# ikergarcia1996/AI-Generated-GTAV

Measured on AMD Instinct MI355X. Metric: generated frames/sec (32-frame clip, 100 noise steps), higher is better.
Workload: dtype fp16 (fp32 accumulate/residual)

## Files before the change

### ai-generated-gtav_amd/csrc/api_dit.hip

```cpp
#include "api_internal.h"

#ifdef GTAV_EXPERIMENTS
static int fold_alloc(gtav_dit* h) {
    gtav_dit::Fold& f = h->fold;
    if (f.ok) return 0;
    GTAV_REQUIRE(f.geom_ok, "dit_set_fold: this geometry has no LayerNorm fold (tokens per frame %d must be a multiple of 16 and >= 64, hidden %% 256 == 0)", h->P);
    Arena& a = h->arena;
    const int D = h->D;
    const size_t Mx = round_up(h->Mmax, 128);
    int rc = 0;
#define A_(expr) do { if (!rc) rc = (expr); } while (0)
    {
        const int nhb = h->L * 2, nseam = 2 * nhb + 1;
        f.col_c.assign(nseam, 0);
        int col = 0;
        for (int hb = 0; hb < nhb; ++hb) { f.col_c[2 * hb + 1] = col; col += 2 * h->Hm; }
        for (int hb = 0; hb < nhb; ++hb) { f.col_c[2 * hb] = col; col += 2 * 3 * D; }
        f.col_c[2 * nhb] = col; col += 2 * h->Nfin;
        f.CTW = col;
        f.n_groups = 2 * nseam; f.n_groups_a = 2 * nhb;
        f.Rp = round_up(h->max_rows, 128);
        A_(a.alloc_t(&f.ctab, (size_t)h->max_rows * f.CTW));
        A_(a.alloc_t(&f.ctab_cur, (size_t)h->maxB * h->maxT * f.CTW));
        A_(a.alloc_t(&f.stats, Mx * (size_t)(D / 64) * 2));
        A_(a.alloc_t(&f.sx, (size_t)f.n_groups * f.Rp * D));
        A_(a.alloc_t(&f.groups_dev, f.n_groups)); A_(a.alloc_t(&f.gcol_dev, f.n_groups)); A_(a.alloc_t(&f.gscale_dev, f.n_groups));
        if (!rc) {
            std::vector<GemmGroup> groups(f.n_groups);
            std::vector<int> gcol(f.n_groups), gsc(f.n_groups);
            auto add = [&](int q, int seam, const f16* W, int N, const float* bias, int shift_col, int scale_col) {
                for (int kind = 0; kind < 2; ++kind) {
                    GemmGroup& g = groups[2 * q + kind];
                    g.X = f.sx + (size_t)(2 * q + kind) * f.Rp * D; g.W = W; g.N = N; g.ldo = f.CTW;
                    g.out = f.ctab + f.col_c[seam] + (kind ? N : 0); g.bias = kind ? bias : nullptr;
                    gcol[2 * q + kind] = kind ? shift_col : scale_col; gsc[2 * q + kind] = kind ? 0 : 1;
                }
            };
            for (int hb = 0; hb < nhb; ++hb) {
                add(hb, 2 * hb + 1, h->halves[hb].w_fc1, h->Hm, h->halves[hb].b_fc1, (hb * 6 + 3) * D, (hb * 6 + 4) * D);
                add(nhb + hb, 2 * hb, h->halves[hb].w_qkv, 3 * D, nullptr, (hb * 6 + 0) * D, (hb * 6 + 1) * D);
            }
            add(2 * nhb, 2 * nhb, h->w_final, h->Nfin, h->b_final, h->L * 12 * D, h->L * 12 * D + D);
            if (hipMemcpy(f.groups_dev, groups.data(), groups.size() * sizeof(GemmGroup), hipMemcpyHostToDevice) != hipSuccess ||
                hipMemcpy(f.gcol_dev, gcol.data(), gcol.size() * sizeof(int), hipMemcpyHostToDevice) != hipSuccess ||
                hipMemcpy(f.gscale_dev, gsc.data(), gsc.size() * sizeof(int), hipMemcpyHostToDevice) != hipSuccess) {
                set_error("dit_create: upload of the LayerNorm-fold group tables failed");
                rc = 1;
            }
            f.ok = !rc;
        }
    }
#undef A_
    return rc;
}
#endif

static bool fused_spatial_ok(int M, int D, int P) { return gemm_qkvs_attn_ok(M, D, P) && M / P >= 5 && (M / P) * (D / 64) >= 80; }

static void fold_policy(const gtav_dit* h, int M, bool& fa, bool& fb) {
    const gtav_dit::Fold& f = h->fold;
    fa = fb = false;
    if (!f.ok || f.mode == 0 || h->tr.on || h->fuse_tattn || h->any_bf16) return;
    fa = f.mode == 2 || M >= f.min_m_a;
    fb = f.mode == 2 || M >= f.min_m_b;
}
static int dit_fold_tables(gtav_dit* h, int rows, bool fa, bool fb, hipStream_t s) {
    if (!fa && !fb) return 0;
#ifndef GTAV_EXPERIMENTS
    (void)h; (void)rows; (void)s;
    GTAV_REQUIRE(false, "the LayerNorm fold exists only in the experiments build");
#else
    gtav_dit::Fold& f = h->fold;
    const int ng = fb ? f.n_groups : f.n_groups_a;
    RET_IF(launch_ctab_inputs(h->mod, h->MODW, rows, round_up(rows, 128), h->D, f.gcol_dev, f.gscale_dev, ng, f.sx, (size_t)f.Rp * h->D, s));
    return launch_gemm_grouped(f.groups_dev, ng, h->Hm > 3 * h->D ? h->Hm : 3 * h->D, rows, h->D, s);
#endif
}

static int dit_cond(gtav_dit* h, const int64_t* t64, int rows, int Tq, const StepParams* sp, int use_cur, const float* actions,
                    int64_t act_outer, int64_t act_inner, hipStream_t s) {
    GTAV_REQUIRE(rows <= h->max_rows, "conditioning rows %d exceed max_cond_rows %d", rows, h->max_rows);
    const int ldhc = h->D + h->Apad;
    RET_IF(launch_cond_inputs(t64, rows, Tq, sp, use_cur, h->sincos, h->E, actions, act_outer, act_inner, h->A, h->HC, ldhc,
                              h->D, h->Apad, h->err_flag, s));
    RET_IF(launch_skinny_f32(h->E, 256, h->w_t0, h->b_t0, h->HC, ldhc, rows, h->D, 256, 1, s));
    RET_IF(launch_skinny_f32(h->HC, ldhc, h->w_t2cat, actions ? h->b_t2a : h->b_t2, h->Sc, h->D, rows, h->D, ldhc, 1, s));
    RET_IF(launch_skinny_f32(h->Sc, h->D, h->w_ada, h->b_ada, h->mod, h->MODW, rows, h->MODW, h->D, 0, s));
    bool fa, fb;
    fold_policy(h, rows * h->P, fa, fb);
    return dit_fold_tables(h, rows, fa, fb, s);
}

static int dit_forward_core(gtav_dit* h, const float* x_src, const int* frame_index, int B, int Tq, int t0,
                            const float* mod, const int* mod_rows, const float* ctab, float* v_out, hipStream_t s) {
    const int D = h->D, P = h->P, NB = B * Tq, M = NB * P;
    GTAV_REQUIRE(M <= h->Mmax, "forward: %d tokens exceed workspace (%d)", M, h->Mmax);
    bool fold_a, fold_b;
    fold_policy(h, M, fold_a, fold_b);
    const gtav_dit::Fold& fo = h->fold;
    auto fold_consumer = [&](GemmParams& q, int seam, int N) {
        q.bias = nullptr;
        q.f_P = P; q.f_rows = mod_rows; q.f_stats = fo.stats; q.f_nslot = D / 64;
        q.f_c1 = ctab + fo.col_c[seam]; q.f_c2 = q.f_c1 + N; q.f_ldc = fo.CTW;
    };
    auto fold_producer = [&](int cls, const f16* X, const f16* Wt, int K, const float* bias, const float* gate, const float* next_scale) -> int {
        GemmParams q;
        memset(&q, 0, sizeof(q));
        q.X = X; q.ldx = K; q.W = Wt; q.M = M; q.N = D; q.K = K; q.out = h->resid; q.ldo = D; q.bias = bias; q.err_flag = h->err_flag;
        q.gate = gate; q.gate_stride = h->MODW; q.gate_rows = mod_rows; q.rows_per_gate = P;
        q.f_P = P; q.f_rows = mod_rows; q.f_scale = next_scale; q.f_stats_out = fo.stats; q.f_a = h->xn;
        PROF(h, cls, s, launch_gemm(q, EPI_RESID_FOLD, s));
        return 0;
    };
    const int g_embed = 2 * h->L, g_final = 2 * h->L + 1;
    PROF(h, PC_OTHER, s, h->ops(g_embed).patchify(x_src, frame_index, NB, h->C, h->H, h->W, h->p, h->xp, h->Kpe, 1.f, 0.f, h->err_of(g_embed), s));
    GemmParams g;
    memset(&g, 0, sizeof(g));
    g.X = h->xp; g.ldx = h->Kpe; g.W = h->w_pe; g.M = M; g.N = D; g.K = h->Kpe; g.bias = h->b_pe; g.out = h->resid; g.ldo = D;
    PROF(h, PC_OTHER, s, h->ops(g_embed).gemm(g, EPI_F32, s));
    LnPending pend;
    bool have_pend = false;
    const int pf_max_m = 1536;
    static const int pf_min_m = GTAV_ENV_INT("GTAV_PF_MIN_M", 256);
    const bool pf_on = h->w_prefetch && M >= pf_min_m && M <= pf_max_m;
    struct PfNext { const f16* W; int N, K, sk, consumer; };
    auto pf_target = [&](int hb, int pos) -> PfNext {
        const int q = pos + 1, hb2 = hb + q / 4, p2 = q % 4;
        if (!pf_on || hb2 >= 2 * h->L) return PfNext{nullptr, 0, 0, 1, 0};
        const gtav_dit::Half& w2 = h->halves[hb2];
        if (p2 == 0) {
            const bool fused2 = !h->tr.on && w2.w_qkv_hm && !h->ops(hb2).bf16 &&
                                ((hb2 & 1) ? h->fuse_tattn && gemm_qkvt_attn_ok(M, D, P, Tq, t0) : h->fuse_sattn && fused_spatial_ok(M, D, P));
            return PfNext{fused2 ? w2.w_qkv_hm : w2.w_qkv, 3 * D, D, 1, 3};
        }
        if (p2 == 1) return PfNext{w2.w_out, D, D, gemm_choose_splitk(M, D, D), 0};
        if (p2 == 2) return PfNext{w2.w_fc1, h->Hm, D, 1, 1};
        return PfNext{w2.w_fc2, D, h->Hm_pad, gemm_choose_splitk(M, D, h->Hm_pad), 2};
    };
    auto set_pf = [&](GemmParams& q, const PfNext& t) {
        const int v = h->w_prefetch_cls[t.consumer];
        if (!pf_on || !t.W || !v) return;
        const int nkt = t.K / 64;
        int skn = t.sk;
        if (skn < 1 || nkt % skn || (skn >= 8 ? skn % 8 : 8 % skn)) skn = 1;
        q.pf = PrefetchDesc{t.W, cdiv(t.N, 128), nkt, skn, v >= 2 ? v : 0};
    };
    auto resid_gemm = [&](const OperandOps& ops, int cls, const f16* X, int ldx, const f16* Wt, int K, const float* bias, const float* gate, const PfNext& pfn) -> int {
        GemmParams q;
        memset(&q, 0, sizeof(q));
        q.X = X; q.ldx = ldx; q.W = Wt; q.M = M; q.N = D; q.K = K; q.out = h->parts; q.ldo = D;
        set_pf(q, pfn);
        q.splitk = gemm_choose_splitk(M, D, K);
        if (gemm_pp_ok(M, D, K, EPI_RESID) || (q.splitk == 1 && M >= h->resid_inplace_min_m) || gemm_resid_inplace_ok(M, D, K, P)) {
            q.splitk = 0; q.out = h->resid; q.bias = bias; q.gate = gate; q.gate_stride = h->MODW; q.gate_rows = mod_rows;
            q.rows_per_gate = P;
            PROF(h, cls, s, ops.gemm(q, EPI_RESID, s));
            have_pend = false;
            return 0;
        }
        GTAV_REQUIRE((size_t)q.splitk * M <= h->parts_rows, "split-K slabs exceed workspace");
        PROF(h, cls, s, ops.gemm(q, EPI_PARTIAL, s));
        memset(&pend, 0, sizeof(pend));
        pend.parts = h->parts; pend.nsplit = q.splitk; pend.slab_stride = (size_t)M * D; pend.ld = D; pend.bias = bias;
        pend.gate = gate; pend.gate_stride = h->MODW; pend.gate_rows = mod_rows; pend.rows_per_gate = P;
        have_pend = true;
        return 0;
    };
    bool folded_in = false;
    for (int l = 0; l < h->L; ++l) {
        for (int hf = 0; hf < 2; ++hf) {
            const int hb = l * 2 + hf;
            const gtav_dit::Half& w = h->halves[hb];
            const OperandOps& ops = h->ops(hb);
            int* const ef = h->err_of(hb);
            const float* mb = mod + (size_t)hb * 6 * D;
            const bool fused_t = hf == 1 && h->fuse_tattn && !h->tr.on && !ops.bf16 && w.w_qkv_hm && gemm_qkvt_attn_ok(M, D, P, Tq, t0);
            if (fused_t) {
                if (!have_pend) memset(&pend, 0, sizeof(pend));
                pend.tperm_T = Tq; pend.tperm_P = P;
            }
            if (!folded_in)
                PROF(h, PC_LN, s, ops.ln_modulate(h->resid, D, h->xn, D, M, D, mb, mb + D, h->MODW, mod_rows, P, (have_pend || fused_t) ? &pend : nullptr, ef, s));
            have_pend = false;
            memset(&g, 0, sizeof(g));
            g.X = h->xn; g.ldx = D; g.W = w.w_qkv; g.M = M; g.N = 3 * D; g.K = D; g.D = D; g.S = P; g.err_flag = ef;
            if (folded_in) fold_consumer(g, 2 * hb, 3 * D);
            set_pf(g, pf_target(hb, 0));
            const bool fused_s = hf == 0 && h->fuse_sattn && !h->tr.on && !ops.bf16 && !folded_in && w.w_qkv_hm && fused_spatial_ok(M, D, P);
            if (fused_t) {
                g.W = w.w_qkv_hm; g.qkv_mode = QKV_TEMPORAL; g.k = h->kvcache[l]; g.v = h->kvcache[l]; g.out = h->ao; g.ldo = D;
                g.Tq = Tq; g.t0 = t0; g.Tmax = h->maxT; g.rope_cs = h->rope_t.cs_dev;
                PROF(h, PC_ATTN_T, s, launch_gemm_qkvt_attn(g, s));
            } else if (fused_s) {
                g.W = w.w_qkv_hm; g.qkv_mode = QKV_SPATIAL; g.out = h->ao; g.ldo = D; g.rope_cs = h->rope_s.cs_dev;
                PROF(h, PC_ATTN_S, s, launch_gemm_qkvs_attn(g, s));
            } else {
                if (hf == 0) {
                    g.qkv_mode = QKV_SPATIAL; g.q = h->qs; g.k = h->ks; g.v = h->vts;
                    g.rope_cs = h->rope_s.cs_dev;
                } else {
                    g.qkv_mode = QKV_TEMPORAL; g.q = h->qt; g.k = h->kvcache[l]; g.v = h->kvcache[l];
                    g.Tq = Tq; g.t0 = t0; g.Tmax = h->maxT;
                    g.rope_cs = h->rope_t.cs_dev;
                }
                PROF(h, PC_QKV, s, ops.gemm(g, folded_in ? EPI_QKV_FOLD : EPI_QKV, s));
                if (hf == 0) PROF(h, PC_ATTN_S, s, ops.attn_spatial(h->qs, h->ks, h->vts, h->ao, NB, h->heads, P, s, false));
                else PROF(h, PC_ATTN_T, s, ops.attn_temporal(h->qt, h->kvcache[l], h->ao, B, P, D, Tq, t0, h->maxT, s));
            }
            folded_in = false;
            memset(&g, 0, sizeof(g));
            g.X = h->xn; g.ldx = D; g.W = w.w_fc1; g.M = M; g.N = h->Hm; g.K = D; g.bias = w.b_fc1; g.out = h->hbuf; g.ldo = h->Hm_pad; g.err_flag = ef;
            set_pf(g, pf_target(hb, 2));
            if (fold_a) {
                RET_IF(fold_producer(PC_OUT, h->ao, w.w_out, D, w.b_out, mb + 2 * D, mb + 4 * D));
                fold_consumer(g, 2 * hb + 1, h->Hm);
                PROF(h, PC_FC1, s, launch_gemm(g, EPI_GELU_TANH_FOLD, s));
            } else {
                RET_IF(resid_gemm(ops, PC_OUT, h->ao, D, w.w_out, D, w.b_out, mb + 2 * D, pf_target(hb, 1)));
                PROF(h, PC_LN, s, ops.ln_modulate(h->resid, D, h->xn, D, M, D, mb + 3 * D, mb + 4 * D, h->MODW, mod_rows, P, have_pend ? &pend : nullptr, ef, s));
                have_pend = false;
                PROF(h, PC_FC1, s, ops.gemm(g, EPI_GELU_TANH, s));
            }
            if (fold_b) {
                const float* next_scale = hb + 1 < 2 * h->L ? mod + (size_t)(hb + 1) * 6 * D + D : mod + (size_t)h->L * 12 * D + D;
                RET_IF(fold_producer(PC_FC2, h->hbuf, w.w_fc2, h->Hm_pad, w.b_fc2, mb + 5 * D, next_scale));
                folded_in = true;
            } else {
                RET_IF(resid_gemm(ops, PC_FC2, h->hbuf, h->Hm_pad, w.w_fc2, h->Hm_pad, w.b_fc2, mb + 5 * D, pf_target(hb, 3)));
            }
        }
    }
    const float* mf = mod + (size_t)h->L * 12 * D;
    if (!folded_in)
        PROF(h, PC_LN, s, h->ops(g_final).ln_modulate(h->resid, D, h->xn, D, M, D, mf, mf + D, h->MODW, mod_rows, P, have_pend ? &pend : nullptr, h->err_of(g_final), s));
    memset(&g, 0, sizeof(g));
    g.X = h->xn; g.ldx = D; g.W = h->w_final; g.M = M; g.N = h->Nfin; g.K = D; g.bias = h->b_final; g.out = h->fo; g.ldo = h->Nfin;
    if (folded_in) fold_consumer(g, 4 * h->L, h->Nfin);
    PROF(h, PC_OTHER, s, h->ops(g_final).gemm(g, folded_in ? EPI_F32_FOLD : EPI_F32, s));
    PROF(h, PC_OTHER, s, launch_unpatchify(h->fo, h->Nfin, v_out, NB, h->C, h->H, h->W, h->p, 0, 1.f, 0.f, s));
    PROF(h, PC_EMPTY, s, 0);
    return h->prof.collect(s);
}

extern "C" {



int gtav_dit_create(const gtav_dit_config* c, gtav_dit** out) {
    GTAV_REQUIRE(c && out, "dit_create: null argument");
    GTAV_REQUIRE(c->hidden_size % 256 == 0 && c->hidden_size <= 2048, "hidden_size=%d must be a multiple of 256, <= 2048", c->hidden_size);
    GTAV_REQUIRE(c->num_heads > 0 && c->hidden_size / c->num_heads == 64 && c->hidden_size % c->num_heads == 0,
                 "only head_dim 64 is implemented (hidden %d, heads %d)", c->hidden_size, c->num_heads);
    GTAV_REQUIRE(c->input_h % c->patch_size == 0 && c->input_w % c->patch_size == 0, "input %dx%d not divisible by patch %d",
                 c->input_h, c->input_w, c->patch_size);
    GTAV_REQUIRE(c->max_frames >= 1 && c->max_frames <= 32, "max_frames=%d must be in [1, 32]", c->max_frames);
    GTAV_REQUIRE(c->max_batch >= 1 && c->depth >= 1, "bad max_batch/depth");
    RET_IF(skinny_init());
    gtav_dit* h = new gtav_dit();
    h->cfg = *c;
    h->D = c->hidden_size; h->L = c->depth; h->heads = c->num_heads; h->C = c->in_channels; h->p = c->patch_size;
    h->H = c->input_h; h->W = c->input_w; h->gh = h->H / h->p; h->gw = h->W / h->p; h->P = h->gh * h->gw;
    const int D = h->D;
    if ((h->P % 8) != 0) {
        set_error("tokens per frame P=%d must be a multiple of 8", h->P);
        delete h;
        return 2;
    }
    h->Hm = (int)(D * c->mlp_ratio); h->Hm_pad = round_up(h->Hm, 128);
    h->A = c->external_cond_dim > 0 ? c->external_cond_dim : 0; h->Apad = round_up(h->A > 0 ? h->A : 1, 32);
    h->MODW = h->L * 12 * D + 2 * D;
    h->Kpe = round_up(h->C * h->p * h->p, 64);
    h->Nfin = h->p * h->p * h->C;
    h->maxB = c->max_batch; h->maxT = c->max_frames; h->Mmax = h->maxB * h->maxT * h->P;
    h->max_rows = c->max_cond_rows > h->maxB * h->maxT ? c->max_cond_rows : h->maxB * h->maxT;
    Arena& a = h->arena;
    WeightTable& wt = h->wt;
    int rc = 0;
#define A_(expr) do { if (!rc) rc = (expr); } while (0)
    A_(a.alloc_t(&h->w_pe, (size_t)round_up(D, 128) * h->Kpe));
    h->n_groups = 2 * h->L + 2;
    h->grp_bf16.assign(h->n_groups, 0);
    wt.add_f16("x_embedder.proj.weight", D, h->C * h->p * h->p, h->w_pe, round_up(D, 128), h->Kpe, 2 * h->L);
    A_(a.alloc_t(&h->b_pe, D)); wt.add_f32("x_embedder.proj.bias", 1, D, h->b_pe, D);
    A_(a.alloc_t(&h->w_t0, (size_t)D * 256)); wt.add_f32("t_embedder.mlp.0.weight", D, 256, h->w_t0, 256);
    A_(a.alloc_t(&h->b_t0, D)); wt.add_f32("t_embedder.mlp.0.bias", 1, D, h->b_t0, D);
    const int ldhc = D + h->Apad;
    A_(a.alloc_t(&h->w_t2cat, (size_t)D * ldhc)); wt.add_f32("t_embedder.mlp.2.weight", D, D, h->w_t2cat, ldhc, 0);
    A_(a.alloc_t(&h->b_t2, D)); wt.add_f32("t_embedder.mlp.2.bias", 1, D, h->b_t2, D);
    A_(a.alloc_t(&h->b_ext, D)); A_(a.alloc_t(&h->b_t2a, D));
    if (h->A > 0) {
        wt.add_f32("external_cond.weight", D, h->A, h->w_t2cat, ldhc, D);
        wt.add_f32("external_cond.bias", 1, D, h->b_ext, D);
    }
    A_(a.alloc_t(&h->w_ada, (size_t)h->MODW * D)); A_(a.alloc_t(&h->b_ada, h->MODW));
    h->halves.resize(h->L * 2);
    h->fuse_sattn = h->P == 144 && D % 256 == 0;
    for (int l = 0; l < h->L && !rc; ++l)
        for (int hf = 0; hf < 2; ++hf) {
            gtav_dit::Half& w = h->halves[l * 2 + hf];
            char pre[64];
            snprintf(pre, sizeof(pre), "blocks.%d.%c_", l, hf == 0 ? 's' : 't');
            std::string P_(pre);
            const int grp = l * 2 + hf;
            A_(a.alloc_t(&w.w_qkv, (size_t)3 * D * D)); wt.add_f16(P_ + "attn.to_qkv.weight", 3 * D, D, w.w_qkv, 3 * D, D, grp);
            w.w_qkv_hm = nullptr;
            if (hf == 0 && h->P == 144 && D % 256 == 0) A_(a.alloc_t(&w.w_qkv_hm, (size_t)3 * D * D));
            A_(a.alloc_t(&w.w_out, (size_t)D * D)); wt.add_f16(P_ + "attn.to_out.weight", D, D, w.w_out, D, D, grp);
            A_(a.alloc_t(&w.b_out, D)); wt.add_f32(P_ + "attn.to_out.bias", 1, D, w.b_out, D);
            A_(a.alloc_t(&w.w_fc1, (size_t)h->Hm_pad * D)); wt.add_f16(P_ + "mlp.fc1.weight", h->Hm, D, w.w_fc1, h->Hm_pad, D, grp);
            A_(a.alloc_t(&w.b_fc1, h->Hm_pad)); wt.add_f32(P_ + "mlp.fc1.bias", 1, h->Hm, w.b_fc1, h->Hm);
            A_(a.alloc_t(&w.w_fc2, (size_t)D * h->Hm_pad)); wt.add_f16(P_ + "mlp.fc2.weight", D, h->Hm, w.w_fc2, D, h->Hm_pad, grp);
            A_(a.alloc_t(&w.b_fc2, D)); wt.add_f32(P_ + "mlp.fc2.bias", 1, D, w.b_fc2, D);
            const size_t row0 = (size_t)(l * 2 + hf) * 6 * D;
            wt.add_f32(P_ + "adaLN_modulation.1.weight", 6 * D, D, h->w_ada + row0 * D, D);
            wt.add_f32(P_ + "adaLN_modulation.1.bias", 1, 6 * D, h->b_ada + row0, 6 * D);
        }
    A_(a.alloc_t(&h->w_final, (size_t)round_up(h->Nfin, 128) * D));
    wt.add_f16("final_layer.linear.weight", h->Nfin, D, h->w_final, round_up(h->Nfin, 128), D, 2 * h->L + 1);
    A_(a.alloc_t(&h->b_final, round_up(h->Nfin, 128))); wt.add_f32("final_layer.linear.bias", 1, h->Nfin, h->b_final, h->Nfin);
    {
        const size_t row0 = (size_t)h->L * 12 * D;
        wt.add_f32("final_layer.adaLN_modulation.1.weight", 2 * D, D, h->w_ada + row0 * D, D);
        wt.add_f32("final_layer.adaLN_modulation.1.bias", 1, 2 * D, h->b_ada + row0, 2 * D);
    }
    A_(a.alloc_t(&h->sincos, (size_t)1000 * 256)); wt.add_f32("tables.timestep_sincos", 1000, 256, h->sincos, 256, 0, false);
    h->rope_s.npos = h->P; h->rope_t.npos = h->maxT;
    A_(a.alloc_t(&h->rope_s.cos_dev, (size_t)h->P * 64)); wt.add_f32("tables.rope_spatial_cos", h->P, 64, h->rope_s.cos_dev, 64, 0, false);
    A_(a.alloc_t(&h->rope_s.sin_dev, (size_t)h->P * 64)); wt.add_f32("tables.rope_spatial_sin", h->P, 64, h->rope_s.sin_dev, 64, 0, false);
    A_(a.alloc_t(&h->rope_t.cos_dev, (size_t)h->maxT * 64)); wt.add_f32("tables.rope_temporal_cos", h->maxT, 64, h->rope_t.cos_dev, 64, 0, false);
    A_(a.alloc_t(&h->rope_t.sin_dev, (size_t)h->maxT * 64)); wt.add_f32("tables.rope_temporal_sin", h->maxT, 64, h->rope_t.sin_dev, 64, 0, false);
    A_(a.alloc_t(&h->rope_s.cs_dev, (size_t)h->P * 64)); A_(a.alloc_t(&h->rope_t.cs_dev, (size_t)h->maxT * 64));
    A_(a.alloc_t(&h->freqs_s_dev, 16)); wt.add_f32("spatial_rotary_emb.freqs", 1, 16, h->freqs_s_dev, 16, 0, false);
    A_(a.alloc_t(&h->freqs_t_dev, 32)); wt.add_f32("temporal_rotary_emb.freqs", 1, 32, h->freqs_t_dev, 32, 0, false);
    const size_t Mx = round_up(h->Mmax, 128);
    A_(a.alloc_t(&h->xp, Mx * h->Kpe)); A_(a.alloc_t(&h->xn, Mx * D)); A_(a.alloc_t(&h->qs, Mx * D)); A_(a.alloc_t(&h->ks, Mx * D));
    A_(a.alloc_t(&h->vts, Mx * D)); A_(a.alloc_t(&h->qt, Mx * D)); A_(a.alloc_t(&h->ao, Mx * D)); A_(a.alloc_t(&h->hbuf, Mx * h->Hm_pad));
    h->kvcache.resize(h->L);
    for (int l = 0; l < h->L; ++l) A_(a.alloc_t(&h->kvcache[l], Mx * 2 * D));
    A_(a.alloc_t(&h->resid, Mx * D)); A_(a.alloc_t(&h->fo, Mx * h->Nfin));
    A_(a.alloc_t(&h->vout, Mx / h->P * h->C * h->H * h->W));
    h->parts_rows = (2 * Mx * D > (size_t)(8u << 20) ? 2 * Mx * D : (size_t)(8u << 20)) / D;
    A_(a.alloc_t(&h->parts, h->parts_rows * D));
    const size_t R = h->max_rows;
    A_(a.alloc_t(&h->E, R * 256)); A_(a.alloc_t(&h->HC, R * ldhc)); A_(a.alloc_t(&h->Sc, R * D)); A_(a.alloc_t(&h->mod, R * h->MODW));
    A_(a.alloc_t(&h->err_flag, 4 + h->n_groups)); A_(a.alloc_t(&h->frame_idx, (size_t)h->maxB * h->maxT)); A_(a.alloc_t(&h->ac_table, 1000));
    A_(a.alloc_t(&h->step_dev, 4)); A_(a.alloc_t(&h->mod_rows_dev, (size_t)h->maxB * h->maxT));
    A_(a.alloc_t(&h->mod_cur, (size_t)h->maxB * h->maxT * h->MODW)); A_(a.alloc_t(&h->mod_last, (size_t)h->maxB * h->maxT)); A_(a.alloc_t(&h->mod_changed, (size_t)h->maxB * h->maxT)); A_(a.alloc_t(&h->t_steps_dev, 1024));
    wt.err_words = h->err_flag; wt.err_per_group = true;
    h->use_graph = GTAV_ENV_INT("GTAV_GRAPH", 1) != 0;
    h->fold.geom_ok = h->P % 16 == 0 && h->P >= 64 && D % 256 == 0 && h->Hm % 128 == 0 && h->Nfin % 4 == 0;
#undef A_
    if (rc) {
        delete h;
        return rc;
    }
    *out = h;
    return 0;
}

void gtav_dit_destroy(gtav_dit* h) { delete h; }

int gtav_dit_set_weight(gtav_dit* h, const char* name, const float* src, int64_t numel, void* stream) {
    GTAV_REQUIRE(h && name && src, "dit_set_weight: null argument");
    std::string n(name);
    if (n.size() > 16 && n.compare(n.size() - 16, 16, "rotary_emb.freqs") == 0) {
        const bool spatial = n.rfind("spatial_", 0) == 0 || n.find(".s_attn.") != std::string::npos;
        n = spatial ? "spatial_rotary_emb.freqs" : "temporal_rotary_emb.freqs";
    }
    h->finalized = false;
    return h->wt.set(n.c_str(), src, numel, (hipStream_t)stream);
}

int gtav_dit_get_weight(gtav_dit* h, const char* name, float* dst, int64_t numel, void* stream) {
    GTAV_REQUIRE(h && name && dst, "dit_get_weight: null argument");
    return h->wt.get(name, dst, numel, (hipStream_t)stream);
}

int gtav_dit_finalize(gtav_dit* h, void* stream) {
    GTAV_REQUIRE(h, "dit_finalize: null handle");
    hipStream_t s = (hipStream_t)stream;
    RET_IF(h->wt.check_complete());
    GTAV_CHECK_HIP(hipStreamSynchronize(s));
    const int D = h->D;
    RET_IF(launch_add_f32(h->b_t2, h->b_ext, h->b_t2a, D, s));
    std::vector<float> fs(16), ft(32);
    if (h->wt.slots["spatial_rotary_emb.freqs"].set) GTAV_CHECK_HIP(hipMemcpy(fs.data(), h->freqs_s_dev, 64, hipMemcpyDeviceToHost));
    else { std::vector<float> l = linspace_f32(1.0f, 128.0f, 16); for (int i = 0; i < 16; ++i) fs[i] = l[i] * (float)M_PI; }
    if (h->wt.slots["temporal_rotary_emb.freqs"].set) GTAV_CHECK_HIP(hipMemcpy(ft.data(), h->freqs_t_dev, 128, hipMemcpyDeviceToHost));
    else for (int i = 0; i < 32; ++i) ft[i] = 1.0f / powf(10000.0f, (float)(2 * i) / 64.0f);
    if (!(h->wt.slots["tables.rope_spatial_cos"].set && h->wt.slots["tables.rope_spatial_sin"].set)) {
        std::vector<float> c, sn;
        build_axial_table(fs, h->gh, h->gw, c, sn);
        RET_IF(upload(h->rope_s.cos_dev, c)); RET_IF(upload(h->rope_s.sin_dev, sn));
    }
    if (!(h->wt.slots["tables.rope_temporal_cos"].set && h->wt.slots["tables.rope_temporal_sin"].set)) {
        std::vector<float> c((size_t)h->maxT * 64), sn((size_t)h->maxT * 64);
        for (int t = 0; t < h->maxT; ++t)
            for (int d = 0; d < 64; ++d) {
                const float ang = (float)t * ft[d / 2];
                c[t * 64 + d] = cosf(ang); sn[t * 64 + d] = sinf(ang);
            }
        RET_IF(upload(h->rope_t.cos_dev, c)); RET_IF(upload(h->rope_t.sin_dev, sn));
    }
    if (!h->wt.slots["tables.timestep_sincos"].set) {
        std::vector<float> tab((size_t)1000 * 256);
        for (int k = 0; k < 128; ++k) {
            const float f = expf(-logf(10000.0f) * (float)k / 128.0f);
            for (int t = 0; t < 1000; ++t) {
                const float arg = (float)t * f;
                tab[(size_t)t * 256 + k] = cosf(arg);
                tab[(size_t)t * 256 + 128 + k] = sinf(arg);
            }
        }
        RET_IF(upload(h->sincos, tab));
    }
    for (size_t hb = 0; hb < h->halves.size(); ++hb) {
        gtav_dit::Half& w = h->halves[hb];
        if (w.w_qkv_hm) RET_IF(launch_qkv_head_major(w.w_qkv, w.w_qkv_hm, D, s, (hb & 1) ? 0 : 1));
    }
    RET_IF(launch_rope_interleave(h->rope_s.cos_dev, h->rope_s.sin_dev, h->rope_s.cs_dev, h->P, s));
    RET_IF(launch_rope_interleave(h->rope_t.cos_dev, h->rope_t.sin_dev, h->rope_t.cs_dev, h->maxT, s));
    GTAV_CHECK_HIP(hipStreamSynchronize(s));
    h->finalized = true;
    return 0;
}

int gtav_dit_forward(gtav_dit* h, const float* x, const int64_t* t, const float* actions, float* out, int32_t B, int32_t T,
                     void* stream) {
    GTAV_REQUIRE(h && x && t && out, "dit_forward: null argument");
    GTAV_REQUIRE(h->finalized, "dit_forward: call gtav_dit_finalize first");
    GTAV_REQUIRE(B >= 1 && B <= h->maxB && T >= 1 && T <= h->maxT, "dit_forward: B=%d T=%d outside capacity (%d, %d)", B, T, h->maxB, h->maxT);
    GTAV_REQUIRE(!actions || h->A > 0, "dit_forward: model has no external_cond");
    hipStream_t s = (hipStream_t)stream;
    h->prepared.valid = false;
    h->kvrec.valid = false;
    RET_IF(dit_cond(h, t, B * T, 1, nullptr, 0, actions, h->A, 0, s));
    return dit_forward_core(h, x, nullptr, B, T, 0, h->mod, nullptr, h->fold.ctab, out, s);
}

int gtav_dit_set_schedule(gtav_dit* h, const float* ac, int32_t n) {
    GTAV_REQUIRE(h && ac && n == 1000, "dit_set_schedule: expected 1000 alphas_cumprod values");
    h->ac_host.assign(ac, ac + n);
    GTAV_CHECK_HIP(hipMemcpy(h->ac_table, ac, n * sizeof(float), hipMemcpyHostToDevice));
    return 0;
}

static int denoise_step_body(gtav_dit* h, float* x, int B, int F, int T, const float* actions, int mode, float* v_out,
                             bool prepared, hipStream_t s) {
    const size_t fsz = (size_t)h->C * h->H * h->W;
    const int Tq = mode == 1 ? 1 : T, t0 = mode == 1 ? T - 1 : 0;
    if (!prepared) RET_IF(dit_cond(h, nullptr, B * Tq, Tq, h->step_dev, mode == 1, actions, (int64_t)F * h->A, h->A, s));
    RET_IF(dit_forward_core(h, x, h->frame_idx, B, Tq, t0, prepared ? h->mod_cur : h->mod, nullptr, prepared ? h->fold.ctab_cur : h->fold.ctab, h->vout, s));
    const float* vlast = h->vout + (size_t)(Tq - 1) * fsz;
    RET_IF(launch_ddim_update_step(x, F, vlast, (size_t)Tq * fsz, B, (int)fsz, h->step_dev, s));
    if (v_out) RET_IF(launch_copy_rows_f32(vlast, (size_t)Tq * fsz, v_out, fsz, B, fsz, s));
    return 0;
}

int gtav_dit_prepare_frame(gtav_dit* h, int32_t B, int32_t F, int32_t start, int32_t cur, int32_t t_ctx,
                           const int32_t* t_steps_host, int32_t n_steps, const float* actions, void* stream) {
    GTAV_REQUIRE(h && t_steps_host, "prepare_frame: null argument");
    GTAV_REQUIRE(h->finalized, "prepare_frame: finalize the model first");
    const int T = cur - start + 1;
    GTAV_REQUIRE(start >= 0 && cur < F && T >= 1 && T <= h->maxT && B >= 1 && B <= h->maxB && n_steps >= 1 && n_steps <= 1024,
                 "prepare_frame: bad window [%d, %d] / steps %d", start, cur, n_steps);
    GTAV_REQUIRE(!actions || h->A > 0, "prepare_frame: model has no external_cond");
    const int rows = B * (T - 1) + n_steps * B;
    GTAV_REQUIRE(rows <= h->max_rows, "prepare_frame: %d conditioning rows exceed max_cond_rows %d", rows, h->max_rows);
    hipStream_t s = (hipStream_t)stream;
    GTAV_CHECK_HIP(hipStreamSynchronize(s));
    GTAV_CHECK_HIP(hipMemcpy(h->t_steps_dev, t_steps_host, n_steps * sizeof(int), hipMemcpyHostToDevice));
    const int ldhc = h->D + h->Apad;
    RET_IF(launch_cond_inputs_frame(rows, B, T, F, start, cur, t_ctx, h->t_steps_dev, h->sincos, h->E, actions, h->A, h->HC, ldhc,
                                    h->D, h->Apad, h->err_flag, s));
    RET_IF(launch_skinny_f32(h->E, 256, h->w_t0, h->b_t0, h->HC, ldhc, rows, h->D, 256, 1, s));
    RET_IF(launch_skinny_f32(h->HC, ldhc, h->w_t2cat, actions ? h->b_t2a : h->b_t2, h->Sc, h->D, rows, h->D, ldhc, 1, s));
    RET_IF(launch_skinny_f32(h->Sc, h->D, h->w_ada, h->b_ada, h->mod, h->MODW, rows, h->MODW, h->D, 0, s));
    {
        bool fa, fb, fa1, fb1;
        fold_policy(h, B * T * h->P, fa, fb);
        fold_policy(h, B * h->P, fa1, fb1);
        RET_IF(dit_fold_tables(h, rows, fa || fa1, fb || fb1, s));
        h->prepared.fold_tables = fa || fa1 || fb || fb1;
    }
    GTAV_CHECK_HIP(hipMemsetAsync(h->mod_last, 0xFF, (size_t)h->maxB * h->maxT * sizeof(int), s));
    h->prepared.valid = true; h->prepared.B = B; h->prepared.F = F; h->prepared.start = start; h->prepared.cur = cur;
    h->prepared.n_steps = n_steps; h->prepared.actions = actions;
    return 0;
}

int gtav_dit_denoise_step(gtav_dit* h, float* x, int32_t B, int32_t F, int32_t start, int32_t cur, int32_t t_ctx,
                          int32_t t_cur, int32_t t_next, int32_t is_final, const float* actions, int32_t mode,
                          int32_t cond_step, float* v_out, void* stream) {
    GTAV_REQUIRE(h && x, "denoise_step: null argument");
    GTAV_REQUIRE(h->finalized && !h->ac_host.empty(), "denoise_step: finalize the model and set the schedule first");
    const int T = cur - start + 1;
    GTAV_REQUIRE(start >= 0 && cur < F && T >= 1 && T <= h->maxT && B >= 1 && B <= h->maxB, "denoise_step: bad window [%d, %d] of %d frames", start, cur, F);
    GTAV_REQUIRE(t_cur >= 0 && t_cur < 1000 && t_next >= 0 && t_next < 1000 && t_ctx >= 0 && t_ctx < 1000, "denoise_step: timestep out of range");
    GTAV_REQUIRE(!actions || h->A > 0, "denoise_step: model has no external_cond");
    GTAV_REQUIRE(mode == 0 || mode == 1, "denoise_step: mode %d", mode);
    const bool prepared = cond_step >= 0;
    if (prepared)
        GTAV_REQUIRE(h->prepared.valid && h->prepared.B == B && h->prepared.F == F && h->prepared.start == start &&
                         h->prepared.cur == cur && cond_step < h->prepared.n_steps && h->prepared.actions == actions,
                     "denoise_step: cond_step=%d but gtav_dit_prepare_frame was not called for this window", cond_step);
    else
        h->prepared.valid = false;
    if (mode == 1) {
        GTAV_REQUIRE(h->kvrec.valid && h->kvrec.B == B && h->kvrec.F == F && h->kvrec.start == start && h->kvrec.cur == cur &&
                         h->kvrec.x == (const void*)x,
                     "denoise_step: context-cached step (mode 1) on window [%d, %d] without a preceding full-window step (mode 0) "
                     "on the same batch / window / latent buffer: the temporal K/V caches would be stale", start, cur);
    } else {
        h->kvrec.valid = true; h->kvrec.B = B; h->kvrec.F = F; h->kvrec.start = start; h->kvrec.cur = cur; h->kvrec.x = x;
    }
    hipStream_t s = (hipStream_t)stream;
    StepParams sp;
    sp.first = start; sp.cur = cur; sp.t_ctx = t_ctx; sp.t_cur = t_cur; sp.is_final = is_final != 0;
    sp.alpha_t = h->ac_host[t_cur]; sp.alpha_next = h->ac_host[t_next]; sp.cond_step = cond_step;
    RET_IF(launch_step_setup(h->step_dev, sp, h->frame_idx, h->mod_rows_dev, prepared ? h->mod_last : nullptr, h->mod_changed, B, mode == 1 ? 1 : T, T, F,
                             mode == 1, s));
    if (prepared) RET_IF(launch_gather_rows(h->mod, h->mod_rows_dev, h->mod_changed, h->mod_cur, B * (mode == 1 ? 1 : T), h->MODW,
                                            h->prepared.fold_tables ? h->fold.ctab : nullptr, h->fold.ctab_cur, h->fold.CTW, s));
    if (!h->use_graph || h->prof.on) return denoise_step_body(h, x, B, F, T, actions, mode, v_out, prepared, s);

    gtav_dit::GraphKey key{B, F, T, mode * 2 + (prepared ? 1 : 0), x, actions, v_out};
    auto it = h->graphs.find(key);
    if (it == h->graphs.end()) {
        if (h->graphs.size() > 64) {
            for (auto& kv : h->graphs)
                if (kv.second) (void)hipGraphExecDestroy(kv.second);
            h->graphs.clear();
        }
        h->graphs[key] = nullptr;
        return denoise_step_body(h, x, B, F, T, actions, mode, v_out, prepared, s);
    }
    if (!it->second) {
        if (!h->cap_stream && hipStreamCreateWithFlags(&h->cap_stream, hipStreamNonBlocking) != hipSuccess) {
            h->use_graph = false;
            return denoise_step_body(h, x, B, F, T, actions, mode, v_out, prepared, s);
        }
        hipGraph_t graph = nullptr;
        if (hipStreamBeginCapture(h->cap_stream, hipStreamCaptureModeThreadLocal) != hipSuccess) {
            (void)hipGetLastError();
            h->use_graph = false;
            return denoise_step_body(h, x, B, F, T, actions, mode, v_out, prepared, s);
        }
        const int rc = denoise_step_body(h, x, B, F, T, actions, mode, v_out, prepared, h->cap_stream);
        const hipError_t ce = hipStreamEndCapture(h->cap_stream, &graph);
        if (rc || ce != hipSuccess || !graph) {
            if (graph) (void)hipGraphDestroy(graph);
            h->use_graph = false;
            if (rc) return rc;
            return denoise_step_body(h, x, B, F, T, actions, mode, v_out, prepared, s);
        }
        hipGraphExec_t exec = nullptr;
        const hipError_t ie = hipGraphInstantiate(&exec, graph, nullptr, nullptr, 0);
        (void)hipGraphDestroy(graph);
        if (ie != hipSuccess || !exec) {
            h->use_graph = false;
            return denoise_step_body(h, x, B, F, T, actions, mode, v_out, prepared, s);
        }
        it->second = exec;
    }
    GTAV_CHECK_HIP(hipGraphLaunch(it->second, s));
    return 0;
}

int gtav_dit_set_graph(gtav_dit* h, int32_t enable) {
    GTAV_REQUIRE(h, "dit_set_graph: null handle");
    h->use_graph = enable != 0;
    return 0;
}

int gtav_dit_set_weight_prefetch(gtav_dit* h, int32_t enable) {
    GTAV_REQUIRE(h, "dit_set_weight_prefetch: null handle");
    GTAV_REQUIRE(enable == 0 || enable == 1 || (enable >> 16) == 1,
                 "dit_set_weight_prefetch: mode %d (0 off, 1 on, 0x10000 | per-class nibbles: bits 0-3 out-proj's weight, 4-7 fc1's, 8-11 fc2's, 12-15 to_qkv's; "
                 "nibble 0 = not prefetched, 1 = the whole slice, k >= 2 = the first k K tiles of every row tile)", enable);
    int cls[4];
    for (int c = 0; c < 4; ++c) cls[c] = enable == 0 ? 0 : enable == 1 ? 1 : (enable >> (4 * c)) & 15;
    const bool on = cls[0] || cls[1] || cls[2] || cls[3];
    if (h->w_prefetch != on || memcmp(cls, h->w_prefetch_cls, sizeof(cls))) {
        for (auto& kv : h->graphs)
            if (kv.second) (void)hipGraphExecDestroy(kv.second);
        h->graphs.clear();
    }
    h->w_prefetch = on;
    memcpy(h->w_prefetch_cls, cls, sizeof(cls));
    return 0;
}

#ifdef GTAV_EXPERIMENTS
int gtav_dit_set_fold(gtav_dit* h, int32_t mode, int32_t min_tokens_a, int32_t min_tokens_b) {
    GTAV_REQUIRE(h && mode >= 0 && mode <= 2, "dit_set_fold: mode %d", mode);
    if (min_tokens_a >= 0) h->fold.min_m_a = min_tokens_a;
    if (min_tokens_b >= 0) h->fold.min_m_b = min_tokens_b;
    if (mode == 2 || (mode == 1 && (h->fold.min_m_a < (1 << 30) || h->fold.min_m_b < (1 << 30)))) RET_IF(fold_alloc(h));
    for (auto& kv : h->graphs)
        if (kv.second) (void)hipGraphExecDestroy(kv.second);
    h->graphs.clear();
    h->prepared.valid = false;
    h->fold.mode = mode;
    return 0;
}
#endif

int gtav_dit_set_fused_temporal(gtav_dit* h, int32_t enable) {
    GTAV_REQUIRE(h, "dit_set_fused_temporal: null handle");
    if (h->fuse_tattn != (enable != 0)) {
        for (auto& kv : h->graphs)
            if (kv.second) (void)hipGraphExecDestroy(kv.second);
        h->graphs.clear();
    }
    if (enable && h->P % 16 == 0 && h->D % 256 == 0 && h->maxT >= 5) {
        for (int l = 0; l < h->L; ++l) {
            gtav_dit::Half& w = h->halves[l * 2 + 1];
            if (w.w_qkv_hm) continue;
            RET_IF(h->arena.alloc_t(&w.w_qkv_hm, (size_t)3 * h->D * h->D));
            if (h->finalized) RET_IF(launch_qkv_head_major(w.w_qkv, w.w_qkv_hm, h->D, nullptr));
        }
        if (h->finalized) GTAV_CHECK_HIP(hipDeviceSynchronize());
    }
    h->fuse_tattn = enable != 0;
    return 0;
}

int gtav_dit_set_fused_spatial(gtav_dit* h, int32_t enable) {
    GTAV_REQUIRE(h, "dit_set_fused_spatial: null handle");
    if (h->fuse_sattn != (enable != 0)) {
        for (auto& kv : h->graphs)
            if (kv.second) (void)hipGraphExecDestroy(kv.second);
        h->graphs.clear();
    }
    if (enable && h->P == 144 && h->D % 256 == 0) {
        for (int l = 0; l < h->L; ++l) {
            gtav_dit::Half& w = h->halves[l * 2];
            if (w.w_qkv_hm) continue;
            RET_IF(h->arena.alloc_t(&w.w_qkv_hm, (size_t)3 * h->D * h->D));
            if (h->finalized) RET_IF(launch_qkv_head_major(w.w_qkv, w.w_qkv_hm, h->D, nullptr, 1));
        }
        if (h->finalized) GTAV_CHECK_HIP(hipDeviceSynchronize());
    }
    h->fuse_sattn = enable != 0;
    return 0;
}

int gtav_dit_fused_launches(gtav_dit* h, int32_t B, int32_t T, int32_t t0) {
    if (!h || B < 1 || T < 1) return 0;
    const int M = B * T * h->P;
    int mask = 0;
    for (int hb = 0; hb < 2 * h->L; ++hb) {
        const gtav_dit::Half& w = h->halves[hb];
        if (h->tr.on || h->ops(hb).bf16 || !w.w_qkv_hm) continue;
        if (!(hb & 1) && h->fuse_sattn && fused_spatial_ok(M, h->D, h->P)) mask |= 1;
        if ((hb & 1) && h->fuse_tattn && gemm_qkvt_attn_ok(M, h->D, h->P, T, t0)) mask |= 2;
    }
    return mask;
}

int gtav_dit_profile(gtav_dit* h, int32_t enable) {
    GTAV_REQUIRE(h, "dit_profile: null handle");
    h->prof.on = enable != 0;
    h->prof.used = 0;
    for (int i = 0; i < PC_COUNT; ++i) { h->prof.ms[i] = 0; h->prof.n[i] = 0; }
    return 0;
}
int gtav_dit_profile_read(gtav_dit* h, double* ms_by_class, int64_t* launches_by_class) {
    GTAV_REQUIRE(h && ms_by_class && launches_by_class, "dit_profile_read: null argument");
    for (int i = 0; i < PC_COUNT; ++i) { ms_by_class[i] = h->prof.ms[i]; launches_by_class[i] = h->prof.n[i]; }
    return 0;
}


static int dit_read_err_words(gtav_dit* h, std::vector<int>& words, hipStream_t s) {
    words.assign(4 + h->n_groups, 0);
    GTAV_CHECK_HIP(hipMemcpyAsync(words.data(), h->err_flag, words.size() * sizeof(int), hipMemcpyDeviceToHost, s));
    GTAV_CHECK_HIP(hipStreamSynchronize(s));
    GTAV_CHECK_HIP(hipMemsetAsync(h->err_flag, 0, words.size() * sizeof(int), s));
    return 0;
}

int gtav_dit_check(gtav_dit* h, void* stream) {
    GTAV_REQUIRE(h, "dit_check: null handle");
    std::vector<int> w;
    RET_IF(dit_read_err_words(h, w, (hipStream_t)stream));
    int flag = w[0];
    for (int g = 0; g < h->n_groups; ++g) flag |= w[4 + g];
    return report_err_flag(flag, "DiT");
}

static void dit_drop_graphs(gtav_dit* h) {
    for (auto& kv : h->graphs)
        if (kv.second) (void)hipGraphExecDestroy(kv.second);
    h->graphs.clear();
}

int gtav_dit_set_operand_dtype(gtav_dit* h, int32_t group, int32_t dtype) {
    GTAV_REQUIRE(h, "dit_set_operand_dtype: null handle");
    GTAV_REQUIRE(dtype == GTAV_OPERAND_F16 || dtype == GTAV_OPERAND_BF16, "dit_set_operand_dtype: dtype %d (0 = fp16, 1 = bf16)", dtype);
    GTAV_REQUIRE(group >= -1 && group < h->n_groups, "dit_set_operand_dtype: group %d outside [-1, %d)", group, h->n_groups);
    if (h->tr.on && h->tr.bf16)
        GTAV_REQUIRE(dtype == GTAV_OPERAND_BF16, "dit_set_operand_dtype: a bf16 training handle keeps bf16 operands in every group (its masters, optimizer state and "
                     "loss scale were set up for them; create a new handle to train on fp16 operands)");
    else
        GTAV_REQUIRE(!h->tr.on || dtype == GTAV_OPERAND_F16, "dit_set_operand_dtype: a training handle keeps fp16 operands (its backward pass and loss scaling are fp16)");
    int changed = 0;
    for (int g = (group < 0 ? 0 : group); g < (group < 0 ? h->n_groups : group + 1); ++g) {
        if ((h->grp_bf16[g] != 0) == (dtype == GTAV_OPERAND_BF16)) continue;
        h->grp_bf16[g] = dtype == GTAV_OPERAND_BF16;
        changed += 1 + h->wt.set_dtype(g, dtype == GTAV_OPERAND_BF16);
    }
    if (changed) {
        h->finalized = false;
        h->kvrec.valid = false;
        dit_drop_graphs(h);
    }
    h->any_bf16 = false;
    for (unsigned char b : h->grp_bf16) h->any_bf16 |= b != 0;
    return 0;
}

int gtav_dit_get_operand_dtype(gtav_dit* h, int32_t group, int32_t* dtype) {
    GTAV_REQUIRE(h && dtype && group >= 0 && group < h->n_groups, "dit_get_operand_dtype: bad argument (group %d of %d)", group, h ? h->n_groups : 0);
    *dtype = h->grp_bf16[group] ? GTAV_OPERAND_BF16 : GTAV_OPERAND_F16;
    return 0;
}

int gtav_dit_operand_groups(gtav_dit* h, int32_t* n_groups) {
    GTAV_REQUIRE(h && n_groups, "dit_operand_groups: null argument");
    *n_groups = h->n_groups;
    return 0;
}

int gtav_dit_autorange(gtav_dit* h, int32_t* n_switched, void* stream) {
    GTAV_REQUIRE(h && n_switched, "dit_autorange: null argument");
    *n_switched = 0;
    std::vector<int> w;
    RET_IF(dit_read_err_words(h, w, (hipStream_t)stream));
    int other = w[0];
    for (int g = 0; g < h->n_groups; ++g) {
        other |= w[4 + g] & ~ERR_F16_SAT;
        if ((w[4 + g] & ERR_F16_SAT) && !h->grp_bf16[g]) {
            RET_IF(gtav_dit_set_operand_dtype(h, g, GTAV_OPERAND_BF16));
            *n_switched += 1;
        }
    }
    return report_err_flag(other, "DiT");
}

}
```

### ai-generated-gtav_amd/csrc/api_internal.h

```cpp
#pragma once
#include "../../include/gtav_amd.h"
#include "../../include/gtav_amd_testing.h"
#include "ops.h"
#include "ops_bf16.h"

#include <cmath>
#include <cstdarg>
#include <cstdio>
#include <cstdlib>
#include <cstring>
#include <map>
#include <string>
#include <tuple>
#include <vector>

using namespace gtav;

#define RET_IF(expr)            \
    do {                        \
        int _rc = (expr);       \
        if (_rc) return _rc;    \
    } while (0)

namespace gtav {
// ... 157 lines not shown
        attached = false;
        GTAV_CHECK_HIP(hipEventRecord(ev[used], s));
        return 0;
    }
    int end(hipStream_t s) {
        if (!on) return 0;
        if (attached && g_launch_ev[0]) {
            g_launch_ev[0] = nullptr;
            GTAV_CHECK_HIP(hipEventRecord(ev[used], s));
            attached = false;
        }
        if (!attached) GTAV_CHECK_HIP(hipEventRecord(ev[used + 1], s));
        used += 2;
        return 0;
    }
    int collect(hipStream_t s) {
        if (!on || used == 0) return 0;
        GTAV_CHECK_HIP(hipStreamSynchronize(s));
        for (size_t i = 0; i < used; i += 2) {
            float t = 0.f;
            GTAV_CHECK_HIP(hipEventElapsedTime(&t, ev[i], ev[i + 1]));
            ms[cls[i / 2]] += t;
            n[cls[i / 2]] += 1;
        }
        used = 0;
        return 0;
    }
    ~Profiler() {
        for (hipEvent_t e : ev) (void)hipEventDestroy(e);
    }
};
#define PROF(h, c, s, expr)            \
    do {                               \
        RET_IF((h)->prof.begin(c, s)); \
        RET_IF(expr);                  \
        RET_IF((h)->prof.end(s));      \
    } while (0)

inline int report_err_flag(int flag, const char* who) {
    GTAV_REQUIRE(!(flag & ERR_TIMESTEP), "%s: a timestep outside [0, 999] was passed", who);
    GTAV_REQUIRE(!(flag & ERR_NONFINITE), "%s: a NaN or inf was found in the input tensor", who);
    GTAV_REQUIRE(!(flag & ERR_F16_SAT), "%s: an activation exceeded the fp16 range (|x| > 65504) and was saturated; results since the "
                 "last check are finite but clipped (the reference runs this path in bf16, which has fp32 range)", who);
    return 0;
}

}
}
using namespace gtav::api;

struct gtav_dit {
    Profiler prof;
    gtav_dit_config cfg;
    int D, L, heads, P, gh, gw, C, p, H, W, Hm, Hm_pad, A, Apad, MODW, Kpe, Nfin, maxB, maxT, Mmax, max_rows;
    Arena arena;
    WeightTable wt;
    f16 *w_pe = nullptr, *w_final = nullptr;
    struct Half { f16 *w_qkv, *w_out, *w_fc1, *w_fc2; float *b_out, *b_fc1, *b_fc2; f16* w_qkv_hm; };
    std::vector<Half> halves;
    float *b_pe = nullptr, *b_final = nullptr;
    float *w_t0, *b_t0, *w_t2cat, *b_t2, *b_ext, *b_t2a, *w_ada, *b_ada;
    float* sincos = nullptr;
    bool sincos_set = false;
    RopeTable rope_s, rope_t;
    std::vector<float> freqs_s, freqs_t;
    float *freqs_s_dev = nullptr, *freqs_t_dev = nullptr;
    f16 *xp, *xn, *qs, *ks, *vts, *qt, *ao, *hbuf;
    std::vector<f16*> kvcache;
    float *resid, *fo, *vout, *E, *HC, *Sc, *mod, *parts;
    size_t parts_rows = 0;
    int* err_flag = nullptr;
    std::vector<unsigned char> grp_bf16;
    int n_groups = 0;
    bool any_bf16 = false;
    const OperandOps& ops(int g) const { return operand_ops(grp_bf16[g] != 0); }
    int* err_of(int g) const { return err_flag + 4 + g; }
    int* frame_idx = nullptr;
    StepParams* step_dev = nullptr;
    int* mod_rows_dev = nullptr;
    float* mod_cur = nullptr;
    int *mod_last = nullptr, *mod_changed = nullptr;
    int* t_steps_dev = nullptr;
    struct { bool valid = false, fold_tables = false; int B = 0, F = 0, start = 0, cur = 0, n_steps = 0; const float* actions = nullptr; } prepared;
    struct { bool valid = false; int B = 0, F = 0, start = 0, cur = 0; const void* x = nullptr; } kvrec;
    struct GraphKey {
        int B, F, T, mode;
        const void *x, *actions, *vout;
        bool operator<(const GraphKey& o) const {
            return std::tie(B, F, T, mode, x, actions, vout) < std::tie(o.B, o.F, o.T, o.mode, o.x, o.actions, o.vout);
        }
    };
    std::map<GraphKey, hipGraphExec_t> graphs;
    bool use_graph = true;
    bool fuse_tattn = false;
    bool fuse_sattn = false;
    bool w_prefetch = true;
    int w_prefetch_cls[4] = {1, 4, 4, 1};
    int resid_inplace_min_m = GTAV_ENV_INT("GTAV_RESID_INPLACE_MIN_M", 1 << 30);
    struct Fold {
        bool geom_ok = false;
        bool ok = false;
        int mode = 1;
        int min_m_a = 1 << 30, min_m_b = 1 << 30;
        int CTW = 0, n_groups = 0, n_groups_a = 0, Rp = 0;
        std::vector<int> col_c;
        float *ctab = nullptr, *ctab_cur = nullptr, *stats = nullptr;
        f16* sx = nullptr;
        GemmGroup* groups_dev = nullptr;
        int *gcol_dev = nullptr, *gscale_dev = nullptr;
    } fold;
    hipStream_t cap_stream = nullptr;
    ~gtav_dit() {
        for (auto& kv : graphs)
            if (kv.second) (void)hipGraphExecDestroy(kv.second);
        if (cap_stream) (void)hipStreamDestroy(cap_stream);
    }
    float* ac_table = nullptr;
    std::vector<float> ac_host;
    bool finalized = false;
    struct Train {
        bool on = false, have_fwd = false, have_actions = false;
        bool bf16 = false;
        int B = 0, T = 0, M = 0, Mp = 0, rows = 0;
        float loss_scale = 65536.0f;
        float grad_div = 1.0f;
        std::vector<Slot*> params;
        float* grad_arena = nullptr;
        size_t grad_count = 0;
        float* ctl = nullptr;
        float *ln_part = nullptr;
        float *red_ws = nullptr, *sumsq_part = nullptr;
        AdamParam* adam_params = nullptr;
        AdamItem* adam_items = nullptr;
        int adam_n_items = 0;
        std::vector<float*> res;
        struct HB { f16 *xnA, *ao, *y1, *xnB, *u, *hh, *y2, *q, *k, *v; };
        std::vector<HB> hb;
        f16 *xnF = nullptr, *xp = nullptr;
        float *z0 = nullptr, *cpre = nullptr;
        float *dres = nullptr, *dtmp = nullptr, *stats = nullptr, *dmod = nullptr, *dSc = nullptr, *ada_part = nullptr, *dc = nullptr, *dh0 = nullptr, *dz0 = nullptr;
        f16 *g_d = nullptr, *g_d2 = nullptr, *g_h = nullptr, *g_u = nullptr, *g_qkv = nullptr, *dao = nullptr, *tA = nullptr, *tB = nullptr, *dfo = nullptr;
        f16 *tAg[4] = {nullptr, nullptr, nullptr, nullptr}, *tBg[4] = {nullptr, nullptr, nullptr, nullptr};
    } tr;
};
```

### ai-generated-gtav_amd/csrc/api_train.hip

```cpp
#include "api_internal.h"

static int g_dw_grouped = GTAV_ENV_INT("GTAV_DW_GROUPED", 1);
static int g_fuse_gelu_fwd = GTAV_ENV_INT("GTAV_FUSE_GELU_FWD", 1);
static int g_fuse_gelu = GTAV_ENV_INT("GTAV_FUSE_GELU_BWD", 1);
static int g_fuse_ln = GTAV_ENV_INT("GTAV_FUSE_LN_BWD", 1);
static int g_fuse_gate = GTAV_ENV_INT("GTAV_FUSE_GATE", 1);
static int g_dw_tn = GTAV_ENV_INT("GTAV_DW_TN", 1);

static int train_enable_body(gtav_dit* h, float* grad_arena_dev, int64_t grad_arena_numel);

static int train_window_ok(const gtav_dit* h) {
    GTAV_REQUIRE(h->maxT <= 8, "train_enable: training is implemented for windows of at most 8 frames (the backward temporal attention and the adaLN-gradient "
                 "reduction are sized for it); this handle was created with max_frames=%d", h->maxT);
    return 0;
}

extern "C" {

int gtav_dit_train_enable(gtav_dit* h, float* grad_arena_dev, int64_t grad_arena_numel) {
    GTAV_REQUIRE(h, "train_enable: null handle");
    RET_IF(train_window_ok(h));
    GTAV_REQUIRE(!h->tr.on, "train_enable: already enabled");
    GTAV_REQUIRE(!h->any_bf16, "train_enable: the training step runs on fp16 operands (gtav_dit_set_operand_dtype(h, -1, GTAV_OPERAND_F16) first)");
    return train_enable_body(h, grad_arena_dev, grad_arena_numel);
}

int gtav_dit_train_enable_typed(gtav_dit* h, float* grad_arena_dev, int64_t grad_arena_numel, int32_t dtype) {
    GTAV_REQUIRE(h, "train_enable_typed: null handle");
    GTAV_REQUIRE(dtype == GTAV_OPERAND_F16 || dtype == GTAV_OPERAND_BF16, "train_enable_typed: dtype %d (0 = fp16, 1 = bf16)", dtype);
    if (dtype == GTAV_OPERAND_F16) return gtav_dit_train_enable(h, grad_arena_dev, grad_arena_numel);
    RET_IF(train_window_ok(h));
    GTAV_REQUIRE(!h->tr.on, "train_enable: already enabled");
    int nb = 0;
    for (unsigned char b : h->grp_bf16) nb += b != 0;
    GTAV_REQUIRE(nb == 0 || nb == h->n_groups, "train_enable_typed: %d of the %d operand groups are bf16; a training handle has one operand type for every group", nb,
                 h->n_groups);
    for (auto& kv : h->wt.slots) GTAV_REQUIRE(!kv.second.set, "train_enable: call it before any gtav_dit_set_weight (the fp32 masters are filled by set_weight)");
    RET_IF(gtav_dit_set_operand_dtype(h, -1, GTAV_OPERAND_BF16));
    h->tr.bf16 = true;
    h->tr.loss_scale = 1.0f;
    return train_enable_body(h, grad_arena_dev, grad_arena_numel);
}

}

static int train_enable_body(gtav_dit* h, float* grad_arena_dev, int64_t grad_arena_numel) {
    for (auto& kv : h->wt.slots) GTAV_REQUIRE(!kv.second.set, "train_enable: call it before any gtav_dit_set_weight (the fp32 masters are filled by set_weight)");
    gtav_dit::Train& t = h->tr;
    Arena& a = h->arena;
    const int D = h->D, L = h->L, Hp = h->Hm_pad;
    GTAV_REQUIRE(h->Hm == h->Hm_pad && h->Kpe == h->C * h->p * h->p, "train_enable: padded MLP width / patch size are not implemented for training");
    size_t count = 0;
    std::vector<std::string> names;
    for (auto& kv : h->wt.slots) {
        const std::string& n = kv.first;
        if (n.rfind("tables.", 0) == 0 || n.find("rotary_emb.freqs") != std::string::npos) continue;
        kv.second.trainable = true;
        t.params.push_back(&kv.second);
        names.push_back(n);
        count += (size_t)kv.second.R * kv.second.C;
    }
    t.grad_count = count;
    if (grad_arena_dev) {
        GTAV_REQUIRE(grad_arena_numel == (int64_t)count, "train_enable: the gradient arena has %lld elements, the model has %lld trainable parameters",
                     (long long)grad_arena_numel, (long long)count);
        t.grad_arena = grad_arena_dev;
    } else {
        RET_IF(a.alloc_t(&t.grad_arena, count));
    }
    size_t off = 0;
    for (size_t pi = 0; pi < t.params.size(); ++pi) {
        Slot* sl = t.params[pi];
        const size_t n = (size_t)sl->R * sl->C;
        sl->grad = t.grad_arena + off;
        off += n;
        RET_IF(a.alloc_t(&sl->am, n));
        RET_IF(a.alloc_t(&sl->av, n));
        if (sl->kind == SLOT_F16_PAD) {
            RET_IF(a.alloc_t(&sl->master, n));
            if (names[pi] != "x_embedder.proj.weight")
                RET_IF(a.alloc_t(&sl->wT, (size_t)round_up(sl->C, 128) * round_up(sl->R, 64)));
        } else {
            sl->master = (float*)sl->dst + sl->c0;
        }
    }
    RET_IF(a.alloc_t(&t.ctl, 8));
    RET_IF(a.alloc_t(&t.red_ws, colsum_workspace(h->Mmax > h->max_rows ? h->Mmax : h->max_rows, h->Hm_pad > 6 * D ? h->Hm_pad : 6 * D)));
    RET_IF(a.alloc_t(&t.sumsq_part, (size_t)sumsq_parts(count)));
    {
        std::vector<AdamParam> ap;
        std::vector<AdamItem> ai;
        for (size_t pi = 0; pi < t.params.size(); ++pi) {
            Slot* sl = t.params[pi];
            AdamParam d;
            memset(&d, 0, sizeof(d));
            const bool f16w = sl->kind == SLOT_F16_PAD;
            d.p = sl->master; d.ldp = f16w ? sl->C : sl->Cp; d.R = sl->R; d.C = sl->C; d.g = sl->grad; d.m = sl->am; d.v = sl->av;
            if (f16w) { d.w16 = (f16*)sl->dst; d.Cp16 = sl->Cp; d.wT = sl->wT; d.RpT = round_up(sl->R, 64); }
            ap.push_back(d);
            if (f16w) {
                const unsigned nt = (unsigned)(cdiv(sl->R, 64) * cdiv(sl->C, 64));
                for (unsigned i = 0; i < nt; ++i) ai.push_back(AdamItem{(int)pi, i});
            } else {
                const size_t n = (size_t)sl->R * sl->C;
                for (size_t st = 0; st < n; st += 4096) ai.push_back(AdamItem{(int)pi, (unsigned)st});
            }
        }
        RET_IF(a.alloc_t(&t.adam_params, ap.size()));
        RET_IF(a.alloc_t(&t.adam_items, ai.size()));
        GTAV_CHECK_HIP(hipMemcpy(t.adam_params, ap.data(), ap.size() * sizeof(AdamParam), hipMemcpyHostToDevice));
        GTAV_CHECK_HIP(hipMemcpy(t.adam_items, ai.data(), ai.size() * sizeof(AdamItem), hipMemcpyHostToDevice));
        t.adam_n_items = (int)ai.size();
    }
    const size_t Mx = round_up(h->Mmax, 128), Mp = round_up(h->Mmax, 64), Mm = h->Mmax;
    t.res.resize(4 * L + 1);
    for (auto& r : t.res) RET_IF(a.alloc_t(&r, Mx * D));
    t.hb.resize(2 * L);
    for (int i = 0; i < 2 * L; ++i) {
        gtav_dit::Train::HB& b = t.hb[i];
        RET_IF(a.alloc_t(&b.xnA, Mx * D)); RET_IF(a.alloc_t(&b.ao, Mx * D)); RET_IF(a.alloc_t(&b.y1, Mx * D)); RET_IF(a.alloc_t(&b.xnB, Mx * D));
        RET_IF(a.alloc_t(&b.u, Mx * Hp)); RET_IF(a.alloc_t(&b.hh, Mx * Hp)); RET_IF(a.alloc_t(&b.y2, Mx * D));
        RET_IF(a.alloc_t(&b.q, Mx * D));
        if (i % 2 == 0) { RET_IF(a.alloc_t(&b.k, Mx * D)); RET_IF(a.alloc_t(&b.v, Mx * D)); }
        else { RET_IF(a.alloc_t(&b.k, Mx * 2 * D)); b.v = b.k; }
    }
    RET_IF(a.alloc_t(&t.xnF, Mx * D)); RET_IF(a.alloc_t(&t.xp, Mx * h->Kpe));
    const size_t R = h->max_rows;
    RET_IF(a.alloc_t(&t.z0, R * D)); RET_IF(a.alloc_t(&t.cpre, R * D));
    RET_IF(a.alloc_t(&t.dres, Mx * D)); RET_IF(a.alloc_t(&t.dtmp, Mx * D)); RET_IF(a.alloc_t(&t.stats, 2 * Mx));
    if (ln_bwd_fused_ok(D)) RET_IF(a.alloc_t(&t.ln_part, ln_bwd_fused_workspace((int)R, h->P, D)));
    RET_IF(a.alloc_t(&t.dmod, R * h->MODW)); RET_IF(a.alloc_t(&t.dSc, R * D)); RET_IF(a.alloc_t(&t.ada_part, ada_bwd_dx_workspace(h->MODW, D, (int)R))); RET_IF(a.alloc_t(&t.dc, R * D)); RET_IF(a.alloc_t(&t.dh0, R * D));
    RET_IF(a.alloc_t(&t.dz0, R * D));
    RET_IF(a.alloc_t(&t.g_d, Mx * D)); RET_IF(a.alloc_t(&t.g_d2, Mx * D)); RET_IF(a.alloc_t(&t.g_h, Mx * Hp)); RET_IF(a.alloc_t(&t.g_u, Mx * Hp)); RET_IF(a.alloc_t(&t.g_qkv, Mx * 3 * D));
    RET_IF(a.alloc_t(&t.dao, Mm * D)); RET_IF(a.alloc_t(&t.dfo, Mx * 64));
    const size_t widest = (size_t)(Hp > 3 * D ? Hp : 3 * D);
    RET_IF(a.alloc_t(&t.tA, widest * Mp)); RET_IF(a.alloc_t(&t.tB, widest * Mp));
    if (D % 256 == 0 && Hp % 256 == 0) {
        const size_t ra[4] = {(size_t)D, (size_t)Hp, (size_t)D, (size_t)3 * D}, rb[4] = {(size_t)Hp, (size_t)D, (size_t)D, (size_t)D};
        for (int i = 0; i < 4; ++i) { RET_IF(a.alloc_t(&t.tAg[i], ra[i] * Mp)); RET_IF(a.alloc_t(&t.tBg[i], rb[i] * Mp)); }
    }
    t.on = true;
    return 0;
}

extern "C" {

int gtav_dit_train_param_count(gtav_dit* h, int64_t* numel) {
    GTAV_REQUIRE(h && numel, "train_param_count: null argument");
    int64_t c = 0;
    for (auto& kv : h->wt.slots) {
        const std::string& n = kv.first;
        if (n.rfind("tables.", 0) == 0 || n.find("rotary_emb.freqs") != std::string::npos) continue;
        c += (int64_t)kv.second.R * kv.second.C;
    }
    *numel = c;
    return 0;
}

int gtav_dit_set_loss_scale(gtav_dit* h, float scale) {
    GTAV_REQUIRE(h && scale > 0.f, "set_loss_scale: bad argument");
    h->tr.loss_scale = scale;
    return 0;
}

int gtav_dit_set_grad_divisor(gtav_dit* h, float divisor) {
    GTAV_REQUIRE(h && h->tr.on && divisor >= 1.0f, "set_grad_divisor: bad argument");
    h->tr.grad_div = divisor;
    return 0;
}
int gtav_dit_zero_grad(gtav_dit* h, void* stream) {
    GTAV_REQUIRE(h && h->tr.on, "zero_grad: training is not enabled");
    RET_IF(launch_fill_f32(h->tr.grad_arena, h->tr.grad_count, 0.f, (hipStream_t)stream));
    return launch_err_clear(h->err_flag, ERR_F16_SAT | ERR_NONFINITE, (hipStream_t)stream);
}

int gtav_dit_get_grad(gtav_dit* h, const char* name, float* dst, int64_t numel, void* stream) {
    GTAV_REQUIRE(h && name && dst && h->tr.on, "get_grad: bad argument / training is not enabled");
    auto it = h->wt.slots.find(name);
    GTAV_REQUIRE(it != h->wt.slots.end() && it->second.grad, "get_grad: '%s' is not a trainable parameter", name);
    GTAV_REQUIRE(numel == (int64_t)it->second.R * it->second.C, "get_grad: '%s' size mismatch", name);
    GTAV_CHECK_HIP(hipMemcpyAsync(dst, it->second.grad, numel * sizeof(float), hipMemcpyDeviceToDevice, (hipStream_t)stream));
    return 0;
}

int gtav_dit_train_forward(gtav_dit* h, const float* x, const int64_t* t64, const float* actions, float* out, int32_t B, int32_t T, void* stream) {
    GTAV_REQUIRE(h && x && t64 && out, "train_forward: null argument");
    GTAV_REQUIRE(h->tr.on && h->finalized, "train_forward: call gtav_dit_train_enable, load the weights and finalize first");
    GTAV_REQUIRE(B >= 1 && B <= h->maxB && T >= 1 && T <= h->maxT, "train_forward: B=%d T=%d outside capacity (%d, %d)", B, T, h->maxB, h->maxT);
    GTAV_REQUIRE(!actions || h->A > 0, "train_forward: model has no external_cond");
    hipStream_t s = (hipStream_t)stream;
    gtav_dit::Train& tr = h->tr;
    const int D = h->D, P = h->P, NB = B * T, M = NB * P, L = h->L, rows = NB, ldhc = D + h->Apad;
    h->prepared.valid = false;
    h->kvrec.valid = false;
    RET_IF(launch_cond_inputs(t64, rows, 1, nullptr, 0, h->sincos, h->E, actions, h->A, 0, h->A, h->HC, ldhc, D, h->Apad, h->err_flag, s));
    RET_IF(launch_skinny_f32(h->E, 256, h->w_t0, h->b_t0, tr.z0, D, rows, D, 256, 0, s));
    RET_IF(launch_silu(tr.z0, D, h->HC, ldhc, rows, D, s));
    RET_IF(launch_skinny_f32(h->HC, ldhc, h->w_t2cat, actions ? h->b_t2a : h->b_t2, tr.cpre, D, rows, D, ldhc, 0, s));
    RET_IF(launch_silu(tr.cpre, D, h->Sc, D, rows, D, s));
    RET_IF(launch_skinny_f32(h->Sc, D, h->w_ada, h->b_ada, h->mod, h->MODW, rows, h->MODW, D, 0, s));
    const float* mod = h->mod;
    const OperandOps& oe = h->ops(2 * L), &ofin = h->ops(2 * L + 1);
    RET_IF(oe.patchify(x, nullptr, NB, h->C, h->H, h->W, h->p, tr.xp, h->Kpe, 1.f, 0.f, h->err_flag, s));
    GemmParams g;
    memset(&g, 0, sizeof(g));
    g.X = tr.xp; g.ldx = h->Kpe; g.W = h->w_pe; g.M = M; g.N = D; g.K = h->Kpe; g.bias = h->b_pe; g.out = tr.res[0]; g.ldo = D;
    RET_IF(oe.gemm(g, EPI_F32, s));
    LnPending pend;
    bool have_pend = false;
    auto resid_gemm = [&](const OperandOps& o, const f16* X, const f16* Wt, int K, const float* bias, const float* gate, float* x_out, f16* y_save) -> int {
        GemmParams q;
        memset(&q, 0, sizeof(q));
        q.X = X; q.ldx = K; q.W = Wt; q.M = M; q.N = D; q.K = K; q.out = h->parts; q.ldo = D;
        q.splitk = gemm_choose_splitk(M, D, K);
        GTAV_REQUIRE((size_t)q.splitk * M <= h->parts_rows, "split-K slabs exceed workspace");
        RET_IF(o.gemm(q, EPI_PARTIAL, s));
        memset(&pend, 0, sizeof(pend));
        pend.parts = h->parts; pend.nsplit = q.splitk; pend.slab_stride = (size_t)M * D; pend.ld = D; pend.bias = bias;
        pend.gate = gate; pend.gate_stride = h->MODW; pend.gate_rows = nullptr; pend.rows_per_gate = P;
        pend.x_out = x_out; pend.y_save = y_save;
        have_pend = true;
        return 0;
    };
    for (int l = 0; l < L; ++l)
        for (int hf = 0; hf < 2; ++hf) {
            const int i = l * 2 + hf;
            const gtav_dit::Half& w = h->halves[i];
            gtav_dit::Train::HB& b = tr.hb[i];
            const float* mb = mod + (size_t)i * 6 * D;
            const OperandOps& o = h->ops(i);
            RET_IF(o.ln_modulate(i == 0 ? tr.res[0] : tr.res[2 * i - 1], D, b.xnA, D, M, D, mb, mb + D, h->MODW, nullptr, P, have_pend ? &pend : nullptr, h->err_flag, s));
            have_pend = false;
            memset(&g, 0, sizeof(g));
            g.X = b.xnA; g.ldx = D; g.W = w.w_qkv; g.M = M; g.N = 3 * D; g.K = D; g.D = D; g.S = P; g.err_flag = h->err_flag;
            if (hf == 0) { g.qkv_mode = QKV_SPATIAL; g.q = b.q; g.k = b.k; g.v = b.v; g.rope_cs = h->rope_s.cs_dev; }
            else { g.qkv_mode = QKV_TEMPORAL; g.q = b.q; g.k = b.k; g.v = b.k; g.Tq = T; g.t0 = 0; g.Tmax = h->maxT; g.rope_cs = h->rope_t.cs_dev; }
            RET_IF(o.gemm(g, EPI_QKV, s));
            if (hf == 0) RET_IF(o.attn_spatial(b.q, b.k, b.v, b.ao, NB, h->heads, P, s, false));
            else RET_IF(o.attn_temporal(b.q, b.k, b.ao, B, P, D, T, 0, h->maxT, s));
            RET_IF(resid_gemm(o, b.ao, w.w_out, D, w.b_out, mb + 2 * D, tr.res[2 * i + 1], b.y1));
            RET_IF(o.ln_modulate(tr.res[2 * i], D, b.xnB, D, M, D, mb + 3 * D, mb + 4 * D, h->MODW, nullptr, P, &pend, h->err_flag, s));
            have_pend = false;
            memset(&g, 0, sizeof(g));
            g.X = b.xnB; g.ldx = D; g.W = w.w_fc1; g.M = M; g.N = h->Hm; g.K = D; g.bias = w.b_fc1; g.out = b.u; g.ldo = h->Hm_pad; g.err_flag = h->err_flag;
            if (g_fuse_gelu_fwd) g.out2 = b.hh;
            RET_IF(o.gemm(g, EPI_F16_TILED, s));
            if (!g_fuse_gelu_fwd) RET_IF(h->ops(i).gelu_tiled(b.u, b.hh, (size_t)round_up(M, 128) * h->Hm_pad, s));
            RET_IF(resid_gemm(o, b.hh, w.w_fc2, h->Hm_pad, w.b_fc2, mb + 5 * D, tr.res[2 * i + 2], b.y2));
        }
    const float* mf = mod + (size_t)L * 12 * D;
    RET_IF(ofin.ln_modulate(tr.res[4 * L - 1], D, tr.xnF, D, M, D, mf, mf + D, h->MODW, nullptr, P, &pend, h->err_flag, s));
    memset(&g, 0, sizeof(g));
    g.X = tr.xnF; g.ldx = D; g.W = h->w_final; g.M = M; g.N = h->Nfin; g.K = D; g.bias = h->b_final; g.out = h->fo; g.ldo = h->Nfin;
    RET_IF(ofin.gemm(g, EPI_F32, s));
    RET_IF(launch_unpatchify(h->fo, h->Nfin, out, NB, h->C, h->H, h->W, h->p, 0, 1.f, 0.f, s));
    tr.B = B; tr.T = T; tr.M = M; tr.Mp = round_up(M, 64); tr.rows = rows; tr.have_actions = actions != nullptr; tr.have_fwd = true;
    return 0;
}

int gtav_dit_train_get_residual(gtav_dit* h, int32_t k, float* dst, int64_t numel, void* stream) {
    GTAV_REQUIRE(h && dst && h->tr.on && h->tr.have_fwd, "train_get_residual: no saved forward");
    GTAV_REQUIRE(k >= 0 && k <= 4 * h->L, "train_get_residual: k=%d must be in [0, %d]", k, 4 * h->L);
    GTAV_REQUIRE(numel == (int64_t)h->tr.M * h->D, "train_get_residual: expected %lld elements", (long long)h->tr.M * h->D);
    GTAV_CHECK_HIP(hipMemcpyAsync(dst, h->tr.res[k], numel * sizeof(float), hipMemcpyDeviceToDevice, (hipStream_t)stream));
    return 0;
}

int gtav_dit_train_backward_phases(gtav_dit* h, const float* v_pred, const float* v_target, int32_t phase_begin, int32_t phase_end, void* stream) {
    GTAV_REQUIRE(h && v_pred && v_target, "train_backward: null argument");
    GTAV_REQUIRE(h->tr.on && h->tr.have_fwd, "train_backward: no saved forward (gtav_dit_train_forward)");
    GTAV_REQUIRE(phase_begin >= 0 && phase_begin <= phase_end && phase_end <= h->L + 2, "train_backward: phases [%d, %d) outside [0, %d]", phase_begin, phase_end,
                 h->L + 2);
    hipStream_t s = (hipStream_t)stream;
    gtav_dit::Train& tr = h->tr;
    const int D = h->D, P = h->P, L = h->L, B = tr.B, T = tr.T, M = tr.M, Mp = tr.Mp, NB = B * T, rows = tr.rows, Hp = h->Hm_pad, MODW = h->MODW;
    const int ldhc = D + h->Apad;
// ... 114 lines not shown
        RET_IF(gemm_dx(tr.g_u, slot(P_ + "mlp.fc1.weight").wT, D, Hp, EPI_F32, tr.dtmp, D));
        RET_IF(ln_bwd(tr.dtmp, tr.res[2 * i + 1], mb + 4 * D, 1, dmb + 3 * D, dmb + 4 * D));
        f16* const g_o = tn_dw ? tr.g_d2 : tr.g_d;
        if (fuse_gate) {
            RET_IF(op->gate_bwd_fused(tr.dres, b.y1, mb + 2 * D, MODW, NB, P, D, g_o, dmb + 2 * D, defer_bias ? nullptr : slot(P_ + "attn.to_out.bias").grad, ws_out, h->err_flag, s));
        } else {
            RET_IF(op->gate_bwd(tr.dres, mb + 2 * D, MODW, P, M, D, g_o, h->err_flag, s));
            RET_IF(op->frame_reduce_gate(tr.dres, b.y1, NB, P, D, dmb + 2 * D, MODW, s));
            RET_IF(op->colsum_tiled(g_o, M, D, slot(P_ + "attn.to_out.bias").grad, tr.red_ws, s));
        }
        RET_IF(gemm_dw(g_o, D, b.ao, D, slot(P_ + "attn.to_out.weight").grad, 2));
        RET_IF(gemm_dx(g_o, slot(P_ + "attn.to_out.weight").wT, D, D, EPI_F16, tr.dao, D));
        if (hf == 0) RET_IF(op->attn_spatial_bwd(b.q, b.k, b.v, tr.dao, NB, h->heads, P, D, h->rope_s.cs_dev, tr.g_qkv, h->err_flag, s));
        else RET_IF(op->attn_temporal_bwd(b.q, b.k, tr.dao, B, P, D, T, h->maxT, h->rope_t.cs_dev, tr.g_qkv, h->err_flag, s));
        RET_IF(gemm_dw(tr.g_qkv, 3 * D, b.xnA, D, slot(P_ + "attn.to_qkv.weight").grad, 3));
        if (defer_bias) {
            const float* wsv[3] = {ws_fc2, ws_out, ws_fc1};
            float* dbv[3] = {slot(P_ + "mlp.fc2.bias").grad, slot(P_ + "attn.to_out.bias").grad, slot(P_ + "mlp.fc1.bias").grad};
            const int spv[3] = {NB, NB, gelu_bwd_colsum_splits(M)}, nv[3] = {D, D, Hp};
            RET_IF(launch_colsum_reduce_multi(wsv, dbv, spv, nv, 3, s));
        }
        RET_IF(flush_dw());
        RET_IF(gemm_dx(tr.g_qkv, slot(P_ + "attn.to_qkv.weight").wT, D, 3 * D, EPI_F32, tr.dtmp, D));
        RET_IF(ln_bwd(tr.dtmp, tr.res[2 * i], mb + D, 1, dmb, dmb + D));
        RET_IF(ada_grads((size_t)i * 6 * D, 6 * D, P_ + "adaLN_modulation.1.weight", P_ + "adaLN_modulation.1.bias"));
    }
    if (!(phase_begin <= L + 1 && L + 1 < phase_end)) return 0;
    op = &h->ops(2 * L);
    RET_IF(launch_colsum_f32(tr.dres, D, M, D, slot("x_embedder.proj.bias").grad, tr.red_ws, s));
    RET_IF(op->to_tiled(tr.dres, M, D, tr.g_d, h->err_flag, s));
    {
        Slot& wpe = slot("x_embedder.proj.weight");
        GTAV_REQUIRE(wpe.C == h->Kpe, "train_backward: a patch embedding with padded K (%d of %d) is not implemented", wpe.C, h->Kpe);
        RET_IF(gemm_dw(tr.g_d, D, tr.xp, h->Kpe, wpe.grad));
    }
    RET_IF(launch_ada_bwd_dx(dmod, MODW, h->w_ada, D, rows, tr.dSc, tr.ada_part, s));
    RET_IF(launch_silu_bwd(tr.dSc, D, tr.cpre, D, tr.dc, D, rows, D, s));
    RET_IF(launch_colsum_f32(tr.dc, D, rows, D, slot("t_embedder.mlp.2.bias").grad, tr.red_ws, s));
    RET_IF(launch_gemm_tn_f32(tr.dc, D, h->HC, ldhc, rows, D, D, slot("t_embedder.mlp.2.weight").grad, D, s));
    if (tr.have_actions) {
        RET_IF(launch_colsum_f32(tr.dc, D, rows, D, slot("external_cond.bias").grad, tr.red_ws, s));
        RET_IF(launch_gemm_tn_f32(tr.dc, D, h->HC + D, ldhc, rows, D, h->A, slot("external_cond.weight").grad, h->A, s));
    }
    RET_IF(launch_gemm_nn_f32(tr.dc, D, h->w_t2cat, ldhc, rows, D, D, tr.dh0, D, s));
    RET_IF(launch_silu_bwd(tr.dh0, D, tr.z0, D, tr.dz0, D, rows, D, s));
    RET_IF(launch_colsum_f32(tr.dz0, D, rows, D, slot("t_embedder.mlp.0.bias").grad, tr.red_ws, s));
    RET_IF(launch_gemm_tn_f32(tr.dz0, D, h->E, 256, rows, D, 256, slot("t_embedder.mlp.0.weight").grad, 256, s));
    RET_IF(launch_overflow_publish(h->err_flag, slot("x_embedder.proj.bias").grad, s));
    return 0;
}

int gtav_dit_train_backward(gtav_dit* h, const float* v_pred, const float* v_target, void* stream) {
    GTAV_REQUIRE(h, "train_backward: null handle");
    return gtav_dit_train_backward_phases(h, v_pred, v_target, 0, h->L + 2, stream);
}

int gtav_dit_train_param_range(gtav_dit* h, const char* prefix, int64_t* offset, int64_t* count) {
    GTAV_REQUIRE(h && prefix && offset && count && h->tr.on, "train_param_range: bad argument / training is not enabled");
    const size_t plen = strlen(prefix);
    int64_t off = -1, cnt = 0, last_end = -1;
    for (auto& kv : h->wt.slots) {
        Slot& sl = kv.second;
        if (!sl.grad || kv.first.compare(0, plen, prefix) != 0) continue;
        const int64_t o = sl.grad - h->tr.grad_arena, n = (int64_t)sl.R * sl.C;
        if (off < 0) off = o;
        GTAV_REQUIRE(last_end < 0 || o == last_end, "train_param_range: parameters with prefix '%s' are not contiguous in the arena", prefix);
        last_end = o + n;
        cnt += n;
    }
    GTAV_REQUIRE(off >= 0, "train_param_range: no trainable parameter starts with '%s'", prefix);
    *offset = off;
    *count = cnt;
    return 0;
}

int gtav_dit_adamw_step(gtav_dit* h, float lr, float beta1, float beta2, float eps, float weight_decay, float max_grad_norm, void* stream) {
    GTAV_REQUIRE(h && h->tr.on, "adamw_step: training is not enabled");
    hipStream_t s = (hipStream_t)stream;
    gtav_dit::Train& tr = h->tr;
    RET_IF(launch_sumsq(tr.grad_arena, tr.grad_count, tr.sumsq_part, s));
    RET_IF(launch_clip_coef(tr.ctl, tr.sumsq_part, sumsq_parts(tr.grad_count), 1.0f / (tr.loss_scale * tr.grad_div), max_grad_norm, beta1, beta2, h->err_flag, s));
    RET_IF(operand_ops(tr.bf16).adamw_multi(tr.adam_params, tr.adam_items, tr.adam_n_items, tr.ctl, lr, beta1, beta2, eps, weight_decay, s));
    RET_IF(launch_add_f32(h->b_t2, h->b_ext, h->b_t2a, h->D, s));
    h->prepared.valid = false;
    h->kvrec.valid = false;
    return 0;
}

static int opt_slot(gtav_dit* h, const char* name, int64_t numel, Slot** out) {
    GTAV_REQUIRE(h && name && h->tr.on, "opt_state: training is not enabled");
    auto it = h->wt.slots.find(name);
    GTAV_REQUIRE(it != h->wt.slots.end() && it->second.trainable && it->second.am && it->second.av, "opt_state: '%s' is not a trainable parameter", name);
    GTAV_REQUIRE(numel == (int64_t)it->second.R * it->second.C, "opt_state: '%s' has %d x %d elements, got %lld", name, it->second.R, it->second.C, (long long)numel);
    *out = &it->second;
    return 0;
}
int gtav_dit_get_opt_state(gtav_dit* h, const char* name, float* m_dst, float* v_dst, int64_t numel, void* stream) {
    Slot* sl = nullptr;
    RET_IF(opt_slot(h, name, numel, &sl));
    GTAV_REQUIRE(m_dst && v_dst, "get_opt_state: null destination");
    GTAV_CHECK_HIP(hipMemcpyAsync(m_dst, sl->am, (size_t)numel * sizeof(float), hipMemcpyDeviceToDevice, (hipStream_t)stream));
    GTAV_CHECK_HIP(hipMemcpyAsync(v_dst, sl->av, (size_t)numel * sizeof(float), hipMemcpyDeviceToDevice, (hipStream_t)stream));
    return 0;
}
int gtav_dit_set_opt_state(gtav_dit* h, const char* name, const float* m_src, const float* v_src, int64_t numel, void* stream) {
    Slot* sl = nullptr;
    RET_IF(opt_slot(h, name, numel, &sl));
    GTAV_REQUIRE(m_src && v_src, "set_opt_state: null source");
    GTAV_CHECK_HIP(hipMemcpyAsync(sl->am, m_src, (size_t)numel * sizeof(float), hipMemcpyDeviceToDevice, (hipStream_t)stream));
    GTAV_CHECK_HIP(hipMemcpyAsync(sl->av, v_src, (size_t)numel * sizeof(float), hipMemcpyDeviceToDevice, (hipStream_t)stream));
    return 0;
}
int gtav_dit_get_opt_step(gtav_dit* h, int64_t* applied_steps, int64_t* skipped_steps, void* stream) {
    GTAV_REQUIRE(h && h->tr.on && applied_steps && skipped_steps, "get_opt_step: bad argument");
    float c[8];
    GTAV_CHECK_HIP(hipMemcpyAsync(c, h->tr.ctl, sizeof(c), hipMemcpyDeviceToHost, (hipStream_t)stream));
    GTAV_CHECK_HIP(hipStreamSynchronize((hipStream_t)stream));
    *applied_steps = (int64_t)c[4];
    *skipped_steps = (int64_t)c[2];
    return 0;
}
int gtav_dit_set_opt_step(gtav_dit* h, int64_t applied_steps, int64_t skipped_steps, void* stream) {
    GTAV_REQUIRE(h && h->tr.on && applied_steps >= 0 && applied_steps < (1 << 24) && skipped_steps >= 0, "set_opt_step: bad argument (the step count is kept as an exact fp32 integer: < 2^24)");
    float c[8];
    GTAV_CHECK_HIP(hipMemcpyAsync(c, h->tr.ctl, sizeof(c), hipMemcpyDeviceToHost, (hipStream_t)stream));
    GTAV_CHECK_HIP(hipStreamSynchronize((hipStream_t)stream));
    c[4] = (float)applied_steps; c[2] = (float)skipped_steps;
    GTAV_CHECK_HIP(hipMemcpy(h->tr.ctl, c, sizeof(c), hipMemcpyHostToDevice));
    return 0;
}
int gtav_dit_train_stats(gtav_dit* h, float* out4_host, void* stream) {
    GTAV_REQUIRE(h && out4_host && h->tr.on, "train_stats: bad argument");
    GTAV_CHECK_HIP(hipMemcpyAsync(out4_host, h->tr.ctl, 4 * sizeof(float), hipMemcpyDeviceToHost, (hipStream_t)stream));
    GTAV_CHECK_HIP(hipStreamSynchronize((hipStream_t)stream));
    return 0;
}

}
```

### ai-generated-gtav_amd/csrc/common.h

```cpp
#pragma once
#include <hip/hip_runtime.h>
#include <hip/hip_fp16.h>
#include <hip/hip_ext.h>
#include <stdint.h>

#ifdef GTAV_BF16_OPERANDS
#define GTAV_F16_T __bf16
#else
#define GTAV_F16_T _Float16
#endif

namespace gtav {

typedef GTAV_F16_T f16;
typedef GTAV_F16_T f16x4 __attribute__((ext_vector_type(4)));
typedef GTAV_F16_T f16x8 __attribute__((ext_vector_type(8)));
typedef GTAV_F16_T f16x2 __attribute__((ext_vector_type(2)));
typedef float f32x4 __attribute__((ext_vector_type(4)));
typedef float f32x16 __attribute__((ext_vector_type(16)));

__device__ __forceinline__ f32x4 mfma16(f16x8 a, f16x8 b, f32x4 c, int, int, int) {
#ifdef GTAV_BF16_OPERANDS
    return __builtin_amdgcn_mfma_f32_16x16x32_bf16(a, b, c, 0, 0, 0);
#else
    return __builtin_amdgcn_mfma_f32_16x16x32_f16(a, b, c, 0, 0, 0);
#endif
}
typedef short i16x4_ __attribute__((ext_vector_type(4)));
__device__ __forceinline__ f32x4 mfma16k16(f16x4 a, f16x4 b, f32x4 c) {
#ifdef GTAV_BF16_OPERANDS
    return __builtin_amdgcn_mfma_f32_16x16x16bf16_1k(__builtin_bit_cast(i16x4_, a), __builtin_bit_cast(i16x4_, b), c, 0, 0, 0);
#else
    return __builtin_amdgcn_mfma_f32_16x16x16f16(a, b, c, 0, 0, 0);
#endif
}
__device__ __forceinline__ float dot2acc(f16x2 a, f16x2 b, float c, bool) {
#ifdef GTAV_BF16_OPERANDS
    return __builtin_amdgcn_fdot2_f32_bf16(a, b, c, false);
#else
    return __builtin_amdgcn_fdot2(a, b, c, false);
#endif
}

constexpr int WAVE = 64;

}
namespace gtav_shared {
extern thread_local hipEvent_t g_launch_ev[2];
void set_error(const char* fmt, ...);
const char* last_error();
}
namespace gtav {
using gtav_shared::g_launch_ev;
using gtav_shared::set_error;
using gtav_shared::last_error;
#define GTAV_LAUNCH(kern, grid, block, shmem, stream, ...)                                                              \
    do {                                                                                                                \
        if (gtav_shared::g_launch_ev[0]) {                                                                                     \
            hipExtLaunchKernelGGL(kern, grid, block, shmem, stream, gtav_shared::g_launch_ev[0], gtav_shared::g_launch_ev[1], 0, __VA_ARGS__); \
            gtav_shared::g_launch_ev[0] = nullptr;                                                                             \
        } else {                                                                                                        \
            hipLaunchKernelGGL(kern, grid, block, shmem, stream, __VA_ARGS__);                                          \
        }                                                                                                               \
    } while (0)

#define GTAV_CHECK_HIP(expr)                                                              \
    do {                                                                                  \
        hipError_t _e = (expr);                                                           \
        if (_e != hipSuccess) {                                                           \
            gtav::set_error("%s failed: %s (%s:%d)", #expr, hipGetErrorString(_e), __FILE__, __LINE__); \
            return 1;                                                                     \
        }                                                                                 \
    } while (0)

#define GTAV_REQUIRE(cond, ...)                                                           \
    do {                                                                                  \
        if (!(cond)) {                                                                    \
            gtav::set_error(__VA_ARGS__);                                                 \
            return 2;                                                                     \
        }                                                                                 \
    } while (0)

#ifdef GTAV_EXPERIMENTS
#define GTAV_ENV_INT(name, dflt) (getenv(name) ? atoi(getenv(name)) : (dflt))
#define GTAV_DBG(p, bits) ((p).debug & (bits))
#else
#define GTAV_ENV_INT(name, dflt) (dflt)
#define GTAV_DBG(p, bits) false
#endif

static inline int cdiv(int a, int b) { return (a + b - 1) / b; }
static inline int round_up(int a, int b) { return cdiv(a, b) * b; }

__host__ __device__ __forceinline__ size_t tiled_off(int r, int k, int K) {
    return ((size_t)(r >> 7) * (size_t)(K >> 6) + (size_t)(k >> 6)) * 8192 + (size_t)((r & 127) * 64) +
           (size_t)(((((k >> 3) & 7) ^ (r & 7)) << 3) + (k & 7));
}

}
namespace gtav_shared {
struct PrefetchDesc {
    const void* next;
    int rt, nkt, splitk;
    int kt_limit;
};
}
namespace gtav {
using gtav_shared::PrefetchDesc;
__device__ __forceinline__ void l2_prefetch_slice(const PrefetchDesc& d, int xcd, int j, int nb, int t, int nt, unsigned& sink) {
    const int sk = d.splitk;
    int ks0, ksn, rt0, rtn;
    if (sk >= 8) {
        ksn = sk >> 3; ks0 = xcd * ksn; rt0 = 0; rtn = d.rt;
    } else {
        const int per = 8 / sk, part = xcd % per;
        ks0 = xcd / per; ksn = 1;
        rt0 = part * d.rt / per; rtn = (part + 1) * d.rt / per - rt0;
    }
    const int kpt = d.nkt / sk;
    const int lim = d.kt_limit > 0 && d.kt_limit < kpt ? d.kt_limit : kpt;
    const int per_rt = ksn * lim;
    const int lines = rtn * per_rt * 128;
    const int l0 = (int)((long long)lines * j / nb), l1 = (int)((long long)lines * (j + 1) / nb);
    for (int l = l0 + t; l < l1; l += nt) {
        const int tile = l >> 7, r = tile / per_rt, rem = tile - r * per_rt, sl = rem / lim, k = rem - sl * lim;
        const char* a = (const char*)d.next + ((size_t)(rt0 + r) * d.nkt + (size_t)(ks0 + sl) * kpt + k) * 16384 + (l & 127) * 128;
        asm volatile("global_load_dword %0, %1, off" : "+v"(sink) : "v"(a) : "memory");
    }
}
static inline bool prefetch_desc_ok(const PrefetchDesc& d) {
    return !d.next || (d.rt > 0 && d.nkt > 0 && d.splitk >= 1 && d.nkt % d.splitk == 0 && (d.splitk >= 8 ? d.splitk % 8 == 0 : 8 % d.splitk == 0));
}

#ifdef GTAV_BF16_OPERANDS
constexpr float F16_MAX = 3.3895313892515355e38f;
#else
constexpr float F16_MAX = 65504.0f;
#endif
constexpr int ERR_TIMESTEP = 1, ERR_F16_SAT = 2, ERR_NONFINITE = 4;
__device__ __forceinline__ f16x4 sat4(float a, float b, float c, float d, float& amax) {
    amax = __builtin_fmaxf(__builtin_fmaxf(__builtin_fabsf(a), __builtin_fabsf(b)), amax);
    amax = __builtin_fmaxf(__builtin_fmaxf(__builtin_fabsf(c), __builtin_fabsf(d)), amax);
    return f16x4{(f16)__builtin_amdgcn_fmed3f(a, -F16_MAX, F16_MAX), (f16)__builtin_amdgcn_fmed3f(b, -F16_MAX, F16_MAX),
                 (f16)__builtin_amdgcn_fmed3f(c, -F16_MAX, F16_MAX), (f16)__builtin_amdgcn_fmed3f(d, -F16_MAX, F16_MAX)};
}
__device__ __forceinline__ void sat_report(float amax, int* err_flag) {
    if (err_flag && amax > F16_MAX) atomicOr(err_flag, ERR_F16_SAT);
}

__device__ __forceinline__ float group8_sum(float v) {
    v += __builtin_bit_cast(float, __builtin_amdgcn_update_dpp(0, __builtin_bit_cast(int, v), 0xB1, 0xF, 0xF, true));
    v += __builtin_bit_cast(float, __builtin_amdgcn_update_dpp(0, __builtin_bit_cast(int, v), 0x4E, 0xF, 0xF, true));
    v += __builtin_bit_cast(float, __builtin_amdgcn_update_dpp(0, __builtin_bit_cast(int, v), 0x141, 0xF, 0xF, true));
    return v;
}

__device__ __forceinline__ float silu_f(float x) { return x / (1.0f + __expf(-x)); }

__device__ __forceinline__ float gelu_tanh_f(float x) {
    const float a = -2.0f * 1.4426950408889634f * 0.7978845608028654f, b = a * 0.044715f;
    const float e = __builtin_amdgcn_exp2f(x * __builtin_fmaf(x * x, b, a));
    return x * __builtin_amdgcn_rcpf(1.0f + e);
}

typedef float f32x2_ __attribute__((ext_vector_type(2)));
__device__ __forceinline__ void gelu_tanh_f4(const float (&x)[4], float (&y)[4]) {
    const float a = -2.0f * 1.4426950408889634f * 0.7978845608028654f, b = a * 0.044715f;
#pragma unroll
    for (int h = 0; h < 2; ++h) {
        const f32x2_ v = f32x2_{x[2 * h], x[2 * h + 1]};
        const f32x2_ t = __builtin_elementwise_fma(v * v, f32x2_{b, b}, f32x2_{a, a});
        const f32x2_ arg = v * t;
        const f32x2_ e = f32x2_{__builtin_amdgcn_exp2f(arg[0]), __builtin_amdgcn_exp2f(arg[1])};
        const f32x2_ d = e + f32x2_{1.0f, 1.0f};
        const f32x2_ r = f32x2_{__builtin_amdgcn_rcpf(d[0]), __builtin_amdgcn_rcpf(d[1])};
        const f32x2_ o = v * r;
        y[2 * h] = o[0];
        y[2 * h + 1] = o[1];
    }
}

__device__ __forceinline__ f32x2_ gelu_tanh_grad_f2(f32x2_ v) {
    const float k = 0.7978845608028654f, c = 0.044715f;
    const float a = -2.0f * 1.4426950408889634f * k, b = a * c, k2 = 2.0f * k, k6 = 6.0f * k * c;
    const f32x2_ z = v * v;
    const f32x2_ arg = v * __builtin_elementwise_fma(z, f32x2_{b, b}, f32x2_{a, a});
    const f32x2_ d = f32x2_{__builtin_amdgcn_exp2f(arg[0]), __builtin_amdgcn_exp2f(arg[1])} + f32x2_{1.0f, 1.0f};
    const f32x2_ s = f32x2_{__builtin_amdgcn_rcpf(d[0]), __builtin_amdgcn_rcpf(d[1])};
    const f32x2_ t = (v * s) * __builtin_elementwise_fma(z, f32x2_{k6, k6}, f32x2_{k2, k2});
    return __builtin_elementwise_fma(t, f32x2_{1.0f, 1.0f} - s, s);
}
// ... 79 lines not shown
```

### ai-generated-gtav_amd/csrc/elementwise.hip

```cpp
#include "ops.h"

#include <cstdlib>
#include <type_traits>

#include <cstring>

namespace gtav {

namespace {

template <int MODE, int NV>
__global__ __launch_bounds__(256) void ln_wave_row_kernel(const float* __restrict__ x, int ldx, f16* __restrict__ out, int M, int D,
                                                          const float* __restrict__ p0, const float* __restrict__ p1, int mod_stride,
                                                          const int* __restrict__ rows, int rows_per_mod, int flags, int* err_flag) {
    const int lane = threadIdx.x & 63;
    const int m = blockIdx.x * 4 + (threadIdx.x >> 6);
    if (m >= M) return;
    const float* xr = x + (size_t)m * ldx;
    f32x4 v[NV], av[NV], bv[NV];
#pragma unroll
    for (int i = 0; i < NV; ++i) v[i] = *(const f32x4*)(xr + i * 256 + lane * 4);
    const float *a, *b;
    if (MODE == 0) {
        int row = m / rows_per_mod;
// ... 293 lines not shown
        if (c >= (size_t)W2) return;
        *(f32x4*)(cur2 + (size_t)slot * W2 + c) = *(const f32x4*)(table2 + (size_t)rows[slot] * W2 + c);
    }
}

__global__ __launch_bounds__(256) void ctab_inputs_kernel(const float* __restrict__ mod, int MODW, int R, int Rp, int D, const int* __restrict__ col,
                                                          const int* __restrict__ is_scale, f16* __restrict__ sx, size_t group_stride) {
    const int g = blockIdx.y;
    const size_t idx = (size_t)blockIdx.x * 256 + threadIdx.x;
    const int per_row = D >> 3;
    const int r = (int)(idx / per_row), k = (int)(idx - (size_t)r * per_row) * 8;
    if (r >= Rp) return;
    union { f16x8 h; u32x4 u; } o;
    if (r < R) {
        const float* src = mod + (size_t)r * MODW + col[g] + k;
        const f32x4 a = *(const f32x4*)src, b = *(const f32x4*)(src + 4);
        const bool sc = is_scale[g] != 0;
        float v[8] = {a[0], a[1], a[2], a[3], b[0], b[1], b[2], b[3]};
#pragma unroll
        for (int e = 0; e < 8; ++e) {
            float x = sc ? 1.0f + (v[e] + 1e-6f) : v[e];
            x = __builtin_amdgcn_fmed3f(x, -F16_MAX, F16_MAX);
            o.h[e] = (f16)x;
        }
    } else {
#pragma unroll
        for (int e = 0; e < 8; ++e) o.h[e] = (f16)0.f;
    }
    *(u32x4*)(sx + (size_t)g * group_stride + tiled_off(r, k, D)) = o.u;
}

__global__ void cond_inputs_frame_kernel(int rows, int B, int T, int F, int start, int cur, int t_ctx, const int* __restrict__ t_steps,
                                         const float* __restrict__ sincos, float* __restrict__ E,
                                         const float* __restrict__ actions, int A, float* __restrict__ HC, int ldhc, int D,
                                         int Apad, int* err_flag) {
    const int r = blockIdx.x;
    if (r >= rows) return;
    const int nctx = B * (T - 1);
    int t, b, frame;
    if (r < nctx) {
        b = r / (T - 1);
        frame = start + (r - b * (T - 1));
        t = t_ctx;
    } else {
        const int q = r - nctx;
        const int sidx = q / B;
        b = q - sidx * B;
        frame = cur;
        t = t_steps[sidx];
    }
    if (t < 0 || t > 999) {
        if (threadIdx.x == 0 && err_flag) atomicOr(err_flag, 1);
        t = t < 0 ? 0 : 999;
    }
    for (int j = threadIdx.x; j < 256; j += blockDim.x) E[(size_t)r * 256 + j] = sincos[(size_t)t * 256 + j];
    const float* arow = actions ? actions + ((size_t)b * F + frame) * A : nullptr;
    for (int j = threadIdx.x; j < Apad; j += blockDim.x) HC[(size_t)r * ldhc + D + j] = (arow && j < A) ? arow[j] : 0.f;
}

__global__ void cond_inputs_kernel(const int64_t* __restrict__ t64, int rows, int Tq, const StepParams* __restrict__ sp, int use_cur,
                                   const float* __restrict__ sincos, float* __restrict__ E, const float* __restrict__ actions,
                                   long long act_outer, long long act_inner, int A, float* __restrict__ HC, int ldhc, int D,
                                   int Apad, int* err_flag) {
    const int r = blockIdx.x;
    if (r >= rows) return;
    const int ro = r / Tq, ri = r - ro * Tq;
    long long t;
    int frame0 = 0;
    if (t64) {
        t = (long long)t64[r];
    } else {
        t = ri == Tq - 1 ? sp->t_cur : sp->t_ctx;
        frame0 = use_cur ? sp->cur : sp->first;
    }
    if (t < 0 || t > 999) {
        if (threadIdx.x == 0 && err_flag) atomicOr(err_flag, 1);
        t = t < 0 ? 0 : 999;
    }
    for (int j = threadIdx.x; j < 256; j += blockDim.x) E[(size_t)r * 256 + j] = sincos[(size_t)t * 256 + j];
    const float* arow = actions ? actions + ro * act_outer + (frame0 + ri) * act_inner : nullptr;
    for (int j = threadIdx.x; j < Apad; j += blockDim.x) HC[(size_t)r * ldhc + D + j] = (arow && j < A) ? arow[j] : 0.f;
}

__device__ __forceinline__ float ddim_one(float xc, float vp, float at, float an, int is_final) {
    const float x0 = sqrtf(at) * xc - sqrtf(1.0f - at) * vp;
    if (is_final) return x0;
    const float eps = (sqrtf(1.0f / at) * xc - x0) / sqrtf(1.0f / at - 1.0f);
    return sqrtf(an) * x0 + sqrtf(1.0f - an) * eps;
}

__global__ void ddim_update_kernel(const float* __restrict__ x, size_t x_stride, const float* __restrict__ v, size_t v_stride,
                                   float* __restrict__ out, size_t out_stride, int n, const float* __restrict__ alpha_t,
                                   const float* __restrict__ alpha_next, int is_final) {
    const int b = blockIdx.y;
    const float at = alpha_t[b];
    const float an = alpha_next ? alpha_next[b] : 1.f;
    for (int i = blockIdx.x * blockDim.x + threadIdx.x; i < n; i += gridDim.x * blockDim.x)
        out[b * out_stride + i] = ddim_one(x[b * x_stride + i], v[b * v_stride + i], at, an, is_final);
}

__global__ void ddim_update_step_kernel(float* __restrict__ x, size_t frames_per_sample, const float* __restrict__ v,
                                        size_t v_stride, int n, const StepParams* __restrict__ sp) {
    const int b = blockIdx.y;
    const float at = sp->alpha_t, an = sp->alpha_next;
    const int fin = sp->is_final;
    float* xf = x + ((size_t)b * frames_per_sample + sp->cur) * n;
    for (int i = blockIdx.x * blockDim.x + threadIdx.x; i < n; i += gridDim.x * blockDim.x)
        xf[i] = ddim_one(xf[i], v[b * v_stride + i], at, an, fin);
}

__global__ void add_noise_kernel(const float* __restrict__ x, const float* __restrict__ noise, const float* __restrict__ alpha,
                                 float* __restrict__ out, int n, float clamp_abs) {
    const int r = blockIdx.y;
    const float a = alpha[r];
    const float sa = sqrtf(a), s1 = sqrtf(1.0f - a);
    for (int i = blockIdx.x * blockDim.x + threadIdx.x; i < n; i += gridDim.x * blockDim.x) {
        const size_t o = (size_t)r * n + i;
        const float z = fminf(fmaxf(noise[o], -clamp_abs), clamp_abs);
        out[o] = x[o] * sa + s1 * z;
    }
}

__global__ void vtarget_kernel(const float* __restrict__ x, const float* __restrict__ noise, const float* __restrict__ alpha,
                               float* __restrict__ vt, int n, float clamp_abs) {
    const int r = blockIdx.y;
    const float a = alpha[r];
    const float sa = sqrtf(a), s1 = sqrtf(1.0f - a);
    for (int i = blockIdx.x * blockDim.x + threadIdx.x; i < n; i += gridDim.x * blockDim.x) {
        const size_t o = (size_t)r * n + i;
        const float z = fminf(fmaxf(noise[o], -clamp_abs), clamp_abs);
        vt[o] = sa * z - s1 * x[o];
    }
}

__global__ __launch_bounds__(256) void mse_partial_kernel(const float* __restrict__ a, size_t a_stride, const float* __restrict__ b,
                                                          size_t b_stride, int n, float* __restrict__ partial) {
    __shared__ float red[4];
    const int r = blockIdx.x;
    float s = 0.f;
    for (int i = threadIdx.x; i < n; i += 256) {
        const float d = a[r * a_stride + i] - b[r * b_stride + i];
        s += d * d;
    }
    s = wave_sum(s);
    if ((threadIdx.x & 63) == 0) red[threadIdx.x >> 6] = s;
    __syncthreads();
    if (threadIdx.x == 0) partial[r] = (red[0] + red[1]) + (red[2] + red[3]);
}
__global__ void mse_final_kernel(const float* partial, int rows, float inv_count, float* out) {
    if (threadIdx.x == 0 && blockIdx.x == 0) {
        float s = 0.f;
        for (int i = 0; i < rows; ++i) s += partial[i];
        *out = s * inv_count;
    }
}

__global__ void unpad_f16_kernel(const f16* __restrict__ src, int lds, int R, int C, float* __restrict__ dst, int tiled) {
    const size_t total = (size_t)R * C;
    for (size_t idx = (size_t)blockIdx.x * blockDim.x + threadIdx.x; idx < total; idx += (size_t)gridDim.x * blockDim.x) {
        const int c = (int)(idx % C);
        const size_t r = idx / C;
        dst[idx] = (float)src[tiled ? tiled_off((int)r, c, lds) : r * lds + c];
    }
}
__global__ void copy_rows_kernel(const float* __restrict__ src, size_t ss, float* __restrict__ dst, size_t ds, size_t n) {
    const int r = blockIdx.y;
    for (size_t i = (size_t)blockIdx.x * blockDim.x + threadIdx.x; i < n; i += (size_t)gridDim.x * blockDim.x)
        dst[r * ds + i] = src[r * ss + i];
}
__global__ void clamp_cols_kernel(float* buf, int M, int ld, int c0, int c1, float lo, float hi) {
    const int w = c1 - c0;
    const size_t total = (size_t)M * w;
    for (size_t idx = (size_t)blockIdx.x * blockDim.x + threadIdx.x; idx < total; idx += (size_t)gridDim.x * blockDim.x) {
// ... 375 lines not shown
```

### ai-generated-gtav_amd/csrc/gemm.hip

```cpp
#include "gemm.h"
#include "attn_tile.h"

#include <cstdlib>
#include <cstring>
#include <type_traits>
#include <hip/hip_ext.h>

namespace gtav {

namespace {

constexpr int TN = 128, TK = 64;
constexpr int TILE_BYTES = 128 * TK * 2;

typedef const __attribute__((address_space(1))) void* gptr_t;
typedef __attribute__((address_space(3))) void* lptr_t;

__device__ __forceinline__ void glds16(const char* src, char* lds_wave_base) {
    __builtin_amdgcn_global_load_lds((gptr_t)src, (lptr_t)lds_wave_base, 16, 0, 0);
}

__device__ __forceinline__ void glds16_s(const void* sbase, unsigned voff, unsigned lds_addr) {
    unsigned keep;
    asm volatile("s_mov_b32 %0, m0\n\ts_mov_b32 m0, %3\n\ts_nop 0\n\tglobal_load_lds_dwordx4 %1, %2\n\ts_mov_b32 m0, %0"
// ... 849 lines not shown
                    if constexpr (FOLD) {
                        const float* cf = (const float*)ft.cb + fold_frame_of(ft, m0 + 16 * FJ * wm + 16 * j) * 2 * TNB + nl;
                        v = fold_apply(acc[i][j], ft.mu[j], ft.rs[j], *(const f32x4*)cf, *(const f32x4*)(cf + TNB));
                    } else {
                        v = acc[i][j] + bv;
                    }
                    if (rope) {
                        f32x4 cs;
                        if constexpr (PRE) cs = prope[i][j];
                        else cs = *(const f32x4*)(rope_tab(p, n) + pos[j] * 64 + d);
                        v = rope4(v, cs);
                    }
                    char* dst = smem + ml * PN + (((nl >> 3) ^ (ml & 7)) << 4) + ((nl >> 2) & 1) * 8;
                    *(uint2*)dst = pack4(amax, v[0], v[1], v[2], v[3]);
                }
            }
        }
    }
    sat_report(amax, p.err_flag);
    __syncthreads();
    const int heads = p.D >> 6;
    if (tr) {
        constexpr int CPR = TM / 8;
        for (int q = threadIdx.x; q < TNB * CPR; q += (int)blockDim.x) {
            const int nl = q / CPR, tc = q % CPR;
            const int n = n0 + nl;
            const int2 t = tab[tc * 8];
            if (n >= p.N || t.x < 0) continue;
            const uint4 val = *(const uint4*)(smem + nl * PT + ((tc ^ (nl & 7)) << 4));
            const int nn = n - 2 * p.D;
            f16* dst = p.v + ((size_t)(t.x * heads + (nn >> 6)) * 64 + (nn & 63)) * p.S + t.y;
            if (p.out_sc1) store16q_sc1(dst, val);
            else *(uint4*)dst = val;
        }
    } else {
        constexpr int CPR = TNB / 8;
        for (int q = threadIdx.x; q < TM * CPR; q += (int)blockDim.x) {
            const int ml = q / CPR, c = q % CPR;
            const int n = n0 + 8 * c;
            const int2 t = tab[ml];
            if (n >= p.N || t.x < 0) continue;
            const uint4 val = *(const uint4*)(smem + ml * PN + ((c ^ (ml & 7)) << 4));
            const int which = n >= 2 * p.D ? 2 : (n >= p.D ? 1 : 0);
            const int nn = n - which * p.D;
            f16* dst;
            if (spatial) dst = (which == 0 ? p.q : p.k) + ((size_t)(t.x * heads + (nn >> 6)) * p.S + t.y) * 64 + (nn & 63);
            else if (which == 0) dst = p.q + (size_t)(m0 + ml) * p.D + nn;
            else dst = p.k + (size_t)t.x * 2 * p.D + (which == 2 ? p.D : 0) + nn;
            if (p.out_sc1) store16q_sc1(dst, val);
            else *(uint4*)dst = val;
        }
    }
}

template <int EPIX, int FI, int WM, int WN = 2, int WOFF = 0>
__device__ __forceinline__ void prefetch_bias(const GemmParams& p, int n0, f32x4 (&pbias)[FI]) {
    constexpr int EPI = epi_base(EPIX);
    const int w = (int)(threadIdx.x >> 6) - WOFF;
    const int lane = threadIdx.x & 63, wn = w % WN, g = lane >> 4;
#pragma unroll
    for (int i = 0; i < FI; ++i) {
        const int n = n0 + 16 * FI * wn + 16 * i + 4 * g;
        pbias[i] = f32x4{0.f, 0.f, 0.f, 0.f};
        if (EPI != EPI_PARTIAL && p.bias && n < p.N && w >= 0 && w < WN * WM) pbias[i] = *(const f32x4*)(p.bias + n);
    }
}

template <int FI, int FJ, int WM, int WN = 2, int WOFF = 0>
__device__ __forceinline__ void prefetch_resid(const GemmParams& p, int n0, int m0, f32x4 (&xpre)[FI][FJ], int qlo, int qhi) {
    const int lane = threadIdx.x & 63, w = (int)(threadIdx.x >> 6) - WOFF;
    const int wn = w % WN, wm = w / WN, li = lane & 15, g = lane >> 4;
    const bool cw = w >= 0 && w < WN * WM;
#pragma unroll
    for (int i = 0; i < FI; ++i) {
        const int n = n0 + 16 * FI * wn + 16 * i + 4 * g;
#pragma unroll
        for (int j = 0; j < FJ; ++j) {
            const int q = i * FJ + j;
            if (q < qlo || q >= qhi) continue;
            const int m = m0 + 16 * FJ * wm + 16 * j + li;
            xpre[i][j] = f32x4{0.f, 0.f, 0.f, 0.f};
            if (cw && n < p.N && m < p.M) xpre[i][j] = *(const f32x4*)((const float*)p.out + (size_t)m * p.ldo + n);
        }
    }
}

template <int EPIX, int FI, int FJ, int WM, int WN = 2, int WOFF = 0, bool PRE = false>
__device__ __forceinline__ void epilogue(const GemmParams& p, f32x4 (&acc)[FI][FJ], const f32x4 (&pbias)[FI], char* smem, int n0, int m0, int ks, bool tr,
                                         const f32x4 (&prope)[FI][FJ], FoldTok<FJ>& ft) {
    constexpr int EPI = epi_base(EPIX);
    constexpr bool FOLD = epi_is_fold_consumer(EPIX);
    constexpr int TM = WM * 16 * FJ, TNB = 16 * FI * WN;
    constexpr int CT = 16 * FI * WN / 64;
    const int lane = threadIdx.x & 63, wraw = threadIdx.x >> 6, w = wraw - WOFF;
    const int wn = w % WN, wm = w / WN, li = lane & 15, g = lane >> 4;
    const bool compute_wave = w >= 0 && w < WN * WM;
    float amax = 0.f;

    if constexpr (EPI == EPI_RESID_FOLD) {
        static_assert(EPI != EPI_RESID_FOLD || (FI == 2 || FI == 4), "a 64-feature statistics slot is one wave (FI = 4) or two (FI = 2)");
        constexpr int WPS = 4 / FI;
        float2* sc = (float2*)(smem + CT * TM * 128);
        __syncthreads();
        if (compute_wave) {
            int rowA, rowB, boundary;
            fold_frames(p, __builtin_amdgcn_readfirstlane(m0 + 16 * FJ * wm), rowA, rowB, boundary);
            const float *gA = p.gate + (size_t)rowA * p.gate_stride, *gB = p.gate + (size_t)rowB * p.gate_stride;
            const float *sA = p.f_scale + (size_t)rowA * p.gate_stride, *sB = p.f_scale + (size_t)rowB * p.gate_stride;
            float s1[FJ], s2[FJ];
#pragma unroll
            for (int j = 0; j < FJ; ++j) s1[j] = 0.f, s2[j] = 0.f;
#pragma unroll
            for (int i = 0; i < FI; ++i) {
                const int nl = 16 * FI * wn + 16 * i + 4 * g;
                const int n = n0 + nl;
                const bool nok = n < p.N;
                const int nc = nok ? n : 0;
                const f32x4 bv = pbias[i];
                f32x4 gA4, gB4, sA4, sB4;
                if (GTAV_DBG(p, 0x100000)) {
                    gA4 = gB4 = f32x4{0.5f, 0.5f, 0.5f, 0.5f}; sA4 = sB4 = f32x4{0.1f, 0.1f, 0.1f, 0.1f};
                } else {
                    gA4 = *(const f32x4*)(gA + nc); gB4 = *(const f32x4*)(gB + nc);
                    sA4 = *(const f32x4*)(sA + nc); sB4 = *(const f32x4*)(sB + nc);
                }
                const int c = nl & 63;
#pragma unroll
                for (int j = 0; j < FJ; ++j) {
                    const int ml = 16 * FJ * wm + 16 * j + li;
                    const int m = m0 + ml;
                    f32x4 a = f32x4{0.f, 0.f, 0.f, 0.f};
                    if (nok && m < p.M) {
                        float* dst = (float*)p.out + (size_t)m * p.ldo + n;
                        const bool inA = m0 + 16 * FJ * wm + 16 * j < boundary;
                        const f32x4 gt = inA ? gA4 : gB4, sc4 = inA ? sA4 : sB4;
                        f32x4 x;
                        if constexpr (PRE) x = prope[i][j];
                        else x = *(const f32x4*)dst;
                        x = x + gt * (acc[i][j] + bv);
                        if (!GTAV_DBG(p, 0x10000)) {
                            if (p.out_sc1 && !GTAV_DBG(p, 0x80000)) store16_sc1(dst, x);
                            else *(f32x4*)dst = x;
                        }
                        s1[j] += (x[0] + x[1]) + (x[2] + x[3]);
                        s2[j] += (x[0] * x[0] + x[1] * x[1]) + (x[2] * x[2] + x[3] * x[3]);
#pragma unroll
                        for (int e = 0; e < 4; ++e) a[e] = x[e] * (1.0f + (sc4[e] + 1e-6f));
                    }
                    char* ld = smem + ((nl >> 6) * TM + ml) * 128 + (((c >> 3) ^ (ml & 7)) << 4) + (c & 7) * 2;
                    *(uint2*)ld = pack4(amax, a[0], a[1], a[2], a[3]);
                }
            }
#pragma unroll
            for (int j = 0; j < FJ; ++j) {
                float t1 = s1[j], t2 = s2[j];
                t1 += __shfl_xor(t1, 16, 64); t2 += __shfl_xor(t2, 16, 64);
                t1 += __shfl_xor(t1, 32, 64); t2 += __shfl_xor(t2, 32, 64);
                if (g == 0) sc[wn * TM + 16 * FJ * wm + 16 * j + li] = float2{t1, t2};
            }
        }
        sat_report(amax, p.err_flag);
        __syncthreads();
        {
            const int nslot = p.N >> 6;
            for (int q = threadIdx.x; q < TM * (TNB / 64); q += (int)blockDim.x) {
                const int sl = q / TM, tok = q - sl * TM;
// ... 155 lines not shown
                tok_pos[j] = tok_b[j];
            } else {
                const int fr = m / p.S;
                const int b = fr / p.Tq;
                const int tfr = p.t0 + (fr - b * p.Tq);
                tok_a[j] = (b * p.Tmax + tfr) * p.S + (m - fr * p.S);
                tok_b[j] = 0;
                tok_pos[j] = tfr;
            }
        }
    }
    if constexpr (EPI == EPI_RESID && !FOLD) {
        int grow[FJ];
#pragma unroll
        for (int j = 0; j < FJ; ++j) {
            int mm = m0 + 16 * FJ * wm + 16 * j + li;
            mm = mm < p.M ? mm : p.M - 1;
            grow[j] = 0;
            if (p.gate) {
                grow[j] = mm / p.rows_per_gate;
                if (p.gate_rows) grow[j] = p.gate_rows[grow[j]];
            }
        }
        f32x4 xo[2][FJ], gt[2][FJ];
        auto loads = [&](int i, f32x4 (&xv)[FJ], f32x4 (&gv)[FJ]) {
            const int n = n0 + 16 * FI * wn + 16 * i + 4 * g;
#pragma unroll
            for (int j = 0; j < FJ; ++j) {
                const int m = m0 + 16 * FJ * wm + 16 * j + li;
                xv[j] = f32x4{0.f, 0.f, 0.f, 0.f};
                gv[j] = f32x4{1.f, 1.f, 1.f, 1.f};
                if (n < p.N && m < p.M) {
                    xv[j] = *(const f32x4*)((const float*)p.out + (size_t)m * p.ldo + n);
                    if (p.gate) gv[j] = *(const f32x4*)(p.gate + (size_t)grow[j] * p.gate_stride + n);
                }
            }
        };
        loads(0, xo[0], gt[0]);
#pragma unroll
        for (int i = 0; i < FI; ++i) {
            if (i + 1 < FI) loads(i + 1, xo[(i + 1) & 1], gt[(i + 1) & 1]);
            const int n = n0 + 16 * FI * wn + 16 * i + 4 * g;
#pragma unroll
            for (int j = 0; j < FJ; ++j) {
                const int m = m0 + 16 * FJ * wm + 16 * j + li;
                if (n < p.N && m < p.M) {
                    const f32x4 x = xo[i & 1][j] + gt[i & 1][j] * (acc[i][j] + pbias[i]);
                    float* dst = (float*)p.out + (size_t)m * p.ldo + n;
                    if (p.out_sc1) store16_sc1(dst, x);
                    else *(f32x4*)dst = x;
                }
            }
        }
        return;
    }
#pragma unroll
    for (int i = 0; i < FI; ++i) {
        const int n = n0 + 16 * FI * wn + 16 * i + 4 * g;
        if (n >= p.N) continue;
        const f32x4 bv = pbias[i];
        int which = 0, nn = n, head = 0, d = 0;
        if constexpr (EPI == EPI_QKV) {
            which = n >= 2 * p.D ? 2 : (n >= p.D ? 1 : 0);
            nn = n - which * p.D;
            head = nn >> 6;
            d = nn & 63;
        }
#pragma unroll
        for (int j = 0; j < FJ; ++j) {
            const int m = m0 + 16 * FJ * wm + 16 * j + li;
            if (m >= p.M) continue;
            f32x4 v;
            if constexpr (FOLD) {
                const float* cf = (const float*)ft.cb + fold_frame_of(ft, m0 + 16 * FJ * wm + 16 * j) * 2 * TNB + (n - n0);
                v = fold_apply(acc[i][j], ft.mu[j], ft.rs[j], *(const f32x4*)cf, *(const f32x4*)(cf + TNB));
            } else {
                v = acc[i][j] + bv;
            }
            if constexpr (EPI == EPI_PARTIAL) {
                float* dst = (float*)p.out + ((size_t)ks * p.M + m) * p.ldo + n;
                if (p.out_sc1) store16_sc1(dst, v);
                else *(f32x4*)dst = v;
            } else if constexpr (EPI == EPI_F32) {
                *(f32x4*)((float*)p.out + (size_t)m * p.ldo + n) = v;
            } else if constexpr (EPI == EPI_F16) {
                *(uint2*)((f16*)p.out + (size_t)m * p.ldo + n) = pack4(amax, v[0], v[1], v[2], v[3]);
            } else if constexpr (EPI == EPI_QKV) {
                if (which < 2) {
                    const f32x4 cs = *(const f32x4*)(rope_tab(p, n) + tok_pos[j] * 64 + d);
                    v = rope4(v, cs);
                }
                const uint2 pk = pack4(amax, v[0], v[1], v[2], v[3]);
                if (p.qkv_mode == QKV_SPATIAL) {
                    const int heads = p.D >> 6;
                    f16* base = which == 0 ? p.q : p.k;
                    f16* dst = base + ((size_t)(tok_a[j] * heads + head) * p.S + tok_b[j]) * 64 + d;
                    *(uint2*)dst = pk;
                } else {
                    if (which == 0) {
                        *(uint2*)(p.q + (size_t)m * p.D + nn) = pk;
                    } else {
                        f16* base = p.k + (size_t)tok_a[j] * 2 * p.D + (which == 2 ? p.D : 0);
                        *(uint2*)(base + nn) = pk;
                    }
                }
            }
        }
    }
    if constexpr (EPI == EPI_F16 || EPI == EPI_QKV) sat_report(amax, p.err_flag);
}

template <int EPIX, int FI, int FJ, int WM, int WN = 2, int WOFF = 0>
__device__ __forceinline__ void epilogue(const GemmParams& p, f32x4 (&acc)[FI][FJ], const f32x4 (&pbias)[FI], char* smem, int n0, int m0, int ks, bool tr) {
    static_assert(!epi_is_fold_consumer(EPIX), "a fold consumer passes its prefetched FoldTok");
    FoldTok<FJ> ft;
    epilogue<EPIX, FI, FJ, WM, WN, WOFF, false>(p, acc, pbias, smem, n0, m0, ks, tr, acc, ft);
}

template <int EPIX, int NS, int WM, int FJ>
__global__ __launch_bounds__(128 * WM, (WM == 2 && NS <= 2) ? 2 : (WM == 4 ? 2 : 1)) void gemm_kernel(GemmParams p) {
    constexpr int EPI = epi_base(EPIX);
    constexpr int TM = WM * 16 * FJ;
    __shared__ __attribute__((aligned(16))) char smem[NS * (1 + TM / 128) * TILE_BYTES];
    static_assert(NS * (1 + TM / 128) * TILE_BYTES >= TM * 256 + TM * 8 + fold_lds_bytes(TN), "the ring must cover the epilogue's LDS image");
    BlockStamps bs;
    bs.begin(p);
    int n0, m0, ks, kt0, nkt;
    tile_map<EPI == EPI_PARTIAL, TN, TM>(p, n0, m0, ks, kt0, nkt);

    f32x4 acc[4][FJ];
#pragma unroll
    for (int i = 0; i < 4; ++i)
#pragma unroll
        for (int j = 0; j < FJ; ++j) acc[i][j] = f32x4{0.f, 0.f, 0.f, 0.f};

    bool tr = false;
    if constexpr (EPI == EPI_QKV) tr = (p.qkv_mode == QKV_SPATIAL) && (n0 >= 2 * p.D);
    f32x4 pbias[4];
    constexpr bool FOLDC = epi_is_fold_consumer(EPIX), FOLDP = EPI == EPI_RESID_FOLD, PREX = FOLDP && NS >= 3;
    FoldTok<FJ> ft;
    f32x4 xpre[PREX ? 4 : 1][PREX ? FJ : 1];
    auto pf = [&]() {
        prefetch_bias<EPI, 4, WM>(p, n0, pbias);
        if constexpr (FOLDC) fold_prefetch<TN, TM, FJ>(p, n0, m0, (int)threadIdx.x, __builtin_amdgcn_readfirstlane(m0 + 16 * FJ * (int)(threadIdx.x >> 7)), true, ft);
    };
    if constexpr (EPI == EPI_QKV) {
        if (tr) mainloop<true, NS, WM, FJ>(p, smem, n0, m0, kt0, nkt, acc, bs, pf);
        else mainloop<false, NS, WM, FJ>(p, smem, n0, m0, kt0, nkt, acc, bs, pf);
    } else if constexpr (PREX) {
        mainloop<false, NS, WM, FJ>(p, smem, n0, m0, kt0, nkt, acc, bs, pf, [&](int t) { prefetch_resid<4, FJ, WM>(p, n0, m0, xpre, t, t + 1); });
        prefetch_resid<4, FJ, WM>(p, n0, m0, xpre, nkt, 4 * FJ);
    } else {
        mainloop<false, NS, WM, FJ>(p, smem, n0, m0, kt0, nkt, acc, bs, pf);
    }
    GTAV_STAMP(bs.t[2]);
    if constexpr (PREX) epilogue<EPIX, 4, FJ, WM, 2, 0, true>(p, acc, pbias, smem, n0, m0, ks, tr, xpre, ft);
    else if constexpr (FOLDC || FOLDP) epilogue<EPIX, 4, FJ, WM, 2, 0, false>(p, acc, pbias, smem, n0, m0, ks, tr, acc, ft);
    else epilogue<EPIX, 4, FJ, WM>(p, acc, pbias, smem, n0, m0, ks, tr);
    bs.end(p);
}

typedef unsigned u32x2_ __attribute__((ext_vector_type(2)));
__device__ __forceinline__ void lds_read_tr_asm(u32x2_& dst, unsigned lds_addr) {
    asm volatile("ds_read_b64_tr_b16 %0, %1" : "=v"(dst) : "v"(lds_addr));
}
union TnFrag { f16x8 h; u32x2_ u[2]; };
template <int NS>
// ... 1520 lines not shown
    return 0;
}

bool gemm_dw_grouped_ok(const GemmDwGroup* g, int n, int K) {
    if (!g || n < 1 || n > GEMM_DW_MAX_GROUPS || K <= 0 || K % TK) return false;
    int tiles = 0;
    for (int i = 0; i < n; ++i) {
        if (g[i].M <= 0 || g[i].N <= 0 || g[i].M % 256 || g[i].N % 256 || g[i].ldo < g[i].N || g[i].ldo % 4) return false;
        tiles += (g[i].M >> 8) * (g[i].N >> 8);
    }
    int dev = 0;
    const int cus = device_cus(&dev);
    return cus > 0 && 2 * tiles >= cus && tiles <= 2 * cus && K >= 2048;
}

int launch_gemm_dw_grouped(const GemmDwGroup* g, int n, int K, int* err_flag, hipStream_t stream, bool tn) {
    GTAV_REQUIRE(g && n >= 1 && n <= GEMM_DW_MAX_GROUPS && K > 0 && K % TK == 0, "gemm_dw_grouped: bad arguments (n=%d K=%d)", n, K);
    GemmDwGroups gs;
    memset(&gs, 0, sizeof(gs));
    gs.n = n;
    for (int i = 0; i < n; ++i) {
        GTAV_REQUIRE(g[i].X && g[i].W && g[i].out && g[i].M > 0 && g[i].N > 0 && g[i].M % 256 == 0 && g[i].N % 256 == 0 && g[i].ldo >= g[i].N && g[i].ldo % 4 == 0,
                     "gemm_dw_grouped: group %d: M=%d, N=%d must be multiples of 256, ldo=%d >= N", i, g[i].M, g[i].N, g[i].ldo);
        GTAV_REQUIRE(((uintptr_t)g[i].X & 15) == 0 && ((uintptr_t)g[i].W & 15) == 0 && ((uintptr_t)g[i].out & 15) == 0, "gemm_dw_grouped: group %d: operands must be 16-byte aligned", i);
        gs.g[i] = g[i];
        gs.first[i + 1] = gs.first[i] + (g[i].M >> 8) * (g[i].N >> 8);
    }
    for (int i = n + 1; i <= GEMM_DW_MAX_GROUPS; ++i) gs.first[i] = gs.first[n];
    GemmParams p;
    memset(&p, 0, sizeof(p));
    p.K = K; p.splitk = 1; p.err_flag = err_flag; p.rows_per_gate = 1;
#ifdef GTAV_EXPERIMENTS
    p.stamps = g_stamps;
#endif
    if (tn) {
        GTAV_REQUIRE(K % 128 == 0, "gemm_dw_grouped: the transpose-free form contracts over whole 128-token row tiles (K=%d)", K);
        GTAV_LAUNCH(gemm256_dw_grouped_kernel<true>, dim3(gs.first[n]), dim3(512), 0, stream, p, gs);
    } else {
        GTAV_LAUNCH(gemm256_dw_grouped_kernel<false>, dim3(gs.first[n]), dim3(512), 0, stream, p, gs);
    }
    GTAV_CHECK_HIP(hipGetLastError());
    return 0;
}

int launch_gemm_grouped(const GemmGroup* groups_dev, int n_groups, int max_N, int M, int K, hipStream_t stream) {
    GTAV_REQUIRE(groups_dev && n_groups > 0 && n_groups < 65536 && M > 0 && max_N > 0 && K > 0 && K % TK == 0, "gemm_grouped: bad arguments");
    GemmParams p;
    memset(&p, 0, sizeof(p));
    p.M = M; p.N = max_N; p.K = K; p.splitk = 1;
    const dim3 grid(cdiv(M, 96) * cdiv(max_N, 128), n_groups);
    hipLaunchKernelGGL((gemm_grouped_kernel<4, 4, 2, 3>), grid, dim3(384), 0, stream, p, groups_dev);
    GTAV_CHECK_HIP(hipGetLastError());
    return 0;
}


int launch_gemm(const GemmParams& p_in, int epi_x, hipStream_t stream) {
    GemmParams p = p_in;
    const int epi = epi_base(epi_x);
    const bool fold_c = epi_is_fold_consumer(epi_x), fold_p = epi_x == EPI_RESID_FOLD;
    if (fold_c || fold_p) {
        GTAV_REQUIRE(p.f_P > 0 && p.f_P % 16 == 0 && p.M % p.f_P == 0, "gemm/fold: %d tokens per frame must be a multiple of 16 and divide M=%d", p.f_P, p.M);
        if (fold_c) {
            GTAV_REQUIRE(p.f_stats && p.f_c1 && p.f_c2 && p.f_ldc >= p.N && p.f_nslot == p.K / 64 && p.f_nslot % 4 == 0,
                         "gemm/fold: consumer needs the row statistics (K/64 = %d slots, a multiple of 4) and the c1 / c2 tables", p.K / 64);
            GTAV_REQUIRE(!p.bias, "gemm/fold: the bias of a fold consumer lives in its c2 table");
            if (epi == EPI_QKV) GTAV_REQUIRE(p.qkv_mode == QKV_TEMPORAL || p.S % 16 == 0, "gemm/fold: spatial QKV needs S %% 16 == 0");
        } else {
            GTAV_REQUIRE(p.gate && p.f_scale && p.f_stats_out && p.f_a && p.N % 64 == 0 && p.ldo >= p.N,
                         "gemm/fold: producer needs gate, next scale, statistics and operand buffers, N %% 64 == 0");
        }
    }
    p.debug = g_debug & (3 | 16 | 32 | 2048 | 8192 | 16384 | 0x1F0000);
    p.stamps = nullptr;
#ifdef GTAV_EXPERIMENTS
    p.stamps = g_stamps;
#endif
    p.out_sc1 = (g_debug & 8) ? 0 : 1;
    GTAV_REQUIRE(prefetch_desc_ok(p.pf), "gemm: bad prefetch descriptor (row tiles %d, K tiles %d, K slices %d)", p.pf.rt, p.pf.nkt, p.pf.splitk);
    if (g_debug & 0x800000) p.pf.next = nullptr;
    GTAV_REQUIRE(p.K > 0 && p.K % TK == 0, "gemm: K=%d must be a positive multiple of %d", p.K, TK);
    GTAV_REQUIRE(p.M > 0 && p.N > 0 && p.N % 4 == 0, "gemm: bad M=%d N=%d", p.M, p.N);
    GTAV_REQUIRE(((uintptr_t)p.X & 15) == 0 && ((uintptr_t)p.W & 15) == 0, "gemm: operands must be 16-byte aligned");
    int splitk = 1;
    if (epi == EPI_QKV) {
        GTAV_REQUIRE(p.N == 3 * p.D && p.D % 128 == 0, "gemm/qkv: N=%d must equal 3*D, D=%d %% 128 == 0", p.N, p.D);
        GTAV_REQUIRE(p.S > 0 && p.q && p.k && p.rope_cs, "gemm/qkv: missing buffers");
        if (p.qkv_mode == QKV_SPATIAL) {
            GTAV_REQUIRE(p.S % 4 == 0 && p.M % p.S == 0 && p.v, "gemm/qkv spatial: S=%d must divide M=%d, S %% 4 == 0", p.S, p.M);
        } else {
            GTAV_REQUIRE(p.Tq > 0 && p.M % (p.S * p.Tq) == 0 && p.t0 + p.Tq <= p.Tmax, "gemm/qkv temporal: bad frame geometry");
        }
    } else {
        GTAV_REQUIRE(p.out && p.ldo >= p.N && p.ldo % 4 == 0, "gemm: bad output ldo=%d", p.ldo);
        if (epi == EPI_RESID && p.gate) GTAV_REQUIRE(p.rows_per_gate > 0, "gemm/resid: rows_per_gate");
        if (epi == EPI_GELU_TANH || epi == EPI_GELU_ERF || epi == EPI_F16_TILED) GTAV_REQUIRE(p.ldo % 64 == 0, "gemm/gelu: tile-major output needs ldo %% 64 == 0");
        if (fold_p) GTAV_REQUIRE(p.splitk <= 1, "gemm/fold: the producer epilogue needs the complete sum (no split-K)");
        if (epi == EPI_PARTIAL) {
            splitk = p.splitk;
            GTAV_REQUIRE(splitk >= 1 && (p.K / TK) % splitk == 0, "gemm/partial: splitk=%d must divide K/64=%d", splitk, p.K / TK);
        }
    }
    const int blocks128 = cdiv(p.M, 128) * cdiv(p.N, TN) * splitk;
    const bool foldish = fold_c || fold_p;
    int wm = g_force_wm ? g_force_wm : (blocks128 <= 256 ? 3 : 2);
    if (!g_force_wm && blocks128 <= 256) {
        auto cost = [&](int tn, int tm) { return cdiv(cdiv(p.M, tm) * cdiv(p.N, tn) * splitk, 256) * (tn + tm); };
        int best = cost(128, 128);
        if (cost(128, 96) < best) best = cost(128, 96), wm = 9;
        const bool ok96 = p.N % 96 == 0 && epi != EPI_GELU_TANH && epi != EPI_GELU_ERF && epi != EPI_F16_TILED && !(epi == EPI_QKV && p.qkv_mode == QKV_SPATIAL);
        if (ok96 && cost(96, 96) < best) best = cost(96, 96), wm = 8;
        if (cost(64, 96) < best) best = cost(64, 96), wm = 14;
        if (cost(64, 48) < best) best = cost(64, 48), wm = 11;
    }
    if (!g_force_wm && !(g_debug & 64) && (wm == 9 || (wm == 8 && g_l_for_8))) wm = (g_debug & 128) ? 25 : 20;
#ifdef GTAV_EXPERIMENTS
    if (!g_force_wm && wm == 20 && (g_debug & 0x1000000) && !foldish && (p.K / TK / (splitk > 0 ? splitk : 1)) % 4 == 0) wm = 22;
    if (!g_force_wm && wm == 20 && (g_debug & 0x2000000) && !foldish && (p.K / TK / (splitk > 0 ? splitk : 1)) % 8 == 0) wm = 18;
#endif
    if (!g_force_wm && !(g_debug & 64)) {
        if (wm == 11) wm = 24;
        else if (wm == 14 && !(epi_x == EPI_PARTIAL && splitk >= 8)) wm = 26;
    }
    bool frame_tile = false;
    if (!g_force_wm && !foldish && !(g_debug & 64)) {
        const int t29 = cdiv(p.M, 144) * cdiv(p.N, 128) * splitk, t20 = cdiv(p.M, 96) * cdiv(p.N, 128) * splitk;
        if (t29 > 128 && t29 <= 256 && t20 > 256 && blocks128 <= 320) wm = 29, frame_tile = true;
    }
    if (!g_force_wm && wm == 2 && cdiv(p.M, 192) * cdiv(p.N, 128) * splitk >= 320) {
        wm = 12;
    }
    bool narrow_pick = false;
    if (!g_force_wm && !frame_tile && blocks128 > 256 && p.N <= 2048 && epi != EPI_QKV) {
        const int t12 = cdiv(p.M, 192) * cdiv(p.N, 128) * splitk, t13 = cdiv(p.M, 96) * cdiv(p.N, 128) * splitk;
        if (t12 > 256 && t12 <= 512) wm = 12, narrow_pick = true;
        else if (t13 > 256 && t13 <= 512 && !fold_p) wm = 13, narrow_pick = true;
        else if (fold_p && t12 > 128) wm = 12, narrow_pick = true;
    }
    if (!g_force_wm && splitk == 1 && ((epi_x == EPI_PARTIAL && lp_takes(p.M, p.N, p.K)) || (epi_x == EPI_RESID && gemm_resid_inplace_ok(p.M, p.N, p.K, p.gate ? p.rows_per_gate : 0)))) wm = 31, narrow_pick = true;
    if (!g_force_wm && wm == 31 && epi_x == EPI_RESID && p.N % 256 == 0 && p.N <= 1024 && p.K >= 1024) {
        const int t256 = cdiv(p.M, 256) * (p.N / 256), rounds = cdiv(t256, 256);
        if (rounds >= 2 && t256 * 10 >= rounds * 256 * 9) wm = 7;
    }
#ifdef GTAV_EXPERIMENTS
    if (!g_force_wm && epi_x == EPI_GELU_TANH && (g_debug & 0x600000) && cdiv(p.M, 128) * cdiv(p.N, 256) >= 512) wm = (g_debug & 0x200000) ? 33 : 32;
#endif
    if (!g_force_wm && splitk == 1 && gemm_pp_ok(p.M, p.N, p.K, epi) && !(epi == EPI_QKV && p.qkv_mode == QKV_SPATIAL && p.S % 8 != 0)) wm = 16;
    GTAV_REQUIRE(!(wm == 8 && epi == EPI_QKV && p.qkv_mode == QKV_SPATIAL), "gemm: 96-feature tiles straddle the K / V boundary (spatial QKV)");
    if (!g_force_wm && splitk == 1 && epi != EPI_QKV && !foldish && !narrow_pick && p.N % 256 == 0 && p.N <= 1024 && p.K >= 1024) {
        const int t256 = cdiv(p.M, 256) * (p.N / 256), rounds = cdiv(t256, 256);
        if (t256 * 10 >= rounds * 256 * 7) wm = 7;
    }
    int ns = g_force_stages ? g_force_stages : ((wm == 12 || wm == 13) ? 2 : wm >= 8 ? 4 : wm == 3 ? 4 : 2);
    if (foldish) {
        const int span = wm == 2 ? 64 : (wm == 3 || wm == 14 || wm == 26) ? 32 : (wm == 11 || wm == 24) ? 16 : 48;
        GTAV_REQUIRE(p.f_P >= span, "gemm/fold: frames of %d tokens are shorter than the token span (%d) of a wave of block shape %d", p.f_P, span, wm);
    }
    switch (epi_x) {
#ifdef GTAV_EXPERIMENTS
        case EPI_RESID_FOLD: return launch_epi<EPI_RESID_FOLD>(p, ns, wm, splitk, stream);
        case EPI_QKV_FOLD: return launch_epi<EPI_QKV_FOLD>(p, ns, wm, splitk, stream);
        case EPI_GELU_TANH_FOLD: return launch_epi<EPI_GELU_TANH_FOLD>(p, ns, wm, splitk, stream);
        case EPI_F32_FOLD: return launch_epi<EPI_F32_FOLD>(p, ns, wm, splitk, stream);
#else
        case EPI_RESID_FOLD: case EPI_QKV_FOLD: case EPI_GELU_TANH_FOLD: case EPI_F32_FOLD:
            GTAV_REQUIRE(false, "gemm: the LayerNorm-fold epilogues exist only in the experiments build (csrc/build.sh exp)");
// ... 16 lines not shown
```

### ai-generated-gtav_amd/csrc/gemm_typed.inc

```
struct GemmParams {
    const f16* X;
    int ldx;
    const f16* W;
    int M, N, K;
    int debug;
    unsigned long long* stamps;
    int* err_flag;
    int out_sc1;
    int splitk;
    const float* bias;
    void* out2;
    void* out;
    int ldo;
    const float* gate;
    int gate_stride;
    const int* gate_rows;
    int rows_per_gate;
    int qkv_mode;
    f16* q;
    f16* k;
    f16* v;
    int D;
    int S;
    int Tq;
    int t0;
    int Tmax;
    const float* rope_cs;
    const float* rope_cs_q;
    struct TileMap { int tiles_m, tiles_n, gn, group, tiles; unsigned rcp_tiles, rcp_group, rcp_gn, rcp_gnlast; } tm;
    int f_P;
    const int* f_rows;
    const float* f_stats;
    int f_nslot;
    const float* f_c1;
    const float* f_c2;
    int f_ldc;
    float* f_stats_out;
    const float* f_scale;
    f16* f_a;
    PrefetchDesc pf;
    float* sk_ws;
    int* sk_flags;
    int sk_dp, sk_r;
};
static_assert(sizeof(GemmParams) == 352, "GemmParams: every build and both operand types must see the same struct");

struct GemmGroup { const f16* X; const f16* W; float* out; const float* bias; int N; int ldo; };
int launch_gemm_grouped(const GemmGroup* groups_dev, int n_groups, int max_N, int M, int K, hipStream_t stream);

constexpr int GEMM_DW_MAX_GROUPS = 4;
struct GemmDwGroup { const f16* X; const f16* W; float* out; int M; int N; int ldo; };
static_assert(sizeof(GemmDwGroup) == 40, "GemmDwGroup: every build and both operand types must see the same struct");
bool gemm_dw_grouped_ok(const GemmDwGroup* g, int n, int K);
int launch_gemm_dw_grouped(const GemmDwGroup* g, int n, int K, int* err_flag, hipStream_t stream, bool tn = false);

int launch_gemm(const GemmParams& p, int epi, hipStream_t stream);
bool gemm_qkvt_attn_ok(int M, int D, int S, int Tq, int t0);
int launch_gemm_qkvt_attn(const GemmParams& p, hipStream_t stream);
bool gemm_qkvs_attn_ok(int M, int D, int S);
int launch_gemm_qkvs_attn(const GemmParams& p, hipStream_t stream);
bool gemm_tn_ok(int M, int N, int K);
bool gemm_tn_pays(int M, int N, int K);
int launch_gemm_tn(const GemmParams& p, hipStream_t stream);
```

### ai-generated-gtav_amd/csrc/ops.h

```cpp
#pragma once
#include "common.h"
#include "gemm.h"

namespace gtav {

#include "ops_typed.inc"

int launch_skinny_f32(const float* X, int ldx, const float* W, const float* bias, float* Y, int ldy, int M, int N,
                      int K, int act_silu, hipStream_t stream);
int skinny_init();

struct StepParams {
    int first;
    int cur;
    int t_ctx;
    int t_cur;
    int is_final;
    float alpha_t, alpha_next;
    int cond_step;
};
int launch_step_setup(StepParams* dst, const StepParams& v, int* frame_idx, int* mod_rows, int* last_rows, int* changed, int B, int Tq, int T, int F,
                      int use_cur, hipStream_t stream);
int launch_gather_rows(const float* table, const int* rows, const int* changed, float* cur, int slots, int W, const float* table2, float* cur2, int W2,
                       hipStream_t stream);
int launch_cond_inputs_frame(int rows, int B, int T, int F, int start, int cur, int t_ctx, const int* t_steps, const float* sincos,
                             float* E, const float* actions, int A, float* HC, int ldhc, int D, int Apad, int* err_flag,
                             hipStream_t stream);

int launch_unpatchify(const float* y, int ldy, float* img, int NB, int C, int H, int W, int p, int order, float a,
                      float b, hipStream_t stream);

int launch_copy_f32_strided(const float* src, int lds, int R, int C, float* dst, int ldd, hipStream_t stream);
int launch_copy_rows_f32(const float* src, size_t src_stride, float* dst, size_t dst_stride, int rows, size_t n, hipStream_t stream);
int launch_clamp_cols(float* buf, int M, int ld, int c0, int c1, float lo, float hi, hipStream_t stream);
int launch_frames_to_u8(const float* img, uint8_t* out, int N, int H, int W, hipStream_t stream);
int launch_moments_to_latents(const float* mom, float* lat, int N, int hw, int latent, int mom_ch, float scale, hipStream_t stream);
int launch_latents_to_tokens(const float* lat, float* z, int N, int hw, int latent, hipStream_t stream);
int launch_resize_aa(const void* src, int src_is_u8_strip, float* dst, int n, int H, int W, int OH, int OW, hipStream_t stream);
int launch_copy_f32(const float* src, int lds, int R, int C, float* dst, int ldd, int c0, hipStream_t stream);
int launch_fill_f32(float* dst, size_t n, float v, hipStream_t stream);
int launch_rope_interleave(const float* cos_t, const float* sin_t, float* cs, int npos, hipStream_t stream);
int launch_add_f32(const float* a, const float* b, float* out, size_t n, hipStream_t stream);
int launch_calib_spin(unsigned long long ticks, unsigned long long* dev_ticks, hipStream_t stream);
int launch_axpy_f32(float* y, const float* x, float alpha, size_t n, hipStream_t stream);

int launch_cond_inputs(const int64_t* t64, int rows, int Tq, const StepParams* sp, int use_cur, const float* sincos ,
                       float* E, const float* actions, int64_t act_outer, int64_t act_inner, int A, float* HC, int ldhc,
                       int D, int Apad, int* err_flag, hipStream_t stream);

int launch_ddim_update(const float* x, size_t x_stride, const float* v, size_t v_stride, float* out, size_t out_stride,
                       int B, int n, const float* alpha_t, const float* alpha_next, int is_final, hipStream_t stream);
int launch_ddim_update_step(float* x, size_t frames_per_sample, const float* v, size_t v_stride, int B, int n,
                            const StepParams* sp, hipStream_t stream);

int launch_add_noise(const float* x, const float* noise, const float* alpha , float* out, int rows, int n,
                     float clamp_abs, hipStream_t stream);
int launch_vtarget(const float* x, const float* noise, const float* alpha , float* vt, int rows, int n,
                   float clamp_abs, hipStream_t stream);
int launch_mse(const float* a, size_t a_stride, const float* b, size_t b_stride, int rows, int n, float* out_scalar,
               hipStream_t stream);

int launch_ln_mod_bwd(const float* dxn, const float* x, const float* scale, int mod_stride, int rows_per_mod, int M, int D, float* dres, int accumulate,
                      float* stats, hipStream_t stream);
int launch_frame_reduce_ln(const float* dxn, const float* x, const float* stats, int frames, int P, int D, float* dshift, float* dscale, int mod_stride,
                           hipStream_t stream);
int gelu_bwd_colsum_splits(int M);
int launch_colsum_reduce_multi(const float* const* ws, float* const* db, const int* splits, const int* N, int njobs, hipStream_t stream);
bool ln_bwd_fused_ok(int D);
size_t ln_bwd_fused_workspace(int frames, int P, int D);
int launch_ln_mod_bwd_fused(const float* dxn, const float* x, const float* scale, int mod_stride, int frames, int P, int D, float* dres, int accumulate,
                            float* dshift, float* dscale, float* part, hipStream_t stream);
size_t colsum_workspace(int M, int N);
int launch_colsum_f32(const float* a, int lda, int M, int N, float* db, float* ws, hipStream_t stream);
int launch_silu(const float* x, int ldx, float* y, int ldy, int R, int C, hipStream_t stream);
int launch_silu_bwd(const float* dy, int lddy, const float* x, int ldx, float* dx, int lddx, int R, int C, hipStream_t stream);
int launch_gemm_tn_f32(const float* dY, int lddy, const float* X, int ldx, int R, int N, int K, float* dW, int lddw, hipStream_t stream);
int launch_gemm_nn_f32(const float* dY, int lddy, const float* W, int ldw, int R, int N, int K, float* dX, int lddx, hipStream_t stream);
size_t ada_bwd_dx_workspace(int MODW, int D, int R);
int launch_ada_bwd_dx(const float* dmod, int MODW, const float* W, int D, int R, float* dSc, float* part, hipStream_t stream);
int sumsq_parts(size_t n);
int launch_sumsq(const float* g, size_t n, float* part, hipStream_t stream);
int launch_overflow_publish(const int* err_flag, float* g, hipStream_t stream);
int launch_err_clear(int* err_flag, int bits, hipStream_t stream);
int launch_clip_coef(float* ctl, const float* part, int nparts, float inv_scale, float max_norm, float beta1, float beta2, int* err_flag, hipStream_t stream);
int launch_adamw(float* p, int ldp, int R, int C, const float* g, float* m, float* v, const float* ctl, float lr, float beta1, float beta2, float eps,
                 float wd, hipStream_t stream);

bool attn_spatial_wants_prescaled_q(int S);
constexpr float kAttnQScale = 0.125f * 1.4426950408889634f;

}
```

### ai-generated-gtav_amd/csrc/ops_bf16.h

```cpp
#pragma once
#include "ops.h"

namespace gtav_bf16 {
typedef __bf16 f16;
using gtav_shared::PrefetchDesc;
#include "gemm_typed.inc"
#include "ops_typed.inc"
}

namespace gtav {

#define GTAV_OPERAND_OPS(F)                                 \
    F(gemm, launch_gemm)                                    \
    F(ln_modulate, launch_ln_modulate)                      \
    F(ln_affine, launch_ln_affine)                          \
    F(patchify, launch_patchify)                            \
    F(convert_pad, launch_convert_pad_f16)                  \
    F(unpad, launch_unpad_f16_to_f32)                       \
    F(attn_spatial, launch_attn_spatial)                    \
    F(attn_temporal, launch_attn_temporal)                  \
                     \
    F(gemm_tn, launch_gemm_tn)                              \
    F(gemm_dw_grouped, launch_gemm_dw_grouped)              \
    F(transpose_tiled, launch_transpose_tiled_f16)          \
    F(convert_T, launch_convert_T_f16)                      \
    F(gelu_tiled, launch_gelu_tiled)                        \
    F(gelu_bwd_tiled, launch_gelu_bwd_tiled)                \
    F(gelu_bwd_tiled_colsum, launch_gelu_bwd_tiled_colsum)  \
    F(gate_bwd, launch_gate_bwd)                            \
    F(frame_reduce_gate, launch_frame_reduce_gate)          \
    F(gate_bwd_fused, launch_gate_bwd_fused)                \
    F(colsum_tiled, launch_colsum_tiled_f16)                \
    F(to_tiled, launch_to_tiled_f16)                        \
    F(mse_bwd_patch, launch_mse_bwd_patch)                  \
    F(attn_spatial_bwd, launch_attn_spatial_bwd)            \
    F(attn_temporal_bwd, launch_attn_temporal_bwd)          \
    F(adamw_multi, launch_adamw_multi)

struct OperandOps {
#define GTAV_OPS_FIELD(field, launcher) decltype(&launcher) field;
    GTAV_OPERAND_OPS(GTAV_OPS_FIELD)
#undef GTAV_OPS_FIELD
    bool bf16;
};
const OperandOps& operand_ops(bool bf16);

}
```

### ai-generated-gtav_amd/lib.py

```python
from __future__ import annotations

import ctypes as C
import os
import subprocess

_HERE = os.path.dirname(os.path.abspath(__file__))
LIB_PATH = os.path.join(_HERE, "libgtav_amd.so")
HEADER_PATH = os.path.join(os.path.dirname(_HERE), "include", "gtav_amd.h")


class GtavError(RuntimeError):
    pass


class GtavRangeSwitch(GtavError):

    def __init__(self, msg, groups=()):
        super().__init__(msg)
        self.groups = list(groups)


def build(force: bool = False) -> str:
    src_dir = os.path.join(_HERE, "csrc")
    srcs = [os.path.join(src_dir, f) for f in os.listdir(src_dir)] + [HEADER_PATH]
    if not force and os.path.exists(LIB_PATH):
        if os.path.getmtime(LIB_PATH) >= max(os.path.getmtime(s) for s in srcs):
            return LIB_PATH
    subprocess.run(["bash", os.path.join(src_dir, "build.sh")], check=True)
    return LIB_PATH


class DitConfig(C.Structure):
    _fields_ = [(n, C.c_int32) for n in ("input_h", "input_w", "patch_size", "in_channels", "hidden_size", "depth", "num_heads")] + [
        ("mlp_ratio", C.c_float), ("external_cond_dim", C.c_int32), ("max_frames", C.c_int32), ("max_batch", C.c_int32),
        ("max_cond_rows", C.c_int32)]


class VaeConfig(C.Structure):
    _fields_ = [(n, C.c_int32) for n in ("latent_dim", "input_height", "input_width", "patch_size", "enc_dim", "enc_depth",
                                          "enc_heads", "dec_dim", "dec_depth", "dec_heads")] + [
        ("mlp_ratio", C.c_float), ("use_variational", C.c_int32), ("max_frames_per_call", C.c_int32)]


_p, _i, _f, _l = C.c_void_p, C.c_int32, C.c_float, C.c_int64

SIGNATURES = {
    "gtav_last_error": [],
    "gtav_abi_version": [],
    "gtav_dit_create": [C.POINTER(DitConfig), C.POINTER(_p)],
    "gtav_dit_destroy": [_p],
    "gtav_dit_set_weight": [_p, C.c_char_p, _p, _l, _p],
    "gtav_dit_finalize": [_p, _p],
    "gtav_dit_get_weight": [_p, C.c_char_p, _p, _l, _p],
    "gtav_dit_forward": [_p, _p, _p, _p, _p, _i, _i, _p],
    "gtav_dit_set_schedule": [_p, C.POINTER(C.c_float), _i],
    "gtav_dit_denoise_step": [_p, _p, _i, _i, _i, _i, _i, _i, _i, _i, _p, _i, _i, _p, _p],
    "gtav_dit_prepare_frame": [_p, _i, _i, _i, _i, _i, C.POINTER(C.c_int32), _i, _p, _p],
    "gtav_dit_check": [_p, _p],
    "gtav_dit_operand_groups": [_p, C.POINTER(C.c_int32)],
    "gtav_dit_set_operand_dtype": [_p, _i, _i],
    "gtav_dit_get_operand_dtype": [_p, _i, C.POINTER(C.c_int32)],
    "gtav_dit_autorange": [_p, C.POINTER(C.c_int32), _p],
    "gtav_dit_train_param_count": [_p, C.POINTER(C.c_int64)],
    "gtav_dit_train_enable": [_p, _p, _l],
    "gtav_dit_train_enable_typed": [_p, _p, _l, _i],
    "gtav_dit_set_loss_scale": [_p, _f],
    "gtav_dit_set_grad_divisor": [_p, _f],
    "gtav_dit_zero_grad": [_p, _p],
    "gtav_dit_train_forward": [_p, _p, _p, _p, _p, _i, _i, _p],
    "gtav_dit_train_backward": [_p, _p, _p, _p],
    "gtav_dit_train_backward_phases": [_p, _p, _p, _i, _i, _p],
    "gtav_dit_train_param_range": [_p, C.c_char_p, C.POINTER(C.c_int64), C.POINTER(C.c_int64)],
    "gtav_dit_get_grad": [_p, C.c_char_p, _p, _l, _p],
    "gtav_dit_train_get_residual": [_p, _i, _p, _l, _p],
    "gtav_dit_adamw_step": [_p, _f, _f, _f, _f, _f, _f, _p],
    "gtav_dit_train_stats": [_p, C.POINTER(C.c_float), _p],
    "gtav_dit_get_opt_state": [_p, C.c_char_p, _p, _p, _l, _p],
    "gtav_dit_set_opt_state": [_p, C.c_char_p, _p, _p, _l, _p],
    "gtav_dit_get_opt_step": [_p, C.POINTER(C.c_int64), C.POINTER(C.c_int64), _p],
    "gtav_dit_set_opt_step": [_p, _l, _l, _p],
    "gtav_dit_set_graph": [_p, _i],
    "gtav_dit_set_fused_temporal": [_p, _i],
    "gtav_dit_set_fused_spatial": [_p, _i],
    "gtav_dit_fused_launches": [_p, _i, _i, _i],
    "gtav_dit_set_weight_prefetch": [_p, _i],
    "gtav_dit_profile": [_p, _i],
    "gtav_dit_profile_read": [_p, C.POINTER(C.c_double), C.POINTER(C.c_int64)],
    "gtav_timer_calibrate": [_i, _i, C.POINTER(C.c_double), C.POINTER(C.c_double), _p],
    "gtav_comm_unique_id": [_p],
    "gtav_comm_init": [C.POINTER(_p), _i, _i, _p],
    "gtav_comm_allreduce_f32": [_p, _p, _l, _i, _p],
    "gtav_comm_allgather": [_p, _p, _p, _l, _p],
    "gtav_comm_destroy": [_p],
    "gtav_vae_create": [C.POINTER(VaeConfig), C.POINTER(_p)],
    "gtav_vae_destroy": [_p],
    "gtav_vae_set_weight": [_p, C.c_char_p, _p, _l, _p],
    "gtav_vae_finalize": [_p, _p],
    "gtav_vae_get_weight": [_p, C.c_char_p, _p, _l, _p],
    "gtav_vae_encode": [_p, _p, _f, _f, _p, _i, _p],
    "gtav_vae_decode": [_p, _p, _f, _p, _f, _f, _i, _p],
    "gtav_vae_check": [_p, _p],
    "gtav_vae_set_operand_dtype": [_p, _i],
    "gtav_vae_get_operand_dtype": [_p, C.POINTER(C.c_int32)],
    "gtav_vae_profile": [_p, _i],
    "gtav_vae_profile_read": [_p, C.POINTER(C.c_double), C.POINTER(C.c_int64)],
    "gtav_clamp_frames": [_p, _i, _i, _i, _i, _f, _f, _p],
    "gtav_ddim_update": [_p, _p, _p, _i, _i, _p, _p, _i, _p],
    "gtav_add_noise": [_p, _p, _p, _p, _i, _i, _f, _p],
    "gtav_vtarget": [_p, _p, _p, _p, _i, _i, _f, _p],
    "gtav_mse": [_p, _l, _p, _l, _i, _i, _p, _p],
    "gtav_axpy_f32": [_p, _p, _f, _l, _p],
    "gtav_frames_to_u8": [_p, _p, _i, _i, _i, _p],
    "gtav_moments_to_latents": [_p, _p, _i, _i, _i, _i, _f, _p],
    "gtav_latents_to_tokens": [_p, _p, _i, _i, _i, _p],
    "gtav_strip_to_frames": [_p, _i, _i, _i, _p, _i, _i, _p],
    "gtav_resize_frames": [_p, _p, _i, _i, _i, _i, _i, _p],
    "gtav_op_gemm_f16": [_p, _i, _p, _p, _p, _i, _i, _i, _i, _i, _p, _i, _i, _p],
    "gtav_op_gemm_qkv": [_p, _i, _p, _p, _i, _i, _i, _p, _p, _p, _i, _i, _i, _i, _p, _p],
    "gtav_op_rope_interleave": [_p, _p, _p, _i, _p],
    "gtav_op_skinny_f32": [_p, _i, _p, _p, _p, _i, _i, _i, _i, _i, _p],
    "gtav_op_ln_modulate": [_p, _p, _i, _i, _p, _p, _i, _i, _p],
    "gtav_op_ln_affine": [_p, _p, _i, _i, _p, _p, _p],
    "gtav_op_attn_spatial": [_p, _p, _p, _p, _i, _i, _i, _p],
    "gtav_op_attn_temporal": [_p, _p, _p, _i, _i, _i, _i, _i, _i, _p],
    "gtav_op_attn_temporal_bf16": [_p, _p, _p, _i, _i, _i, _i, _i, _i, _p],
    "gtav_op_qkv_head_major": [_p, _p, _i, _p],
    "gtav_op_gemm_tn": [_p, _p, _i, _i, _i, _p, _i, _p],
    "gtav_op_gemm_dw_grouped": [_i, _p, _p, _p, _p, _p, _p, _i, _p],
    "gtav_op_attn_spatial_bwd": [_p, _p, _p, _p, _i, _i, _i, _p, _p, _p],
    "gtav_op_attn_spatial_bwd_bf16": [_p, _p, _p, _p, _i, _i, _i, _p, _p, _p],
    "gtav_op_gemm_qkvt_attn": [_p, _p, _i, _i, _i, _i, _i, _i, _p, _p, _p, _p],
    "gtav_op_qkv_head_major_spatial": [_p, _p, _i, _p],
    "gtav_op_gemm_qkvs_attn": [_p, _p, _i, _i, _i, _p, _p, _p],
    "gtav_op_convert_f16": [_p, _i, _i, _i, _p, _i, _i, _i, _p],
    "gtav_op_gemm_splitk_ln": [_p, _i, _p, _p, _i, _i, _i, _i, _p, _p, _p, _i, _i, _p, _p, _p, _i, _p],
    "gtav_op_gemm_choose_splitk": [_i, _i, _i],
    "gtav_op_gemm_resid_inplace": [_i, _i, _i],
    "gtav_op_gemm_set_stages": [_i],
    "gtav_op_gemm_set_wm": [_i],
}
_RESTYPES = {"gtav_last_error": C.c_char_p, "gtav_dit_destroy": None, "gtav_vae_destroy": None, "gtav_op_gemm_set_stages": None,
             "gtav_op_gemm_set_wm": None}

_lib = None


def load() -> C.CDLL:
    global _lib
    if _lib is not None:
        return _lib
    if not os.path.exists(LIB_PATH):
        raise GtavError(f"{LIB_PATH} not found: run `python -c 'import __graft_entry__ as g; g.build()'` "
                        f"(hipcc --offload-arch=gfx950). gtav_amd has no CPU fallback.")
    import torch
    lib = C.CDLL(LIB_PATH)
    for name, argtypes in SIGNATURES.items():
        fn = getattr(lib, name)
        fn.argtypes = argtypes
        fn.restype = _RESTYPES.get(name, C.c_int)
    _lib = lib
    return lib


EXP_LIB_PATH = os.environ.get("GTAV_EXP_LIB") or os.path.join(_HERE, "libgtav_amd_exp.so")
EXP_SIGNATURES = {
    "gtav_dit_set_fold": [_p, _i, _i, _i],
# ... 45 lines not shown
```

### ai-generated-gtav_amd/model/dit.py

```python
from __future__ import annotations

import ctypes as C
import math
from collections import OrderedDict
from typing import Dict, Iterator, Optional

import torch

from .. import lib as _lib
from .. import weights as _w


def _rope_tables_axial(freqs: torch.Tensor, gh: int, gw: int):
    def ang(n):
        a = torch.linspace(-1, 1, steps=n)[:, None] * freqs[None, :]
        return a.repeat_interleave(2, dim=-1)
    ah, aw = ang(gh), ang(gw)
    a = torch.cat([ah[:, None, :].expand(gh, gw, -1), aw[None, :, :].expand(gh, gw, -1)], dim=-1).reshape(gh * gw, -1)
    cos, sin = torch.ones(gh * gw, 64), torch.zeros(gh * gw, 64)
    cos[:, : a.shape[1]] = a.cos()
    sin[:, : a.shape[1]] = a.sin()
    return cos.contiguous(), sin.contiguous()


# ... 135 lines not shown
        self._capacity_rows = 0
        hd = hidden_size // num_heads
        self._spatial_freqs = _w.rope_freqs_pixel(hd // 2, 256)
        self._temporal_freqs = _w.rope_freqs_lang(hd)
        self._schedule = None
        self.n_operand_groups = 2 * depth + 2
        self._bf16_groups = set(range(self.n_operand_groups)) if self._train_bf16 else set()
        self.range_policy = range_policy
        if range_policy not in ("report", "auto"):
            raise ValueError("range_policy must be 'report' (check() raises when an fp16 activation saturated) or 'auto' (check() moves the saturated "
                             "layers to bf16 operands and raises GtavRangeSwitch: recompute)")
        if init_weights:
            self.initialize_weights()

    @property
    def max_frames(self):
        return self._max_frames

    @max_frames.setter
    def max_frames(self, v):
        if int(v) > MAX_FRAMES:
            raise ValueError(f"max_frames={int(v)}: the temporal attention serves windows of at most {MAX_FRAMES} frames")
        self._max_frames = int(v)
        cap = min(int(v), TRAIN_MAX_FRAMES) if self._trainable else int(v)
        if cap > self._capacity_t:
            if self._handle and self._trainable and self._grads is not None:
                raise RuntimeError("a trainable DiT cannot grow its window after training was enabled: construct it with the largest max_frames")
            self._capacity_t = cap
            self._free()

    def _shapes(self):
        return _w.dit_param_shapes(**self._cfg_kwargs)

    def _extra_state(self):
        return {"spatial_rotary_emb.freqs": self._spatial_freqs, "temporal_rotary_emb.freqs": self._temporal_freqs}

    def _load_freqs(self, sf, tf):
        if sf is not None:
            self._spatial_freqs = sf.detach().float().cpu()
        if tf is not None:
            self._temporal_freqs = tf.detach().float().cpu()

    def initialize_weights(self):
        for k, shp in self._shapes().items():
            if k.endswith(".bias"):
                v = torch.zeros(shp)
            elif "adaLN_modulation" in k and k.startswith("blocks."):
                v = torch.zeros(shp)
            elif k.startswith("t_embedder.mlp") or k.startswith("final_layer.adaLN_modulation"):
                v = torch.randn(shp) * 0.01
            elif k == "final_layer.linear.weight":
                v = torch.randn(shp) * 0.001
            else:
                v = torch.randn(shp) * 0.02
            self._sd[k] = v
        self._dirty = True

    def _ensure(self, B: int, T: int, cond_rows: int = 0):
        if T > MAX_FRAMES:
            raise ValueError(f"a window of {T} frames: the temporal attention serves at most {MAX_FRAMES} (max_frames <= {MAX_FRAMES})")
        if self._trainable and T > TRAIN_MAX_FRAMES:
            raise ValueError(f"a window of {T} frames on a trainable DiT: the training step (backward temporal attention, adaLN-gradient reduction) is "
                             f"implemented for at most {TRAIN_MAX_FRAMES} frames; windows up to {MAX_FRAMES} need trainable=False")
        grow = (cond_rows > max(self._capacity_rows, self._capacity_b * self._capacity_t)) or T > self._capacity_t or B > self._capacity_b
        if grow and self._handle and self._trainable and self._grads is not None:
            raise RuntimeError(f"a trainable DiT cannot grow its workspace after training was enabled (batch {B} > {self._capacity_b}, window {T} > "
                               f"{self._capacity_t} or {cond_rows} conditioning rows > {max(self._capacity_rows, self._capacity_b * self._capacity_t)}): "
                               "size it with max_batch / max_frames / reserve() before the first step")
        if grow:
            self._capacity_rows = max(self._capacity_rows, cond_rows)
            self._capacity_t = max(self._capacity_t, T)
            self._capacity_b = max(self._capacity_b, B)
            self._free()
        if not self._handle:
            L = _lib.load()
            cfg = _lib.DitConfig(max_frames=self._capacity_t, max_batch=self._capacity_b,
                                 max_cond_rows=max(self._capacity_b * self._capacity_t, self._capacity_rows), **self._cfg_kwargs)
            with torch.cuda.device(self.device):
                _lib.check(L.gtav_dit_create(C.byref(cfg), C.byref(self._handle)))
                if getattr(self, "_fused_temporal", False):
                    _lib.check(L.gtav_dit_set_fused_temporal(self._handle, 1))
                if getattr(self, "_fused_spatial", None) is not None:
                    _lib.check(L.gtav_dit_set_fused_spatial(self._handle, int(self._fused_spatial)))
                if getattr(self, "_fold", None) is not None:
                    _lib.check(L.gtav_dit_set_fold(self._handle, *self._fold))
                if getattr(self, "_weight_prefetch", None) is not None:
                    _lib.check(L.gtav_dit_set_weight_prefetch(self._handle, int(self._weight_prefetch)))
                for g in sorted(self._bf16_groups):
                    _lib.check(L.gtav_dit_set_operand_dtype(self._handle, g, 1))
                if self._trainable:
                    n = C.c_int64(0)
                    _lib.check(L.gtav_dit_train_param_count(self._handle, C.byref(n)))
                    self._grads = torch.zeros(n.value, device=self.device, dtype=torch.float32)
                    if self._train_bf16:
                        _lib.check(L.gtav_dit_train_enable_typed(self._handle, self._grads.data_ptr(), n.value, 1))
                    else:
                        _lib.check(L.gtav_dit_train_enable(self._handle, self._grads.data_ptr(), n.value))
                    _lib.check(L.gtav_dit_set_loss_scale(self._handle, self._loss_scale))
                    if self.grad_divisor != 1.0:
                        _lib.check(L.gtav_dit_set_grad_divisor(self._handle, self.grad_divisor))
            self._dirty = True
        if self._dirty:
            gh, gw = self.input_h // self.patch_size, self.input_w // self.patch_size
            sc, ss = _rope_tables_axial(self._spatial_freqs, gh, gw)
            tc, ts = _rope_tables_temporal(self._temporal_freqs, self._capacity_t)
            extra = {"tables.timestep_sincos": _timestep_table(), "tables.rope_spatial_cos": sc, "tables.rope_spatial_sin": ss,
                     "tables.rope_temporal_cos": tc, "tables.rope_temporal_sin": ts}
            self._upload(extra)
            if self._schedule is not None:
                self.set_schedule(self._schedule)

    def reserve(self, max_batch: int, max_frames: Optional[int] = None, noise_steps: int = 0):
        T = max_frames or self._capacity_t
        self._ensure(max_batch, T, cond_rows=max_batch * (T - 1 + noise_steps + 1) if noise_steps else 0)

    def forward(self, x: torch.Tensor, t: torch.Tensor, external_cond: Optional[torch.Tensor] = None) -> torch.Tensor:
        B, T, Cc, H, W = x.shape
        assert H == self.input_h and W == self.input_w, (
            f"Input image size ({H}*{W}) doesn't match model ({self.input_h}*{self.input_w}).")
        self._ensure(B, T)
        dev = self.device
        xd = x.to(dev, torch.float32).contiguous()
        td = t.to(dev, torch.int64).contiguous()
        ad = external_cond.to(dev, torch.float32).contiguous() if torch.is_tensor(external_cond) else None
        out = torch.empty_like(xd)
        with torch.cuda.device(dev):
            _lib.check(_lib.load().gtav_dit_forward(self._handle, xd.data_ptr(), td.data_ptr(), _lib.ptr(ad), out.data_ptr(),
                                                    B, T, _lib.current_stream()))
        return out

    __call__ = forward

    def forward_train(self, x: torch.Tensor, t: torch.Tensor, external_cond: Optional[torch.Tensor] = None) -> torch.Tensor:
        assert self._trainable, "construct the model with trainable=True"
        B, T, Cc, H, W = x.shape
        assert H == self.input_h and W == self.input_w
        self._ensure(B, T)
        dev = self.device
        xd = x.to(dev, torch.float32).contiguous()
        td = t.to(dev, torch.int64).contiguous()
        ad = external_cond.to(dev, torch.float32).contiguous() if torch.is_tensor(external_cond) else None
        out = torch.empty_like(xd)
        with torch.cuda.device(dev):
            _lib.check(_lib.load().gtav_dit_train_forward(self._handle, xd.data_ptr(), td.data_ptr(), _lib.ptr(ad), out.data_ptr(), B, T,
                                                          _lib.current_stream()))
        return out

    def backward_(self, v_pred: torch.Tensor, v_target: torch.Tensor):
        vt = v_target.to(self.device, torch.float32).contiguous()
        with torch.cuda.device(self.device):
            _lib.check(_lib.load().gtav_dit_train_backward(self._handle, v_pred.data_ptr(), vt.data_ptr(), _lib.current_stream()))

    def backward_phases_(self, v_pred: torch.Tensor, v_target: torch.Tensor, phase_begin: int, phase_end: int):
        vt = v_target.to(self.device, torch.float32).contiguous()
        with torch.cuda.device(self.device):
            _lib.check(_lib.load().gtav_dit_train_backward_phases(self._handle, v_pred.data_ptr(), vt.data_ptr(), phase_begin, phase_end,
                                                                 _lib.current_stream()))

    def param_range(self, prefix: str):
        off, cnt = C.c_int64(0), C.c_int64(0)
        _lib.check(_lib.load().gtav_dit_train_param_range(self._handle, prefix.encode(), C.byref(off), C.byref(cnt)))
        return off.value, cnt.value

    def zero_grad(self):
        if not self._handle:
            self._ensure(self._capacity_b, self._capacity_t)
# ... 64 lines not shown
        L = _lib.load()
        with torch.cuda.device(self.device):
            for k, shp in self._shapes().items():
                m = state["m." + k].to(self.device, torch.float32).contiguous()
                v = state["v." + k].to(self.device, torch.float32).contiguous()
                if tuple(m.shape) != tuple(shp) or tuple(v.shape) != tuple(shp):
                    raise RuntimeError(f"load_opt_state_dict: {k} has shape {tuple(m.shape)}, expected {tuple(shp)}")
                _lib.check(L.gtav_dit_set_opt_state(self._handle, k.encode(), m.data_ptr(), v.data_ptr(), m.numel(), _lib.current_stream()))
            st = state["step"]
            _lib.check(L.gtav_dit_set_opt_step(self._handle, int(st[0]), int(st[1]), _lib.current_stream()))
            torch.cuda.synchronize()

    @property
    def grad_divisor(self) -> float:
        return getattr(self, "_grad_divisor", 1.0)

    @grad_divisor.setter
    def grad_divisor(self, v: float):
        self._grad_divisor = float(v)
        if self._handle:
            _lib.check(_lib.load().gtav_dit_set_grad_divisor(self._handle, self._grad_divisor))

    def pull_weights(self):
        L = _lib.load()
        with torch.cuda.device(self.device):
            for k, shp in self._shapes().items():
                out = torch.empty(shp, device=self.device, dtype=torch.float32)
                _lib.check(L.gtav_dit_get_weight(self._handle, k.encode(), out.data_ptr(), out.numel(), _lib.current_stream()))
                self._sd[k] = out.cpu()

    def set_schedule(self, alphas_cumprod: torch.Tensor):
        ac = alphas_cumprod.detach().reshape(-1).float().cpu().contiguous()
        assert ac.numel() == 1000
        self._schedule = ac
        if self._handle:
            arr = (C.c_float * 1000).from_buffer_copy(ac.numpy().tobytes())
            _lib.check(_lib.load().gtav_dit_set_schedule(self._handle, arr, 1000))

    def prepare_frame_(self, B: int, F: int, start: int, cur: int, t_ctx: int, t_steps, actions: Optional[torch.Tensor] = None):
        n = len(t_steps)
        self._ensure(B, cur - start + 1, cond_rows=B * (cur - start + n))
        arr = (C.c_int32 * n)(*[int(v) for v in t_steps])
        with torch.cuda.device(self.device):
            _lib.check(_lib.load().gtav_dit_prepare_frame(self._handle, B, F, start, cur, int(t_ctx), arr, n, _lib.ptr(actions),
                                                          _lib.current_stream()))

    def denoise_step_(self, x: torch.Tensor, start: int, cur: int, t_ctx: int, t_cur: int, t_next: int, is_final: bool,
                      actions: Optional[torch.Tensor] = None, cached: bool = False, v_out: Optional[torch.Tensor] = None,
                      cond_step: int = -1):
        assert x.is_cuda and x.dtype == torch.float32 and x.is_contiguous()
        B, F = x.shape[:2]
        if cond_step < 0:
            self._ensure(B, cur - start + 1)
        with torch.cuda.device(self.device):
            _lib.check(_lib.load().gtav_dit_denoise_step(
                self._handle, x.data_ptr(), B, F, start, cur, int(t_ctx), int(t_cur), int(t_next), int(bool(is_final)),
                _lib.ptr(actions), 1 if cached else 0, int(cond_step), _lib.ptr(v_out), _lib.current_stream()))

    PROFILE_CLASSES = ("ln_modulate", "gemm_qkv", "attn_spatial", "attn_temporal", "gemm_out", "gemm_fc1", "gemm_fc2", "other",
                       "empty_event_pair")

    def profile(self, enable: bool):
        _lib.check(_lib.load().gtav_dit_profile(self._handle, int(bool(enable))))

    def profile_read(self):
        ms = (C.c_double * 9)()
        n = (C.c_int64 * 9)()
        _lib.check(_lib.load().gtav_dit_profile_read(self._handle, ms, n))
        return {k: (ms[i], n[i]) for i, k in enumerate(self.PROFILE_CLASSES)}

    def set_graph(self, enable: bool):
        _lib.check(_lib.load().gtav_dit_set_graph(self._handle, int(bool(enable))))

    def set_fused_temporal(self, enable: bool):
        self._fused_temporal = bool(enable)
        if self._handle:
            _lib.check(_lib.load().gtav_dit_set_fused_temporal(self._handle, int(self._fused_temporal)))

    def set_fused_spatial(self, enable: bool):
        self._fused_spatial = bool(enable)
        if self._handle:
            _lib.check(_lib.load().gtav_dit_set_fused_spatial(self._handle, int(self._fused_spatial)))

    def fused_launches(self, B: int, T: int, t0: int = 0) -> int:
        self._ensure(B, T)
        return int(_lib.load().gtav_dit_fused_launches(self._handle, int(B), int(T), int(t0)))

    def set_weight_prefetch(self, mode):
        mode = int(mode)
        if mode not in (0, 1) and (mode >> 16) != 1:
            raise ValueError(f"set_weight_prefetch: mode {mode:#x} is neither 0, 1 nor a per-class word (gtav_amd.generate.prefetch_mode)")
        self._weight_prefetch = mode
        if self._handle:
            _lib.check(_lib.load().gtav_dit_set_weight_prefetch(self._handle, mode))

    def set_fold(self, mode: int, min_tokens_a: int = -1, min_tokens_b: int = -1):
        if not getattr(_lib.load(), "_gtav_experiments", False):
            raise _lib.GtavError("set_fold: the LayerNorm fold exists only in the experiments build (gtav_amd.lib.load_experiments())")
        self._fold = (int(mode), int(min_tokens_a), int(min_tokens_b))
        if self._handle:
            _lib.check(_lib.load().gtav_dit_set_fold(self._handle, *self._fold))

    def set_operand_dtype(self, dtype, groups=None):
        if dtype not in (torch.float16, torch.bfloat16):
            raise ValueError(f"set_operand_dtype: {dtype} (torch.float16 or torch.bfloat16)")
        if self._train_bf16 and dtype == torch.float16:
            raise _lib.GtavError("set_operand_dtype: a bf16-trainable DiT (train_dtype=torch.bfloat16) keeps bf16 operands in every layer group")
        if self._trainable and not self._train_bf16 and dtype == torch.bfloat16:
            raise _lib.GtavError("set_operand_dtype: a trainable DiT keeps fp16 operands (its backward pass and loss scaling are fp16)")
        gs = set(range(self.n_operand_groups)) if groups is None else {int(g) for g in groups}
        if any(g < 0 or g >= self.n_operand_groups for g in gs):
            raise ValueError(f"set_operand_dtype: groups {sorted(gs)} outside [0, {self.n_operand_groups})")
        new = (self._bf16_groups | gs) if dtype == torch.bfloat16 else (self._bf16_groups - gs)
        if new == self._bf16_groups:
            return
        if self._handle:
            L = _lib.load()
            for g in sorted(new ^ self._bf16_groups):
                _lib.check(L.gtav_dit_set_operand_dtype(self._handle, g, 1 if g in new else 0))
            self._dirty = True
        self._bf16_groups = new

    def operand_dtypes(self):
        return [torch.bfloat16 if g in self._bf16_groups else torch.float16 for g in range(self.n_operand_groups)]

    def check(self):
        if not self._handle:
            return
        L = _lib.load()
        with torch.cuda.device(self.device):
            if self.range_policy != "auto" or self._trainable:
                _lib.check(L.gtav_dit_check(self._handle, _lib.current_stream()))
                return
            n = C.c_int32(0)
            _lib.check(L.gtav_dit_autorange(self._handle, C.byref(n), _lib.current_stream()))
            if n.value:
                d = C.c_int32(0)
                new = set()
                for g in range(self.n_operand_groups):
                    _lib.check(L.gtav_dit_get_operand_dtype(self._handle, g, C.byref(d)))
                    if d.value == 1:
                        new.add(g)
                switched = sorted(new - self._bf16_groups)
                self._bf16_groups = new
                self._dirty = True
                raise _lib.GtavRangeSwitch(f"DiT: an activation exceeded the fp16 range (|x| > 65504) in operand group(s) {switched}; those layers now run "
                                           "on bf16 operands (the reference's own autocast type): results since the last check are clipped — recompute them", switched)


def DiT_S_2(**kwargs):
    return DiT(input_h=18, input_w=32, patch_size=2, hidden_size=1024, depth=16, num_heads=16, max_frames=5, **kwargs)


DiT_models = {"DiT-S/2": DiT_S_2}
```

### include/gtav_amd.h

```cpp
#ifndef GTAV_AMD_H
#define GTAV_AMD_H

#include <stdint.h>

#ifdef __cplusplus
extern "C" {
#endif

const char* gtav_last_error(void);
int gtav_abi_version(void);

typedef struct gtav_dit_config {
    int32_t input_h, input_w, patch_size, in_channels, hidden_size, depth, num_heads;
    float mlp_ratio;
    int32_t external_cond_dim, max_frames;
    int32_t max_batch;
    int32_t max_cond_rows;
} gtav_dit_config;

typedef struct gtav_dit gtav_dit;

int gtav_dit_create(const gtav_dit_config* cfg, gtav_dit** out);
void gtav_dit_destroy(gtav_dit* h);
int gtav_dit_set_weight(gtav_dit* h, const char* name, const float* src_dev, int64_t numel, void* stream);
int gtav_dit_finalize(gtav_dit* h, void* stream);
int gtav_dit_get_weight(gtav_dit* h, const char* name, float* dst_dev, int64_t numel, void* stream);

int gtav_dit_forward(gtav_dit* h, const float* x_dev, const int64_t* t_dev, const float* actions_dev, float* out_dev,
                     int32_t B, int32_t T, void* stream);

int gtav_dit_set_schedule(gtav_dit* h, const float* alphas_cumprod_host, int32_t n);

int gtav_dit_denoise_step(gtav_dit* h, float* x_dev, int32_t B, int32_t F, int32_t start, int32_t cur, int32_t t_ctx,
                          int32_t t_cur, int32_t t_next, int32_t is_final, const float* actions_dev, int32_t mode,
                          int32_t cond_step, float* v_out_dev, void* stream);
int gtav_dit_prepare_frame(gtav_dit* h, int32_t B, int32_t F, int32_t start, int32_t cur, int32_t t_ctx,
                           const int32_t* t_steps_host, int32_t n_steps, const float* actions_dev, void* stream);

int gtav_dit_set_graph(gtav_dit* h, int32_t enable);

int gtav_dit_set_fused_temporal(gtav_dit* h, int32_t enable);

int gtav_dit_set_fused_spatial(gtav_dit* h, int32_t enable);
int gtav_dit_fused_launches(gtav_dit* h, int32_t B, int32_t T, int32_t t0);

int gtav_dit_set_weight_prefetch(gtav_dit* h, int32_t mode);

#define GTAV_PROFILE_CLASSES 9
int gtav_dit_profile(gtav_dit* h, int32_t enable);
int gtav_dit_profile_read(gtav_dit* h, double* ms_by_class, int64_t* launches_by_class);

int gtav_timer_calibrate(int32_t spin_us, int32_t reps, double* event_us_mean, double* device_us_mean, void* stream);

int gtav_dit_train_param_count(gtav_dit* h, int64_t* numel);
int gtav_dit_train_enable(gtav_dit* h, float* grad_arena_dev, int64_t grad_arena_numel);
int gtav_dit_train_enable_typed(gtav_dit* h, float* grad_arena_dev, int64_t grad_arena_numel, int32_t dtype);
int gtav_dit_set_loss_scale(gtav_dit* h, float scale);
int gtav_dit_set_grad_divisor(gtav_dit* h, float divisor);
int gtav_dit_zero_grad(gtav_dit* h, void* stream);
int gtav_dit_train_forward(gtav_dit* h, const float* x_dev, const int64_t* t_dev, const float* actions_dev, float* out_dev,
                           int32_t B, int32_t T, void* stream);
int gtav_dit_train_backward(gtav_dit* h, const float* v_pred_dev, const float* v_target_dev, void* stream);
int gtav_dit_train_get_residual(gtav_dit* h, int32_t k, float* dst_dev, int64_t numel, void* stream);
int gtav_dit_train_backward_phases(gtav_dit* h, const float* v_pred_dev, const float* v_target_dev, int32_t phase_begin, int32_t phase_end,
                                   void* stream);
int gtav_dit_train_param_range(gtav_dit* h, const char* prefix, int64_t* offset, int64_t* count);
int gtav_dit_get_grad(gtav_dit* h, const char* name, float* dst_dev, int64_t numel, void* stream);
int gtav_dit_adamw_step(gtav_dit* h, float lr, float beta1, float beta2, float eps, float weight_decay, float max_grad_norm, void* stream);
int gtav_dit_train_stats(gtav_dit* h, float* out4_host, void* stream);
int gtav_dit_get_opt_state(gtav_dit* h, const char* name, float* m_dst_dev, float* v_dst_dev, int64_t numel, void* stream);
int gtav_dit_set_opt_state(gtav_dit* h, const char* name, const float* m_src_dev, const float* v_src_dev, int64_t numel, void* stream);
int gtav_dit_get_opt_step(gtav_dit* h, int64_t* applied_steps, int64_t* skipped_steps, void* stream);
int gtav_dit_set_opt_step(gtav_dit* h, int64_t applied_steps, int64_t skipped_steps, void* stream);

int gtav_dit_check(gtav_dit* h, void* stream);

#define GTAV_OPERAND_F16 0
#define GTAV_OPERAND_BF16 1
int gtav_dit_operand_groups(gtav_dit* h, int32_t* n_groups);
int gtav_dit_set_operand_dtype(gtav_dit* h, int32_t group, int32_t dtype);
int gtav_dit_get_operand_dtype(gtav_dit* h, int32_t group, int32_t* dtype);
int gtav_dit_autorange(gtav_dit* h, int32_t* n_switched, void* stream);

typedef struct gtav_vae_config {
    int32_t latent_dim, input_height, input_width, patch_size;
    int32_t enc_dim, enc_depth, enc_heads, dec_dim, dec_depth, dec_heads;
    float mlp_ratio;
    int32_t use_variational;
    int32_t max_frames_per_call;
} gtav_vae_config;

typedef struct gtav_vae gtav_vae;

int gtav_vae_create(const gtav_vae_config* cfg, gtav_vae** out);
void gtav_vae_destroy(gtav_vae* h);
int gtav_vae_set_weight(gtav_vae* h, const char* name, const float* src_dev, int64_t numel, void* stream);
int gtav_vae_finalize(gtav_vae* h, void* stream);
int gtav_vae_get_weight(gtav_vae* h, const char* name, float* dst_dev, int64_t numel, void* stream);

int gtav_vae_encode(gtav_vae* h, const float* img_dev, float in_scale, float in_shift, float* moments_dev, int32_t N,
                    void* stream);
int gtav_vae_decode(gtav_vae* h, const float* z_dev, float z_scale, float* img_dev, float out_scale, float out_shift,
                    int32_t N, void* stream);

int gtav_vae_check(gtav_vae* h, void* stream);
int gtav_vae_set_operand_dtype(gtav_vae* h, int32_t dtype);
int gtav_vae_get_operand_dtype(gtav_vae* h, int32_t* dtype);
int gtav_vae_profile(gtav_vae* h, int32_t enable);
int gtav_vae_profile_read(gtav_vae* h, double* ms_by_class, int64_t* launches_by_class);

int gtav_ddim_update(const float* x_dev, const float* v_dev, float* out_dev, int32_t rows, int32_t n,
                     const float* alpha_t_dev, const float* alpha_next_dev, int32_t is_final, void* stream);
int gtav_add_noise(const float* x_dev, const float* noise_dev, const float* alpha_dev, float* out_dev, int32_t rows,
                   int32_t n, float clamp_abs, void* stream);
int gtav_vtarget(const float* x_dev, const float* noise_dev, const float* alpha_dev, float* vt_dev, int32_t rows,
                 int32_t n, float clamp_abs, void* stream);
int gtav_axpy_f32(float* y_dev, const float* x_dev, float alpha, int64_t n, void* stream);
int gtav_mse(const float* a_dev, int64_t a_stride, const float* b_dev, int64_t b_stride, int32_t rows, int32_t n,
             float* out_dev, void* stream);
int gtav_clamp_frames(float* x_dev, int32_t B, int32_t F, int32_t first, int32_t n, float lo, float hi, void* stream);
int gtav_frames_to_u8(const float* img_dev, uint8_t* out_dev, int32_t N, int32_t H, int32_t W, void* stream);
int gtav_moments_to_latents(const float* moments_dev, float* lat_dev, int32_t N, int32_t hw, int32_t latent,
                            int32_t mom_ch, float scale, void* stream);
int gtav_strip_to_frames(const uint8_t* strip_dev, int32_t H, int32_t W, int32_t n_frames, float* out_dev, int32_t OH, int32_t OW,
                         void* stream);
int gtav_resize_frames(const float* src_dev, float* dst_dev, int32_t N, int32_t H, int32_t W, int32_t OH, int32_t OW, void* stream);
// ... 55 lines not shown
```

Measured before the change: 5.029.

## Fuse unpatchify and DDIM update into final GEMM epilogue; cache conditioning tables

The final projection GEMM can now write its output through a sampler-tail epilogue. That epilogue unpatchifies only the last frame of each sample and applies the DDIM update to x in place, replacing the separate unpatchify and ddim_update launches and the fp32 intermediate round trip. Separately, prepare_frame remembers the key of its last conditioning tables (B, T, t_ctx, step list, fold mask) and skips the host sync, memcpy and skinny GEMMs when the key repeats with no actions. Both paths are on by default (mask 31). The tail adds scattered per-element stores and index math in the GEMM epilogue, and the table cache adds invalidation hooks throughout the API.

Result: no change. 5.025 (median of 2 runs) (-0.1%).

```diff
diff --git a/ai-generated-gtav_amd/csrc/api_dit.hip b/ai-generated-gtav_amd/csrc/api_dit.hip
--- a/ai-generated-gtav_amd/csrc/api_dit.hip
+++ b/ai-generated-gtav_amd/csrc/api_dit.hip
@@ -92,7 +92,7 @@
 }
 
 static int dit_forward_core(gtav_dit* h, const float* x_src, const int* frame_index, int B, int Tq, int t0,
-                            const float* mod, const int* mod_rows, const float* ctab, float* v_out, hipStream_t s) {
+                            const float* mod, const int* mod_rows, const float* ctab, float* v_out, hipStream_t s, const SamplerTail* tail = nullptr) {
     const int D = h->D, P = h->P, NB = B * Tq, M = NB * P;
     GTAV_REQUIRE(M <= h->Mmax, "forward: %d tokens exceed workspace (%d)", M, h->Mmax);
     bool fold_a, fold_b;
@@ -236,8 +236,9 @@
     memset(&g, 0, sizeof(g));
     g.X = h->xn; g.ldx = D; g.W = h->w_final; g.M = M; g.N = h->Nfin; g.K = D; g.bias = h->b_final; g.out = h->fo; g.ldo = h->Nfin;
     if (folded_in) fold_consumer(g, 4 * h->L, h->Nfin);
+    if (tail) g.tail = *tail;
     PROF(h, PC_OTHER, s, h->ops(g_final).gemm(g, folded_in ? EPI_F32_FOLD : EPI_F32, s));
-    PROF(h, PC_OTHER, s, launch_unpatchify(h->fo, h->Nfin, v_out, NB, h->C, h->H, h->W, h->p, 0, 1.f, 0.f, s));
+    if (!tail) PROF(h, PC_OTHER, s, launch_unpatchify(h->fo, h->Nfin, v_out, NB, h->C, h->H, h->W, h->p, 0, 1.f, 0.f, s));
     PROF(h, PC_EMPTY, s, 0);
     return h->prof.collect(s);
 }
@@ -368,6 +369,7 @@
         n = spatial ? "spatial_rotary_emb.freqs" : "temporal_rotary_emb.freqs";
     }
     h->finalized = false;
+    h->cond_tab.valid = false;
     return h->wt.set(n.c_str(), src, numel, (hipStream_t)stream);
 }
 
@@ -381,6 +383,7 @@
     hipStream_t s = (hipStream_t)stream;
     RET_IF(h->wt.check_complete());
     GTAV_CHECK_HIP(hipStreamSynchronize(s));
+    h->cond_tab.valid = false;
     const int D = h->D;
     RET_IF(launch_add_f32(h->b_t2, h->b_ext, h->b_t2a, D, s));
     std::vector<float> fs(16), ft(32);
@@ -432,7 +435,7 @@
     GTAV_REQUIRE(B >= 1 && B <= h->maxB && T >= 1 && T <= h->maxT, "dit_forward: B=%d T=%d outside capacity (%d, %d)", B, T, h->maxB, h->maxT);
     GTAV_REQUIRE(!actions || h->A > 0, "dit_forward: model has no external_cond");
     hipStream_t s = (hipStream_t)stream;
-    h->prepared.valid = false;
+    h->drop_prepared();
     h->kvrec.valid = false;
     RET_IF(dit_cond(h, t, B * T, 1, nullptr, 0, actions, h->A, 0, s));
     return dit_forward_core(h, x, nullptr, B, T, 0, h->mod, nullptr, h->fold.ctab, out, s);
@@ -450,6 +453,10 @@
     const size_t fsz = (size_t)h->C * h->H * h->W;
     const int Tq = mode == 1 ? 1 : T, t0 = mode == 1 ? T - 1 : 0;
     if (!prepared) RET_IF(dit_cond(h, nullptr, B * Tq, Tq, h->step_dev, mode == 1, actions, (int64_t)F * h->A, h->A, s));
+    if ((h->fused_ends & 2) && !h->prof.on && h->C % 4 == 0) {
+        const SamplerTail tail{x, v_out, h->step_dev, h->P, Tq, h->C, h->H, h->W, h->p, F};
+        return dit_forward_core(h, x, h->frame_idx, B, Tq, t0, prepared ? h->mod_cur : h->mod, nullptr, prepared ? h->fold.ctab_cur : h->fold.ctab, nullptr, s, &tail);
+    }
     RET_IF(dit_forward_core(h, x, h->frame_idx, B, Tq, t0, prepared ? h->mod_cur : h->mod, nullptr, prepared ? h->fold.ctab_cur : h->fold.ctab, h->vout, s));
     const float* vlast = h->vout + (size_t)(Tq - 1) * fsz;
     RET_IF(launch_ddim_update_step(x, F, vlast, (size_t)Tq * fsz, B, (int)fsz, h->step_dev, s));
@@ -468,6 +475,20 @@
     const int rows = B * (T - 1) + n_steps * B;
     GTAV_REQUIRE(rows <= h->max_rows, "prepare_frame: %d conditioning rows exceed max_cond_rows %d", rows, h->max_rows);
     hipStream_t s = (hipStream_t)stream;
+    bool fa, fb, fa1, fb1;
+    fold_policy(h, B * T * h->P, fa, fb);
+    fold_policy(h, B * h->P, fa1, fb1);
+    const int fold_mask = ((fa || fa1) ? 1 : 0) | ((fb || fb1) ? 2 : 0);
+    bool keyable = !actions && !h->tr.on && t_ctx >= 0 && t_ctx <= 999;
+    for (int i = 0; keyable && i < n_steps; ++i) keyable = t_steps_host[i] >= 0 && t_steps_host[i] <= 999;
+    auto& ct = h->cond_tab;
+    if (keyable && (h->fused_ends & 4) && ct.valid && ct.B == B && ct.T == T && ct.t_ctx == t_ctx && ct.fold_mask == fold_mask &&
+        (int)ct.t_steps.size() == n_steps && !memcmp(ct.t_steps.data(), t_steps_host, n_steps * sizeof(int))) {
+        h->prepared.valid = true; h->prepared.B = B; h->prepared.F = F; h->prepared.start = start; h->prepared.cur = cur;
+        h->prepared.n_steps = n_steps; h->prepared.actions = nullptr;
+        return 0;
+    }
+    h->drop_prepared();
     GTAV_CHECK_HIP(hipStreamSynchronize(s));
     GTAV_CHECK_HIP(hipMemcpy(h->t_steps_dev, t_steps_host, n_steps * sizeof(int), hipMemcpyHostToDevice));
     const int ldhc = h->D + h->Apad;
@@ -476,16 +497,15 @@
     RET_IF(launch_skinny_f32(h->E, 256, h->w_t0, h->b_t0, h->HC, ldhc, rows, h->D, 256, 1, s));
     RET_IF(launch_skinny_f32(h->HC, ldhc, h->w_t2cat, actions ? h->b_t2a : h->b_t2, h->Sc, h->D, rows, h->D, ldhc, 1, s));
     RET_IF(launch_skinny_f32(h->Sc, h->D, h->w_ada, h->b_ada, h->mod, h->MODW, rows, h->MODW, h->D, 0, s));
-    {
-        bool fa, fb, fa1, fb1;
-        fold_policy(h, B * T * h->P, fa, fb);
-        fold_policy(h, B * h->P, fa1, fb1);
-        RET_IF(dit_fold_tables(h, rows, fa || fa1, fb || fb1, s));
-        h->prepared.fold_tables = fa || fa1 || fb || fb1;
-    }
+    RET_IF(dit_fold_tables(h, rows, fa || fa1, fb || fb1, s));
+    h->prepared.fold_tables = fold_mask != 0;
     GTAV_CHECK_HIP(hipMemsetAsync(h->mod_last, 0xFF, (size_t)h->maxB * h->maxT * sizeof(int), s));
     h->prepared.valid = true; h->prepared.B = B; h->prepared.F = F; h->prepared.start = start; h->prepared.cur = cur;
     h->prepared.n_steps = n_steps; h->prepared.actions = actions;
+    if (keyable) {
+        ct.valid = true; ct.B = B; ct.T = T; ct.t_ctx = t_ctx; ct.fold_mask = fold_mask;
+        ct.t_steps.assign(t_steps_host, t_steps_host + n_steps);
+    }
     return 0;
 }
 
@@ -505,7 +525,7 @@
                          h->prepared.cur == cur && cond_step < h->prepared.n_steps && h->prepared.actions == actions,
                      "denoise_step: cond_step=%d but gtav_dit_prepare_frame was not called for this window", cond_step);
     else
-        h->prepared.valid = false;
+        h->drop_prepared();
     if (mode == 1) {
         GTAV_REQUIRE(h->kvrec.valid && h->kvrec.B == B && h->kvrec.F == F && h->kvrec.start == start && h->kvrec.cur == cur &&
                          h->kvrec.x == (const void*)x,
@@ -600,7 +620,7 @@
     for (auto& kv : h->graphs)
         if (kv.second) (void)hipGraphExecDestroy(kv.second);
     h->graphs.clear();
-    h->prepared.valid = false;
+    h->drop_prepared();
     h->fold.mode = mode;
     return 0;
 }
@@ -643,6 +663,17 @@
         if (h->finalized) GTAV_CHECK_HIP(hipDeviceSynchronize());
     }
     h->fuse_sattn = enable != 0;
+    return 0;
+}
+
+int gtav_dit_set_fused_ends(gtav_dit* h, int32_t mask) {
+    GTAV_REQUIRE(h && mask >= 0 && mask <= 31, "dit_set_fused_ends: mask %d (bit 1 one-launch tail, bit 2 conditioning-table reuse; bits 0, 3 and 4 reserved)", mask);
+    if (h->fused_ends != mask) {
+        for (auto& kv : h->graphs)
+            if (kv.second) (void)hipGraphExecDestroy(kv.second);
+        h->graphs.clear();
+    }
+    h->fused_ends = mask;
     return 0;
 }
 
@@ -714,6 +745,7 @@
     if (changed) {
         h->finalized = false;
         h->kvrec.valid = false;
+        h->cond_tab.valid = false;
         dit_drop_graphs(h);
     }
     h->any_bf16 = false;
diff --git a/ai-generated-gtav_amd/csrc/api_internal.h b/ai-generated-gtav_amd/csrc/api_internal.h
--- a/ai-generated-gtav_amd/csrc/api_internal.h
+++ b/ai-generated-gtav_amd/csrc/api_internal.h
@@ -263,6 +263,9 @@
     int *mod_last = nullptr, *mod_changed = nullptr;
     int* t_steps_dev = nullptr;
     struct { bool valid = false, fold_tables = false; int B = 0, F = 0, start = 0, cur = 0, n_steps = 0; const float* actions = nullptr; } prepared;
+    struct { bool valid = false; int B = 0, T = 0, t_ctx = 0, fold_mask = 0; std::vector<int> t_steps; } cond_tab;
+    void drop_prepared() { prepared.valid = false; cond_tab.valid = false; }
+    int fused_ends = 31;
     struct { bool valid = false; int B = 0, F = 0, start = 0, cur = 0; const void* x = nullptr; } kvrec;
     struct GraphKey {
         int B, F, T, mode;
diff --git a/ai-generated-gtav_amd/csrc/api_train.hip b/ai-generated-gtav_amd/csrc/api_train.hip
--- a/ai-generated-gtav_amd/csrc/api_train.hip
+++ b/ai-generated-gtav_amd/csrc/api_train.hip
@@ -47,6 +47,7 @@
 static int train_enable_body(gtav_dit* h, float* grad_arena_dev, int64_t grad_arena_numel) {
     for (auto& kv : h->wt.slots) GTAV_REQUIRE(!kv.second.set, "train_enable: call it before any gtav_dit_set_weight (the fp32 masters are filled by set_weight)");
     gtav_dit::Train& t = h->tr;
+    h->cond_tab.valid = false;
     Arena& a = h->arena;
     const int D = h->D, L = h->L, Hp = h->Hm_pad;
     GTAV_REQUIRE(h->Hm == h->Hm_pad && h->Kpe == h->C * h->p * h->p, "train_enable: padded MLP width / patch size are not implemented for training");
@@ -191,7 +192,7 @@
     hipStream_t s = (hipStream_t)stream;
     gtav_dit::Train& tr = h->tr;
     const int D = h->D, P = h->P, NB = B * T, M = NB * P, L = h->L, rows = NB, ldhc = D + h->Apad;
-    h->prepared.valid = false;
+    h->drop_prepared();
     h->kvrec.valid = false;
     RET_IF(launch_cond_inputs(t64, rows, 1, nullptr, 0, h->sincos, h->E, actions, h->A, 0, h->A, h->HC, ldhc, D, h->Apad, h->err_flag, s));
     RET_IF(launch_skinny_f32(h->E, 256, h->w_t0, h->b_t0, tr.z0, D, rows, D, 256, 0, s));
@@ -472,7 +473,7 @@
     RET_IF(launch_clip_coef(tr.ctl, tr.sumsq_part, sumsq_parts(tr.grad_count), 1.0f / (tr.loss_scale * tr.grad_div), max_grad_norm, beta1, beta2, h->err_flag, s));
     RET_IF(operand_ops(tr.bf16).adamw_multi(tr.adam_params, tr.adam_items, tr.adam_n_items, tr.ctl, lr, beta1, beta2, eps, weight_decay, s));
     RET_IF(launch_add_f32(h->b_t2, h->b_ext, h->b_t2a, h->D, s));
-    h->prepared.valid = false;
+    h->drop_prepared();
     h->kvrec.valid = false;
     return 0;
 }
diff --git a/ai-generated-gtav_amd/csrc/common.h b/ai-generated-gtav_amd/csrc/common.h
--- a/ai-generated-gtav_amd/csrc/common.h
+++ b/ai-generated-gtav_amd/csrc/common.h
@@ -104,9 +104,32 @@
     int rt, nkt, splitk;
     int kt_limit;
 };
+struct StepParams {
+    int first;
+    int cur;
+    int t_ctx;
+    int t_cur;
+    int is_final;
+    float alpha_t, alpha_next;
+    int cond_step;
+};
+struct SamplerTail {
+    float* x;
+    float* v_out;
+    const StepParams* sp;
+    int P, Tq, C, H, W, p, F;
+};
 }
 namespace gtav {
 using gtav_shared::PrefetchDesc;
+using gtav_shared::StepParams;
+using gtav_shared::SamplerTail;
+__device__ __forceinline__ float ddim_one(float xc, float vp, float at, float an, int is_final) {
+    const float x0 = sqrtf(at) * xc - sqrtf(1.0f - at) * vp;
+    if (is_final) return x0;
+    const float eps = (sqrtf(1.0f / at) * xc - x0) / sqrtf(1.0f / at - 1.0f);
+    return sqrtf(an) * x0 + sqrtf(1.0f - an) * eps;
+}
 __device__ __forceinline__ void l2_prefetch_slice(const PrefetchDesc& d, int xcd, int j, int nb, int t, int nt, unsigned& sink) {
     const int sk = d.splitk;
     int ks0, ksn, rt0, rtn;
diff --git a/ai-generated-gtav_amd/csrc/elementwise.hip b/ai-generated-gtav_amd/csrc/elementwise.hip
--- a/ai-generated-gtav_amd/csrc/elementwise.hip
+++ b/ai-generated-gtav_amd/csrc/elementwise.hip
@@ -399,13 +399,6 @@
     for (int j = threadIdx.x; j < Apad; j += blockDim.x) HC[(size_t)r * ldhc + D + j] = (arow && j < A) ? arow[j] : 0.f;
 }
 
-__device__ __forceinline__ float ddim_one(float xc, float vp, float at, float an, int is_final) {
-    const float x0 = sqrtf(at) * xc - sqrtf(1.0f - at) * vp;
-    if (is_final) return x0;
-    const float eps = (sqrtf(1.0f / at) * xc - x0) / sqrtf(1.0f / at - 1.0f);
-    return sqrtf(an) * x0 + sqrtf(1.0f - an) * eps;
-}
-
 __global__ void ddim_update_kernel(const float* __restrict__ x, size_t x_stride, const float* __restrict__ v, size_t v_stride,
                                    float* __restrict__ out, size_t out_stride, int n, const float* __restrict__ alpha_t,
                                    const float* __restrict__ alpha_next, int is_final) {
diff --git a/ai-generated-gtav_amd/csrc/gemm.hip b/ai-generated-gtav_amd/csrc/gemm.hip
--- a/ai-generated-gtav_amd/csrc/gemm.hip
+++ b/ai-generated-gtav_amd/csrc/gemm.hip
@@ -955,6 +955,25 @@
             xpre[i][j] = f32x4{0.f, 0.f, 0.f, 0.f};
             if (cw && n < p.N && m < p.M) xpre[i][j] = *(const f32x4*)((const float*)p.out + (size_t)m * p.ldo + n);
         }
+    }
+}
+
+__device__ __forceinline__ void sampler_tail_store(const SamplerTail& t, int m, int n, const f32x4& v) {
+    const int nb = m / t.P, b = nb / t.Tq;
+    if (nb - b * t.Tq != t.Tq - 1) return;
+    const int tok = m - nb * t.P, gw = t.W / t.p, ty = tok / gw, tx = tok - ty * gw;
+    const int q = n / t.C, c = n - q * t.C, ph = q / t.p, pw = q - ph * t.p;
+    const size_t hw = (size_t)t.H * t.W, fsz = (size_t)t.C * hw;
+    const size_t o = (size_t)c * hw + (size_t)(ty * t.p + ph) * t.W + (tx * t.p + pw);
+    const StepParams* sp = t.sp;
+    const float at = sp->alpha_t, an = sp->alpha_next;
+    const int fin = sp->is_final;
+    float* xf = t.x + ((size_t)b * t.F + sp->cur) * fsz + o;
+#pragma unroll
+    for (int e = 0; e < 4; ++e) {
+        const float ve = 1.f * v[e] + 0.f;
+        xf[e * hw] = ddim_one(xf[e * hw], ve, at, an, fin);
+        if (t.v_out) t.v_out[(size_t)b * fsz + o + e * hw] = ve;
     }
 }
 
@@ -1276,7 +1295,8 @@
                 if (p.out_sc1) store16_sc1(dst, v);
                 else *(f32x4*)dst = v;
             } else if constexpr (EPI == EPI_F32) {
-                *(f32x4*)((float*)p.out + (size_t)m * p.ldo + n) = v;
+                if (p.tail.x) sampler_tail_store(p.tail, m, n, v);
+                else *(f32x4*)((float*)p.out + (size_t)m * p.ldo + n) = v;
             } else if constexpr (EPI == EPI_F16) {
                 *(uint2*)((f16*)p.out + (size_t)m * p.ldo + n) = pack4(amax, v[0], v[1], v[2], v[3]);
             } else if constexpr (EPI == EPI_QKV) {
@@ -2963,6 +2983,13 @@
     GTAV_REQUIRE(p.K > 0 && p.K % TK == 0, "gemm: K=%d must be a positive multiple of %d", p.K, TK);
     GTAV_REQUIRE(p.M > 0 && p.N > 0 && p.N % 4 == 0, "gemm: bad M=%d N=%d", p.M, p.N);
     GTAV_REQUIRE(((uintptr_t)p.X & 15) == 0 && ((uintptr_t)p.W & 15) == 0, "gemm: operands must be 16-byte aligned");
+    if (p.tail.x) {
+        const SamplerTail& t = p.tail;
+        GTAV_REQUIRE(epi == EPI_F32 && !g_force_wm, "gemm: the sampler tail is an EPI_F32 epilogue of the heuristic's block shapes");
+        GTAV_REQUIRE(t.sp && t.C > 0 && t.C % 4 == 0 && t.p > 0 && t.H % t.p == 0 && t.W % t.p == 0 && t.P == (t.H / t.p) * (t.W / t.p) && p.N == t.C * t.p * t.p &&
+                         t.Tq >= 1 && p.M % (t.P * t.Tq) == 0 && t.F >= 1,
+                     "gemm: bad sampler-tail geometry (N=%d, C=%d, patch %d, %d x %d, %d tokens per frame, %d frames per sample, M=%d)", p.N, t.C, t.p, t.H, t.W, t.P, t.Tq, p.M);
+    }
     int splitk = 1;
     if (epi == EPI_QKV) {
         GTAV_REQUIRE(p.N == 3 * p.D && p.D % 128 == 0, "gemm/qkv: N=%d must equal 3*D, D=%d %% 128 == 0", p.N, p.D);
diff --git a/ai-generated-gtav_amd/csrc/gemm_typed.inc b/ai-generated-gtav_amd/csrc/gemm_typed.inc
--- a/ai-generated-gtav_amd/csrc/gemm_typed.inc
+++ b/ai-generated-gtav_amd/csrc/gemm_typed.inc
@@ -42,8 +42,9 @@
     float* sk_ws;
     int* sk_flags;
     int sk_dp, sk_r;
+    SamplerTail tail;
 };
-static_assert(sizeof(GemmParams) == 352, "GemmParams: every build and both operand types must see the same struct");
+static_assert(sizeof(GemmParams) == 408, "GemmParams: every build and both operand types must see the same struct");
 
 struct GemmGroup { const f16* X; const f16* W; float* out; const float* bias; int N; int ldo; };
 int launch_gemm_grouped(const GemmGroup* groups_dev, int n_groups, int max_N, int M, int K, hipStream_t stream);
diff --git a/ai-generated-gtav_amd/csrc/ops.h b/ai-generated-gtav_amd/csrc/ops.h
--- a/ai-generated-gtav_amd/csrc/ops.h
+++ b/ai-generated-gtav_amd/csrc/ops.h
@@ -10,15 +10,6 @@
                       int K, int act_silu, hipStream_t stream);
 int skinny_init();
 
-struct StepParams {
-    int first;
-    int cur;
-    int t_ctx;
-    int t_cur;
-    int is_final;
-    float alpha_t, alpha_next;
-    int cond_step;
-};
 int launch_step_setup(StepParams* dst, const StepParams& v, int* frame_idx, int* mod_rows, int* last_rows, int* changed, int B, int Tq, int T, int F,
                       int use_cur, hipStream_t stream);
 int launch_gather_rows(const float* table, const int* rows, const int* changed, float* cur, int slots, int W, const float* table2, float* cur2, int W2,
diff --git a/ai-generated-gtav_amd/csrc/ops_bf16.h b/ai-generated-gtav_amd/csrc/ops_bf16.h
--- a/ai-generated-gtav_amd/csrc/ops_bf16.h
+++ b/ai-generated-gtav_amd/csrc/ops_bf16.h
@@ -4,6 +4,7 @@
 namespace gtav_bf16 {
 typedef __bf16 f16;
 using gtav_shared::PrefetchDesc;
+using gtav_shared::SamplerTail;
 #include "gemm_typed.inc"
 #include "ops_typed.inc"
 }
diff --git a/ai-generated-gtav_amd/lib.py b/ai-generated-gtav_amd/lib.py
--- a/ai-generated-gtav_amd/lib.py
+++ b/ai-generated-gtav_amd/lib.py
@@ -82,6 +82,7 @@
     "gtav_dit_set_graph": [_p, _i],
     "gtav_dit_set_fused_temporal": [_p, _i],
     "gtav_dit_set_fused_spatial": [_p, _i],
+    "gtav_dit_set_fused_ends": [_p, _i],
     "gtav_dit_fused_launches": [_p, _i, _i, _i],
     "gtav_dit_set_weight_prefetch": [_p, _i],
     "gtav_dit_profile": [_p, _i],
diff --git a/ai-generated-gtav_amd/model/dit.py b/ai-generated-gtav_amd/model/dit.py
--- a/ai-generated-gtav_amd/model/dit.py
+++ b/ai-generated-gtav_amd/model/dit.py
@@ -241,6 +241,8 @@
                     _lib.check(L.gtav_dit_set_fused_temporal(self._handle, 1))
                 if getattr(self, "_fused_spatial", None) is not None:
                     _lib.check(L.gtav_dit_set_fused_spatial(self._handle, int(self._fused_spatial)))
+                if getattr(self, "_fused_ends", None) is not None:
+                    _lib.check(L.gtav_dit_set_fused_ends(self._handle, int(self._fused_ends)))
                 if getattr(self, "_fold", None) is not None:
                     _lib.check(L.gtav_dit_set_fold(self._handle, *self._fold))
                 if getattr(self, "_weight_prefetch", None) is not None:
@@ -471,6 +473,11 @@
         if self._handle:
             _lib.check(_lib.load().gtav_dit_set_fused_spatial(self._handle, int(self._fused_spatial)))
 
+    def set_fused_ends(self, mask: int):
+        self._fused_ends = int(mask)
+        if self._handle:
+            _lib.check(_lib.load().gtav_dit_set_fused_ends(self._handle, self._fused_ends))
+
     def fused_launches(self, B: int, T: int, t0: int = 0) -> int:
         self._ensure(B, T)
         return int(_lib.load().gtav_dit_fused_launches(self._handle, int(B), int(T), int(t0)))
diff --git a/include/gtav_amd.h b/include/gtav_amd.h
--- a/include/gtav_amd.h
+++ b/include/gtav_amd.h
@@ -42,6 +42,7 @@
 int gtav_dit_set_fused_temporal(gtav_dit* h, int32_t enable);
 
 int gtav_dit_set_fused_spatial(gtav_dit* h, int32_t enable);
+int gtav_dit_set_fused_ends(gtav_dit* h, int32_t mask);
 int gtav_dit_fused_launches(gtav_dit* h, int32_t B, int32_t T, int32_t t0);
 
 int gtav_dit_set_weight_prefetch(gtav_dit* h, int32_t mode);
```
